# NTU-CompHydroMet-Lab/P2I-GAN-benchmark

Measured on AMD Instinct MI355X. Metric: train frames/sec (128x128x16), higher is better.
Workload: dtype f32

## Files before the change

include/p2i_hip.h:

```cpp
#ifndef P2I_HIP_H
#define P2I_HIP_H
#include <stdint.h>

#ifdef __cplusplus
extern "C" {
#endif

#define P2I_OK 0
#define P2I_EINVAL (-1)
#define P2I_ELDS (-2)

#define P2I_ACT_NONE 0
#define P2I_ACT_RELU 1
#define P2I_ACT_LEAKY 2
#define P2I_ACT_TANH 3

int p2i_abi_version(void);
const char* p2i_last_error(void);

typedef struct {
  int B, Cin, Cout;
  int Ti, Hi, Wi;
  int To, Ho, Wo;
  int kt, kh, kw;
  int st, sh, sw;
  int pt, ph, pw;
} p2i_conv_desc;

int p2i_conv_fwd(const p2i_conv_desc* d, const float* x, const float* wp, const float* bias,
                 const float* residual, float* y, int act, void* stream);
int p2i_conv_dgrad(const p2i_conv_desc* d, const float* dy, const float* y_act, int act,
                   const float* wp_d, const float* dx_add, const float* mask_y, int mask_act,
                   float* dx, void* stream);
int p2i_conv_wgrad(const p2i_conv_desc* d, const float* x, const float* dy, const float* y_act,
                   int act, float* dwp, float* dbias, void* stream);
int p2i_conv_wgrad_ws(const p2i_conv_desc* d, const float* x, const float* dy, const float* y_act, int act, float* dwp,
                      float* dbias, float* ws, int64_t ws_floats, void* stream);
int p2i_conv_fwd_x6(const p2i_conv_desc* d, const float* x, const float* wp, uint16_t* wsplit, const float* bias,
                    const float* residual, float* y, int act, void* stream);
int p2i_conv_dgrad_x6(const p2i_conv_desc* d, const float* dy, const float* wp_d, uint16_t* wsplit, const float* dx_add,
                      const float* mask_y, int mask_act, float* dx, void* stream);
int p2i_x6_split(const float* wp, uint16_t* wb, int ntaps, int K, int Mpad, void* stream);
int p2i_x6_split_batched(const float* const* wp, uint16_t* const* wb, const int* ntaps, const int* K, const int* Mpad, int n,
                         void* stream);
int p2i_x6c_would_take(const p2i_conv_desc* d, int dgrad, int act);
int p2i_conv_fwd_x6s(const p2i_conv_desc* d, const float* x, const float* wp, const uint16_t* wb_layer, int ntaps_w,
                     const float* bias, const float* residual, float* y, int act, void* stream);
int p2i_conv_dgrad_x6s(const p2i_conv_desc* d, const float* dy, const float* wp_d, const uint16_t* wb_layer, int ntaps_w,
                       const float* dx_add, const float* mask_y, int mask_act, float* dx, void* stream);
int p2i_conv_last_plan(int* out6);
int p2i_fast_div_magic(int d, uint32_t* magic);
int p2i_wgrad_last_plan(int* out4);

int p2i_doconv_fold_fwd(const float* W, const float* D, const float* D_diag, int O, int I, int groups,
                        int ksz, int identity_rep, float* wp_f, float* wp_d, void* stream);
int p2i_doconv_fold_bwd(const float* dwp_f, const float* W, const float* D, const float* D_diag,
                        int O, int I, int groups, int ksz, float* dW, float* dD, void* stream);

int p2i_doconv_fold_fwd_batched(const float* const* W, const float* const* D, const float* const* D_diag, int n, int O, int I,
                                float* const* wp_f, float* const* wp_d, void* stream);
int p2i_doconv_fold_bwd_batched(const float* const* dwp_f, const float* const* W, const float* const* D,
                                const float* const* D_diag, int n, int O, int I, float* const* dW, float* const* dD,
                                void* stream);

int p2i_weight_pack(const float* w, int O, int I, int ntaps, const float* inv_div_ptr,
                    float* wp_f, float* wp_d, void* stream);
int p2i_weight_unpack_grad(const float* dwp_f, int O, int I, int ntaps, const float* w_orig,
                           const float* sigma_ptr, const float* u, const float* v, float* scratch,
                           float* dw, void* stream);

int p2i_weight_pack_batched(const float* const* w, const int* O, const int* I, const int* ntaps, const float* const* inv_div,
                            float* const* wp_f, float* const* wp_d, int n, void* stream);
int p2i_weight_unpack_grad_batched(const float* const* dwp_f, const int* O, const int* I, const int* ntaps,
                                   const float* const* w_orig, const float* const* sigma, const float* const* u,
                                   const float* const* v, float* dots, float* const* dw, int n, void* stream);

int p2i_weight_unpack_grad_batched_acc(const float* const* dwp_f, const int* O, const int* I, const int* ntaps,
                                       const float* const* w_orig, const float* const* sigma, const float* const* u,
                                       const float* const* v, float* dots, float* const* dw, int n, int accumulate, void* stream);

int p2i_spectral_norm(const float* w, int O, int K, float* u, float* v, int training, float* sigma,
                      float* scratch, void* stream);

int p2i_spectral_norm_batched(const float* const* w, const int* O, const int* K, float* const* u, float* const* v,
                              int training, float* const* sigma, float* const* scratch, float* const* u_snap,
                              float* const* v_snap, int n, void* stream);

int p2i_attn_fwd(const float* x, const float* w0, const float* b0, const float* w1, const float* b1,
                 float* out, int B, int T, int HW, void* stream);
int p2i_attn_bwd(const float* x, const float* w0, const float* b0, const float* w1, const float* b1,
                 const float* dout, float* dw0, float* db0, float* dw1, float* db1,
                 int B, int T, int HW, void* stream);

int p2i_idw_fwd(const float* vals_src, const float* mask, const float* grid_x, const float* grid_y,
                const float* grid_z, float* out, int32_t* pt_pos, int32_t* pt_count, int32_t* frame_count,
                int32_t* row_start, float* pt_xyzn, int32_t* sel_idx, float* sel_w, int B, int T, int H, int W, float tau,
                void* stream);
int p2i_idw_fwd_ws(const float* vals_src, const float* mask, const float* grid_x, const float* grid_y,
                   const float* grid_z, float* out, int32_t* pt_pos, int32_t* pt_count, int32_t* frame_count,
                   int32_t* row_start, float* pt_xyzn, int32_t* sel_idx, float* sel_w, int32_t* amb, int B, int T, int H, int W,
                   float tau, void* stream);
int p2i_idw_bwd(const float* dout, const int32_t* pt_pos, const int32_t* pt_count, const int32_t* sel_idx,
                const float* sel_w, float* dvals_src, int B, int T, int H, int W, void* stream);

int p2i_pooldup_fwd(const float* x, float* y, int B, int C, int H, int W, void* stream);
int p2i_pooldup_bwd(const float* x, const float* dy, float* dx, int B, int C, int H, int W, void* stream);

int p2i_upmod_fwd(const float* x, const float* pos, float* u, int B, int C, int S, int S2w , void* stream);
int p2i_upmod_fwd_ba(const float* v, const float* pos, const float* bias, int act, float* u, int B, int C, int S, int S2w, void* stream);
int p2i_upmod_bwd(const float* x, const float* pos, const float* du, float* dx, float* dpos,
                  int B, int C, int S, int S2w, void* stream);

int p2i_dtail_fwd(const float* out2d, const float* out3d, const float* alpha2d, float* fused,
                  int B, int H2, int W2, int T3, int H3, int W3, void* stream);
int p2i_dtail_bwd(const float* out2d, const float* alpha2d, const float* dfused, float* dout2d,
                  float* dout3d, float* dalpha2d, int B, int H2, int W2, int T3, int H3, int W3, void* stream);

int p2i_recloss(const float* pred, const float* target, float k1_alpha, float* out3, float* dpred,
                float* scratch, int B, int T, int HW, void* stream);
int p2i_gan_loss(const float* logits_a, const float* logits_b, int n, int loss_type, int mode,
                 float weight, float real_label, float fake_label, float* loss, float* dlogits_a,
                 float* dlogits_b, void* stream);

int p2i_loss_transform_fwd(const float* x, float* y, int64_t n, void* stream);
int p2i_loss_transform_bwd(const float* x, const float* dy, float* dx, int64_t n, void* stream);
int p2i_fdiff_fwd(const float* x, float* out, int B, int T, int64_t inner, void* stream);
int p2i_fdiff_bwd(const float* dy, float* dx, int B, int T, int64_t inner, void* stream);
int p2i_wl1_fwd(const float* pred, const float* target, float* out1, int64_t n, void* stream);
int p2i_wl1_bwd(const float* pred, const float* target, const float* gout, float* dpred, int64_t n, void* stream);
int p2i_softmax_t_fwd(const float* x, float* y, int rows, int L, float temperature, void* stream);
int p2i_softmax_t_bwd(const float* y, const float* dy, float* dx, int rows, int L, float temperature, void* stream);
int p2i_kl_fwd(const float* p, const float* q, float* out1, int64_t n, int B, void* stream);
// ... 226 lines not shown
```

p2i-gan-benchmark_amd/csrc/conv.hip:

```cpp
#include "conv_dma.h"

namespace p2i {


template <int MB, int NPIX, int WAVES_M, int CK>
__global__ __launch_bounds__(256) void patch_gemm_kernel(const PatchGeom g) {
  extern __shared__ __attribute__((aligned(16))) float smem[];
  constexpr int WAVES_N = 4 / WAVES_M;
  constexpr int TM = MB / (32 * WAVES_M);
  constexpr int TN = NPIX / (32 * WAVES_N);
  static_assert(TM >= 1 && TN >= 1, "tile too small");
  float* lw = smem;
  float* lp = smem + g.ntaps * CK * MB;

  const int tid = threadIdx.x, lane = tid & 63, wave = tid >> 6;
  const int wm = wave / WAVES_N, wn = wave % WAVES_N;
  const int l31 = lane & 31, lhi = lane >> 5;

  int tile = blockIdx.x;
  const int tw = tile % g.ntw; tile /= g.ntw;
  const int th = tile % g.nth; tile /= g.nth;
  const int tt = tile % g.ntt;
  const int tb = tile / g.ntt;
  const int j0b = tb << g.ljb, j0t = tt << g.ljt, j0h = th << g.ljh, j0w = tw << g.ljw;
// ... 81 lines not shown
    }
  }

  const int dHW = g.dH * g.dW;
#pragma unroll
  for (int f = 0; f < TN; ++f) {
    const int pix = (wn * TN + f) * 32 + l31;
    const int gw = j0w + (pix & JWm);
    const int gh = j0h + ((pix >> g.ljw) & JHm);
    const int gt = j0t + ((pix >> (g.ljw + g.ljh)) & JTm);
    const int gb = j0b + (pix >> (g.ljw + g.ljh + g.ljt));
    const bool pv = gb < g.B && gt < g.nT && gh < g.nH && gw < g.nW;
    const int sp = (gt * g.oT + g.pT) * dHW + (gh * g.oH + g.pH) * g.dW + gw * g.oW + g.pW;
#pragma unroll
    for (int i = 0; i < TM; ++i) {
#pragma unroll
      for (int r = 0; r < 16; ++r) {
        const int o = o0 + (wm * TM + i) * 32 + (r & 3) + 8 * (r >> 2) + 4 * lhi;
        if (pv && o < g.Cm) {
          float v = acc[i][f][r];
          if (g.bias) v += g.bias[o];
          v = act_apply(v, g.act_epi);
          const size_t di = ((size_t)(gb * g.Cm + o)) * g.dT * dHW + sp;
          if (g.res) v += g.res[di];
          if (g.mask_y) v = act_grad(v, g.mask_y[di], g.mask_act);
          g.dst[di] = v;
        }
      }
    }
  }
}


typedef void (*patch_fn)(const PatchGeom);
template <int MB, int NPIX, int WM, int CK>
static int launch_patch(const PatchGeom& g, dim3 grid, size_t lds, hipStream_t s) {
  auto k = patch_gemm_kernel<MB, NPIX, WM, CK>;
  static bool attr_set = false;
  if (!attr_set) {
    (void)hipFuncSetAttribute((const void*)k, hipFuncAttributeMaxDynamicSharedMemorySize, 160 * 1024);
    attr_set = true;
  }
  P2I_LAUNCH(k, grid, dim3(256), lds, s, g);
  return launch_status();
}

static int dispatch_patch_dma(const TileCfg& c, int KG, const PatchGeom& g, dim3 grid, size_t lds, hipStream_t s) {
  int rc = dispatch_patch_dma_g0(c, KG, g, grid, lds, s);
  if (rc == -1) rc = dispatch_patch_dma_g1(c, KG, g, grid, lds, s);
  if (rc == -1) rc = dispatch_patch_dma_g2(c, KG, g, grid, lds, s);
  if (rc == -1) rc = dispatch_patch_dma_g3(c, KG, g, grid, lds, s);
  if (rc != -1) return rc;
  set_error("no DMA kernel instance for tile cfg %d %d %d %d kg %d", c.MB, c.NPIX, c.WM, c.CK, KG);
  return P2I_EINVAL;
}

static int dispatch_patch(const TileCfg& c, const PatchGeom& g, dim3 grid, size_t lds, hipStream_t s) {
#define P2I_CASE(mb_, npix_, wm_, ck_) \
  if (c.MB == mb_ && c.NPIX == npix_ && c.WM == wm_ && c.CK == ck_) return launch_patch<mb_, npix_, wm_, ck_>(g, grid, lds, s);
  P2I_CASE(128, 256, 2, 8)
  P2I_CASE(64, 256, 1, 8)
  P2I_CASE(64, 128, 2, 8)
  P2I_CASE(32, 128, 1, 8)
  P2I_CASE(128, 256, 2, 4)
  P2I_CASE(64, 256, 1, 4)
  P2I_CASE(64, 128, 2, 4)
  P2I_CASE(32, 128, 1, 4)
  P2I_CASE(128, 256, 2, 2)
  P2I_CASE(64, 256, 1, 2)
  P2I_CASE(64, 128, 2, 2)
  P2I_CASE(32, 128, 1, 2)
#undef P2I_CASE
  set_error("no kernel instance for tile cfg %d %d %d %d", c.MB, c.NPIX, c.WM, c.CK);
  return P2I_EINVAL;
}


static thread_local int g_last_plan[6] = {0, 0, 0, 0, 0, 0};

static int run_patch_gemm(PatchGeom g, const ClassSpec& cs, hipStream_t s);

static int run_patch_gemm_classes(PatchGeom g, const ClassSpec* css, int ncls, hipStream_t s) {
  if (g.src_y != nullptr || ncls > MAX_CLASSES) return 1;
  if (const X6Ctx& xc = x6_ctx(); xc.wb != nullptr) {
    bool all = true;
    for (int q = 0; q < ncls && all; ++q) all = run_patch_gemm_x6c(g, css[q], xc.wb, xc.ntaps_w, nullptr, s, true) == 0;
    if (all) {
      for (int q = 0; q < ncls; ++q)
        if (const int rc = run_patch_gemm_x6c(g, css[q], xc.wb, xc.ntaps_w, g_last_plan, s)) return rc == 1 ? P2I_EINVAL : rc;
      return P2I_OK;
    }
  }
  const ClassSpec& c0s = css[0];
  g.mT = c0s.mT; g.mH = c0s.mH; g.mW = c0s.mW;
  g.oT = c0s.oT; g.oH = c0s.oH; g.oW = c0s.oW;
  int lo[MAX_CLASSES][3], rng[3] = {0, 0, 0}, mx[3] = {0, 0, 0}, max_taps = 0;
  long long total_pix = 0;
  for (int q = 0; q < ncls; ++q) {
    const ClassSpec& cs = css[q];
    int hi[3] = {0, 0, 0};
    lo[q][0] = lo[q][1] = lo[q][2] = 0;
    for (int i = 0; i < cs.ntaps; ++i) {
      const int d[3] = {cs.dt[i], cs.dh[i], cs.dw[i]};
      for (int k = 0; k < 3; ++k) {
        if (i == 0 || d[k] < lo[q][k]) lo[q][k] = d[k];
        if (i == 0 || d[k] > hi[k]) hi[k] = d[k];
      }
    }
    for (int k = 0; k < 3; ++k) if (hi[k] - lo[q][k] > rng[k]) rng[k] = hi[k] - lo[q][k];
    if (cs.nT > mx[0]) mx[0] = cs.nT;
    if (cs.nH > mx[1]) mx[1] = cs.nH;
    if (cs.nW > mx[2]) mx[2] = cs.nW;
    if (cs.ntaps > max_taps) max_taps = cs.ntaps;
    total_pix += (long long)g.B * (cs.nT > 0 ? cs.nT : 0) * (cs.nH > 0 ? cs.nH : 0) * (cs.nW > 0 ? cs.nW : 0);
  }
  if (mx[0] <= 0 || mx[1] <= 0 || mx[2] <= 0) return P2I_OK;
  if (max_taps == 0) max_taps = 1;
  g.ntaps = max_taps;
  static const int cand[5][3] = {{128, 256, 2}, {64, 256, 1}, {128, 128, 2}, {64, 128, 2}, {32, 128, 1}};
  int best = -1, best_ck = 0;
  long long best_score = -1;
  PatchGeom bg = g;
  size_t best_lds = 0;
  dim3 best_grid;
  for (int ci = 0; ci < 5; ++ci) {
    const int MBc = cand[ci][0], NP = cand[ci][1];
    if (MBc > 32 && g.Cm <= MBc / 2) continue;
    int jb, jt, jh, jw;
    pick_tile_dims(NP, g.B, mx[0], mx[1], mx[2], jb, jt, jh, jw);
    PatchGeom t = g;
    t.ljb = ilog2(jb); t.ljt = ilog2(jt); t.ljh = ilog2(jh); t.ljw = ilog2(jw);
    t.eT = (jt - 1) * g.mT + rng[0] + 1;
    t.eH = patch_extent_div((jh - 1) * g.mH + rng[1] + 1);
    t.eW = (jw - 1) * g.mW + rng[2] + 1;
    bool same_lo_w = true;
    for (int q = 1; q < ncls; ++q) same_lo_w = same_lo_w && lo[q][2] == lo[0][2];
    t.v4 = (conv_v4_on() && same_lo_w && (g.sW & 3) == 0 && ((jw * g.mW) & 3) == 0) ? 1 : 0;
    t.v4sh = 0;
    if (t.v4) {
      t.v4sh = ((lo[0][2] % 4) + 4) % 4;
      t.eW = (t.eW + t.v4sh + 3) & ~3;
      t.eW4 = t.eW >> 2;
    }
    if (!t.v4) t.eW = patch_extent_div(t.eW);
    t.eWp = t.eW;
    t.eth = t.eT * t.eH;
    t.rpc = jb * t.eth;
    t.CSl = t.rpc * t.eW;
    t.CS = t.CSl;
    t.G4 = t.CSl >> 2;
    const int force_ck16 = P2I_ENV_ONCE("P2I_CONV_CK16", 0);
    for (int CKc = ((max_taps <= 4 || ((force_ck16 || g.Ck >= 256) && max_taps == 9 && MBc <= 64)) ? 16 : 8); CKc >= 2; CKc >>= 1) {
      if (g.Ck >= CKc ? (g.Ck % CKc != 0) : (CKc != 2 && g.Ck * 2 <= CKc)) continue;
      if (CKc == 2 && !(MBc == 64 && NP == 128) && !(MBc == 32)) continue;
      if ((CKc == 4 || CKc == 16) && MBc == 128 && NP == 128) continue;
      const int PT = CKc * t.CSl;
      if (PT >= 65536 || t.CSl >= 65536) continue;
      const int PTp = t.v4 ? (((PT >> 2) + 63) & ~63) * 4 : (PT + 63) & ~63;
      const int nwrows = max_taps * CKc;
      const size_t WSZ = (size_t)((nwrows * (MBc / 4) + 63) & ~63) * 4;
      const size_t lds = sizeof(float) * (((nwrows + 63) & ~63) + (size_t)PTp + 2 * (WSZ + PTp));
      if (lds > 160 * 1024) continue;
      const long long nb = (long long)ceil_div(g.Cm, MBc) * ((total_pix + NP - 1) / NP);
      long long score = (nb >= 256 ? 1000000000ll : nb * 1000000ll) + (long long)MBc * NP * 10 + CKc + (lds <= 80 * 1024 ? 5 : 0);
      if (score > best_score) {
        best_score = score; best = ci; best_ck = CKc; best_lds = lds;
        bg = t; bg.PT = PT;
// ... 224 lines not shown
        cs.ntaps = n;
        if (mergeable) css[ncls++] = cs;
        else if (int e = run_patch_gemm(g, cs, (hipStream_t)stream)) return e;
      }
  if (mergeable) {
    int rc = 1;
    if (const X6Ctx& xc = x6_ctx(); xc.wb != nullptr && ncls == 4)
      rc = run_patch_gemm_x6c_fused(g, css, ncls, xc.wb, xc.ntaps_w, g_last_plan, (hipStream_t)stream);
    if (rc == 1) rc = (ncls > 1 && x6_ctx().wb == nullptr) ? run_patch_gemm_fused(g, css, ncls, g_last_plan, (hipStream_t)stream) : 1;
    if (rc == 1) rc = ncls > 1 ? run_patch_gemm_classes(g, css, ncls, (hipStream_t)stream) : 1;
    if (rc == 1) {
      for (int q = 0; q < ncls; ++q)
        if (int e = run_patch_gemm(g, css[q], (hipStream_t)stream)) return e;
    } else if (rc != P2I_OK) return rc;
  }
  return P2I_OK;
}


namespace p2i { int x6_split_weights(const float* wp, uint16_t* wb, int ntaps, int Ck, int CmPad, hipStream_t s); }


extern "C" int p2i_conv_fwd_x6(const p2i_conv_desc* d, const float* x, const float* wp, uint16_t* wsplit, const float* bias,
                               const float* residual, float* y, int act, void* stream) {
  if (int e = check_desc(d)) return e;
  if (wsplit == nullptr || (d->Cin & 15) != 0 || !x6c_would_take(d, false, act))
    return p2i_conv_fwd(d, x, wp, bias, residual, y, act, stream);
  P2I_REQUIRE(wp != nullptr, "null pointer");
  const int nt = d->kt * d->kh * d->kw;
  if (int e = x6_split_weights(wp, wsplit, nt, d->Cin, (d->Cout + 31) / 32 * 32, (hipStream_t)stream)) return e;
  x6_ctx() = X6Ctx{wsplit, nt};
  const int rc = p2i_conv_fwd(d, x, wp, bias, residual, y, act, stream);
  x6_ctx() = X6Ctx{nullptr, 0};
  return rc;
}

extern "C" int p2i_conv_dgrad_x6(const p2i_conv_desc* d, const float* dy, const float* wp_d, uint16_t* wsplit, const float* dx_add,
                                 const float* mask_y, int mask_act, float* dx, void* stream) {
  if (int e = check_desc(d)) return e;
  if (wsplit == nullptr || (d->Cout & 15) != 0 || d->Cin == 1 || !x6c_would_take(d, true, P2I_ACT_NONE))
    return p2i_conv_dgrad(d, dy, nullptr, P2I_ACT_NONE, wp_d, dx_add, mask_y, mask_act, dx, stream);
  P2I_REQUIRE(wp_d != nullptr, "null pointer");
  const int nt = d->kt * d->kh * d->kw;
  if (int e = x6_split_weights(wp_d, wsplit, nt, d->Cout, (d->Cin + 31) / 32 * 32, (hipStream_t)stream)) return e;
  x6_ctx() = X6Ctx{wsplit, nt};
  const int rc = p2i_conv_dgrad(d, dy, nullptr, P2I_ACT_NONE, wp_d, dx_add, mask_y, mask_act, dx, stream);
  x6_ctx() = X6Ctx{nullptr, 0};
  return rc;
}

extern "C" int p2i_x6_split(const float* wp, uint16_t* wb, int ntaps, int K, int Mpad, void* stream) {
  P2I_REQUIRE(wp && wb && ntaps > 0 && K > 0 && (K & 7) == 0 && Mpad > 0 && (Mpad & 31) == 0, "p2i_x6_split: bad arguments");
  return x6_split_weights(wp, wb, ntaps, K, Mpad, (hipStream_t)stream);
}

extern "C" int p2i_x6c_would_take(const p2i_conv_desc* d, int dgrad, int act) {
  if (check_desc(d)) return 0;
  if (dgrad ? ((d->Cout & 15) != 0 || d->Cin == 1) : (d->Cin & 15) != 0) return 0;
  return x6c_would_take(d, dgrad != 0, dgrad ? P2I_ACT_NONE : act) ? 1 : 0;
}

extern "C" int p2i_conv_fwd_x6s(const p2i_conv_desc* d, const float* x, const float* wp, const uint16_t* wb_layer, int ntaps_w,
                                const float* bias, const float* residual, float* y, int act, void* stream) {
  if (int e = check_desc(d)) return e;
  if (wb_layer == nullptr || (d->Cin & 15) != 0 || !x6c_would_take(d, false, act)) return p2i_conv_fwd(d, x, wp, bias, residual, y, act, stream);
  P2I_REQUIRE(ntaps_w >= d->kt * d->kh * d->kw, "ntaps_w smaller than the layer's tap count");
  x6_ctx() = X6Ctx{wb_layer, ntaps_w};
  const int rc = p2i_conv_fwd(d, x, wp, bias, residual, y, act, stream);
  x6_ctx() = X6Ctx{nullptr, 0};
  return rc;
}

extern "C" int p2i_conv_dgrad_x6s(const p2i_conv_desc* d, const float* dy, const float* wp_d, const uint16_t* wb_layer, int ntaps_w,
                                  const float* dx_add, const float* mask_y, int mask_act, float* dx, void* stream) {
  if (int e = check_desc(d)) return e;
  if (wb_layer == nullptr || (d->Cout & 15) != 0 || d->Cin == 1 || !x6c_would_take(d, true, P2I_ACT_NONE))
    return p2i_conv_dgrad(d, dy, nullptr, P2I_ACT_NONE, wp_d, dx_add, mask_y, mask_act, dx, stream);
  P2I_REQUIRE(ntaps_w >= d->kt * d->kh * d->kw, "ntaps_w smaller than the layer's tap count");
  x6_ctx() = X6Ctx{wb_layer, ntaps_w};
  const int rc = p2i_conv_dgrad(d, dy, nullptr, P2I_ACT_NONE, wp_d, dx_add, mask_y, mask_act, dx, stream);
  x6_ctx() = X6Ctx{nullptr, 0};
  return rc;
}
```

p2i-gan-benchmark_amd/csrc/conv_common.h:

```cpp
#pragma once
#include "common.h"

namespace p2i {

typedef float f32x16 __attribute__((ext_vector_type(16)));
constexpr int MAX_TAPS = 27;

typedef __attribute__((address_space(3))) void lds_void;
typedef int v4i32 __attribute__((ext_vector_type(4)));

__device__ __forceinline__ v4i32 make_rsrc(const void* p, unsigned bytes) {
  const unsigned long long a = (unsigned long long)p;
  v4i32 r;
  r[0] = __builtin_amdgcn_readfirstlane((int)(unsigned)a);
  r[1] = __builtin_amdgcn_readfirstlane((int)(unsigned)(a >> 32));
  r[2] = __builtin_amdgcn_readfirstlane((int)bytes);
  r[3] = 0x00020000;
  return r;
}
__device__ __forceinline__ unsigned lds_base(const float* shared_array) {
  return (unsigned)(size_t)(const lds_void*)shared_array;
}
__device__ __forceinline__ void dma_b32(const v4i32 rsrc, unsigned lds_addr, int voff, int soff) {
  const unsigned la = __builtin_amdgcn_readfirstlane(lds_addr);
// ... 59 lines not shown
                                                  const float* __restrict__ res, const float* __restrict__ mask_y, int mask_act,
                                                  float* __restrict__ dst, bool atomic_out) {
#pragma unroll
  for (int k = 0; k < 8; ++k) {
    float v = acc[h8 * 8 + k];
    if (bias) v += b.bv[k];
    v = act_apply(v, act_epi);
    if (res) v += b.rv[k];
    if (mask_y) v = act_grad(v, b.mv[k], mask_act);
    if (b.ok[k]) {
      if (atomic_out) atomicAdd(dst + b.di[k], v);
      else dst[b.di[k]] = v;
    }
  }
}
__device__ __forceinline__ void epilogue_tile16(const f32x16& acc, int o_base, int lhi, int Cm, bool pv, size_t pos_off, size_t chan_stride,
                                                const float* __restrict__ bias, int act_epi, const float* __restrict__ res,
                                                const float* __restrict__ mask_y, int mask_act, float* __restrict__ dst,
                                                bool atomic_out = false) {
#pragma unroll
  for (int h8 = 0; h8 < 2; ++h8) {
    int di[8];
    bool ok[8];
#pragma unroll
    for (int k = 0; k < 8; ++k) {
      const int r = h8 * 8 + k;
      const int o = o_base + (r & 3) + 8 * (r >> 2) + 4 * lhi;
      ok[k] = pv && o < Cm;
      di[k] = ok[k] ? (int)((size_t)o * chan_stride + pos_off) : 0;
    }
    float rv[8], mv[8];
    if (res) {
#pragma unroll
      for (int k = 0; k < 8; ++k) rv[k] = res[di[k]];
    }
    if (mask_y) {
#pragma unroll
      for (int k = 0; k < 8; ++k) mv[k] = mask_y[di[k]];
    }
#pragma unroll
    for (int k = 0; k < 8; ++k) {
      const int r = h8 * 8 + k;
      const int o = o_base + (r & 3) + 8 * (r >> 2) + 4 * lhi;
      float v = acc[r];
      if (bias) v += bias[o < Cm ? o : 0];
      v = act_apply(v, act_epi);
      if (res) v += rv[k];
      if (mask_y) v = act_grad(v, mv[k], mask_act);
      if (ok[k]) {
        if (atomic_out) atomicAdd(dst + di[k], v);
        else dst[di[k]] = v;
      }
    }
    __builtin_amdgcn_sched_barrier(0);
  }
}

typedef float f32x4e __attribute__((ext_vector_type(4)));
struct EpiOps4v {
  int di[4];
  bool ok[4];
  f32x4e rv[4], mv[4];
  float bv[4];
};
__device__ __forceinline__ void epi_tile16_v4_fetch(EpiOps4v& b, int o_base, int lane, int Cm, size_t pos4_off, bool pv4, size_t chan_stride,
                                                    const float* __restrict__ bias, const float* __restrict__ res, const float* __restrict__ mask_y) {
#pragma unroll
  for (int k = 0; k < 4; ++k) {
    const int o = o_base + k * 8 + (lane >> 3);
    b.ok[k] = pv4 && o < Cm;
    b.di[k] = b.ok[k] ? (int)((size_t)o * chan_stride + pos4_off) : 0;
    b.bv[k] = bias ? bias[o < Cm ? o : 0] : 0.f;
  }
  if (res) {
#pragma unroll
    for (int k = 0; k < 4; ++k) b.rv[k] = *reinterpret_cast<const f32x4e*>(res + b.di[k]);
  }
  if (mask_y) {
#pragma unroll
    for (int k = 0; k < 4; ++k) b.mv[k] = *reinterpret_cast<const f32x4e*>(mask_y + b.di[k]);
  }
}
__device__ __forceinline__ void epi_tile16_v4_finish(const EpiOps4v& b, const f32x16& acc, float* __restrict__ tile_lds, int lane, int act_epi, const float* __restrict__ res,
                                                     const float* __restrict__ mask_y, int mask_act, float* __restrict__ dst, bool atomic_out) {
  constexpr int PITCH = 36;
  const int l31 = lane & 31, lhi = lane >> 5;
#pragma unroll
  for (int r = 0; r < 16; ++r) tile_lds[((r & 3) + 8 * (r >> 2) + 4 * lhi) * PITCH + l31] = acc[r];
  __builtin_amdgcn_fence(__ATOMIC_RELEASE, "wavefront");
  __builtin_amdgcn_wave_barrier();
  const int p4 = (lane & 7) * 4;
  f32x4e v[4];
#pragma unroll
  for (int k = 0; k < 4; ++k) v[k] = *reinterpret_cast<const f32x4e*>(tile_lds + (k * 8 + (lane >> 3)) * PITCH + p4);
#pragma unroll
  for (int k = 0; k < 4; ++k) {
#pragma unroll
    for (int e = 0; e < 4; ++e) {
      float x = act_apply(v[k][e] + b.bv[k], act_epi);
      if (res) x += b.rv[k][e];
      if (mask_y) x = act_grad(x, b.mv[k][e], mask_act);
      v[k][e] = x;
    }
    if (b.ok[k]) {
      if (atomic_out) {
#pragma unroll
        for (int e = 0; e < 4; ++e) atomicAdd(dst + b.di[k] + e, v[k][e]);
      } else {
        *reinterpret_cast<f32x4e*>(dst + b.di[k]) = v[k];
      }
    }
  }
  __builtin_amdgcn_wave_barrier();
}

typedef float f32x2e __attribute__((ext_vector_type(2)));
struct EpiOps4p {
  int di[4];
  bool ok[4];
  f32x2e rv[4], mv[4];
};
__device__ __forceinline__ void epi_pair16_fetch(EpiOps4p& b, int h4, int o_base, int lhi, int Cm, bool pv, size_t pos_off, size_t chan_stride,
                                                 const float* __restrict__ res, const float* __restrict__ mask_y) {
#pragma unroll
  for (int k = 0; k < 4; ++k) {
    const int r = h4 * 4 + k;
    const int o = o_base + (r & 3) + 8 * (r >> 2) + 4 * lhi;
    b.ok[k] = pv && o < Cm;
    b.di[k] = b.ok[k] ? (int)((size_t)o * chan_stride + pos_off) : 0;
  }
  if (res) {
#pragma unroll
    for (int k = 0; k < 4; ++k) b.rv[k] = *reinterpret_cast<const f32x2e*>(res + b.di[k]);
  }
  if (mask_y) {
#pragma unroll
    for (int k = 0; k < 4; ++k) b.mv[k] = *reinterpret_cast<const f32x2e*>(mask_y + b.di[k]);
  }
}
__device__ __forceinline__ void epi_pair16_finish(const EpiOps4p& b, int h4, const f32x16& acc0, const f32x16& acc1,
                                                  const float* __restrict__ res, const float* __restrict__ mask_y, int mask_act,
                                                  float* __restrict__ dst, bool atomic_out) {
#pragma unroll
  for (int k = 0; k < 4; ++k) {
    const int r = h4 * 4 + k;
    f32x2e v;
    v[0] = acc0[r]; v[1] = acc1[r];
    if (res) { v[0] += b.rv[k][0]; v[1] += b.rv[k][1]; }
    if (mask_y) { v[0] = act_grad(v[0], b.mv[k][0], mask_act); v[1] = act_grad(v[1], b.mv[k][1], mask_act); }
    if (b.ok[k]) {
      if (atomic_out) { atomicAdd(dst + b.di[k], v[0]); atomicAdd(dst + b.di[k] + 1, v[1]); }
      else *reinterpret_cast<f32x2e*>(dst + b.di[k]) = v;
    }
  }
}
__device__ __forceinline__ void epilogue_pair16(const f32x16& acc0, const f32x16& acc1, int o_base, int lhi, int Cm, bool pv, size_t pos_off,
                                                size_t chan_stride, const float* __restrict__ res, const float* __restrict__ mask_y,
                                                int mask_act, float* __restrict__ dst, bool atomic_out = false) {
#pragma unroll
  for (int h4 = 0; h4 < 4; ++h4) {
    int di[4];
    bool ok[4];
#pragma unroll
    for (int k = 0; k < 4; ++k) {
      const int r = h4 * 4 + k;
      const int o = o_base + (r & 3) + 8 * (r >> 2) + 4 * lhi;
      ok[k] = pv && o < Cm;
      di[k] = ok[k] ? (int)((size_t)o * chan_stride + pos_off) : 0;
    }
    f32x2e rv[4], mv[4];
    if (res) {
#pragma unroll
      for (int k = 0; k < 4; ++k) rv[k] = *reinterpret_cast<const f32x2e*>(res + di[k]);
    }
    if (mask_y) {
#pragma unroll
      for (int k = 0; k < 4; ++k) mv[k] = *reinterpret_cast<const f32x2e*>(mask_y + di[k]);
    }
#pragma unroll
    for (int k = 0; k < 4; ++k) {
      const int r = h4 * 4 + k;
      f32x2e v;
      v[0] = acc0[r]; v[1] = acc1[r];
      if (res) { v[0] += rv[k][0]; v[1] += rv[k][1]; }
      if (mask_y) { v[0] = act_grad(v[0], mv[k][0], mask_act); v[1] = act_grad(v[1], mv[k][1], mask_act); }
      if (ok[k]) {
        if (atomic_out) { atomicAdd(dst + di[k], v[0]); atomicAdd(dst + di[k] + 1, v[1]); }
        else *reinterpret_cast<f32x2e*>(dst + di[k]) = v;
      }
    }
    __builtin_amdgcn_sched_barrier(0);
  }
// ... 9 lines not shown
  jt = pow2_ceil(nT); if (jt > rem) jt = rem;
  rem /= jt;
  jb = rem;
  (void)B;
}


static inline int check_desc(const p2i_conv_desc* d) {
  P2I_REQUIRE(d != nullptr, "null conv desc");
  P2I_REQUIRE(d->B > 0 && d->Cin > 0 && d->Cout > 0, "bad channel/batch dims");
  P2I_REQUIRE(d->kt >= 1 && d->kh >= 1 && d->kw >= 1 && d->kt * d->kh * d->kw <= MAX_TAPS, "kernel taps > %d", MAX_TAPS);
  P2I_REQUIRE(d->st >= 1 && d->sh >= 1 && d->sw >= 1, "bad stride");
  P2I_REQUIRE(d->To == (d->Ti + 2 * d->pt - d->kt) / d->st + 1, "To inconsistent");
  P2I_REQUIRE(d->Ho == (d->Hi + 2 * d->ph - d->kh) / d->sh + 1, "Ho inconsistent");
  P2I_REQUIRE(d->Wo == (d->Wi + 2 * d->pw - d->kw) / d->sw + 1, "Wo inconsistent");
  const long long nin = (long long)d->B * d->Cin * d->Ti * d->Hi * d->Wi;
  const long long nout = (long long)d->B * d->Cout * d->To * d->Ho * d->Wo;
  P2I_REQUIRE(nin < (1ll << 31) && nout < (1ll << 31), "tensor too large for 32-bit indexing");
  return P2I_OK;
}


struct ClassGeom {
  int nT, nH, nW, pT, pH, pW, bT, bH, bW, ntaps;
  short tap_w[MAX_TAPS];
  int tap_off[MAX_TAPS];
};
constexpr int MAX_CLASSES = 8;

struct PatchGeom {
  const float* src;
  const float* src_y;
  const float* wp;
  const float* bias;
  const float* res;
  float* dst;
  int act_epi;
  int act_pro;
  int B, Ck, Cm, CmPad;
  int sT, sH, sW;
  int dT, dH, dW;
  int nT, nH, nW;
  int mT, mH, mW;
  int oT, oH, oW;
  int pT, pH, pW;
  int bT, bH, bW;
  int eT, eH, eW, eWp;
  int ljb, ljt, ljh, ljw;
  int ntt, nth, ntw;
  int ntaps;
  int CS;
  int rpc, eth;
  unsigned mg_rpc, mg_eth, mg_eh;
  short tap_w[MAX_TAPS];
  int tap_off[MAX_TAPS];
  const float* mask_y;
  int mask_act;
  int CSl;
  int PT;
  unsigned src_bytes, wp_bytes;
  unsigned mg_csl, mg_ew;
  int v4, v4sh;
  int eW4, G4;
  unsigned mg_g4, mg_ew4;
  const uint16_t* wb;
  unsigned wb_bytes;
  int ntaps_w;
  int TG, NTP, R;
  int ksplit;
  int pair_w;
  int nclass;
  ClassGeom cls[MAX_CLASSES];
};

struct ClassSpec {
  int nT, nH, nW;
  int mT, mH, mW;
  int oT, oH, oW, pT, pH, pW;
  int ntaps;
  short tw[MAX_TAPS];
  int dt[MAX_TAPS], dh[MAX_TAPS], dw[MAX_TAPS];
};

struct X6Ctx { const uint16_t* wb; int ntaps_w; };
X6Ctx& x6_ctx();

int run_patch_gemm_x6c(const PatchGeom& g, const ClassSpec& cs, const uint16_t* wb, int ntaps_w, int* plan6, hipStream_t s, bool dry = false);
int run_patch_gemm_x6c_fused(const PatchGeom& g, const ClassSpec* css, int ncls, const uint16_t* wb, int ntaps_w, int* plan6, hipStream_t s, bool dry = false);
bool x6c_would_take(const p2i_conv_desc* d, bool dgrad, int act_epi);

int run_patch_gemm_fused(PatchGeom g, const ClassSpec* css, int ncls, int* plan6, hipStream_t s);

int c1_dgrad(const p2i_conv_desc* d, const float* dy, const float* wp_d, const float* add, const float* mask_y, int mask_act,
             float* dx, hipStream_t s);
int c1_wgrad(const p2i_conv_desc* d, const float* x, const float* dy, float* dwp, float* dbias, hipStream_t s);
int c1_fwd(const p2i_conv_desc* d, const float* x, const float* wp, const float* bias, float* y, int act, hipStream_t s);
int o1_fwd(const p2i_conv_desc* d, const float* x, const float* wp, const float* bias, float* y, int act, hipStream_t s);

}
```

p2i-gan-benchmark_amd/csrc/conv_x6c.hip:

```cpp
#include "conv_common.h"

namespace p2i {

#ifdef P2I_STAMP
extern __device__ unsigned long long* p2i_stamp_buf;
#define X6C_NOW(v) do { __builtin_amdgcn_sched_barrier(0); asm volatile("s_memtime %0\n\ts_waitcnt lgkmcnt(0)" : "=s"(v) :: "memory"); __builtin_amdgcn_sched_barrier(0); } while (0)
#define X6C_ACC(sum, t_prev) do { unsigned long long t_; X6C_NOW(t_); sum += t_ - t_prev; t_prev = t_; } while (0)
#else
#define X6C_NOW(v) do { } while (0)
#define X6C_ACC(sum, t_prev) do { } while (0)
#endif

typedef __bf16 bf16x8c __attribute__((ext_vector_type(8)));
typedef unsigned u32x4c __attribute__((ext_vector_type(4)));

__device__ __forceinline__ unsigned pack_hi16c(float lo_elem, float hi_elem) {
  return __builtin_amdgcn_perm(__float_as_uint(hi_elem), __float_as_uint(lo_elem), 0x07060302u);
}
__device__ __forceinline__ float trunc_bf16c(float v) { return __uint_as_float(__float_as_uint(v) & 0xFFFF0000u); }
__device__ __forceinline__ void split8c(const float (&v)[8], u32x4c& hi, u32x4c& mid, u32x4c& lo) {
#pragma unroll
  for (int j = 0; j < 4; ++j) {
    const float a = v[2 * j], b = v[2 * j + 1];
    hi[j] = pack_hi16c(a, b);
    const float ra = a - trunc_bf16c(a), rb = b - trunc_bf16c(b);
    mid[j] = pack_hi16c(ra, rb);
    const float sa = ra - trunc_bf16c(ra), sb = rb - trunc_bf16c(rb);
    lo[j] = pack_hi16c(sa, sb);
  }
}

template <class S, class I>
__device__ __forceinline__ void split8_store(const float* __restrict__ p, S stride, u32x4c* __restrict__ out, I total, I i) {
  float v[8];
#pragma unroll
  for (int q = 0; q < 8; ++q) v[q] = p[(S)q * stride];
  u32x4c h, mi, lo;
  split8c(v, h, mi, lo);
  out[i] = h;
  out[total + i] = mi;
  out[2 * total + i] = lo;
}

__global__ __launch_bounds__(256) void wsplit_kernel(const float* __restrict__ wp, u32x4c* __restrict__ wb, int ntaps, int Ck, int CmPad) {
  const int KCt = Ck >> 3;
  const int total = ntaps * KCt * CmPad;
  for (int i = blockIdx.x * 256 + threadIdx.x; i < total; i += gridDim.x * 256) {
    const int m = i % CmPad;
    const int r = i / CmPad;
    const int kc = r % KCt, tap = r / KCt;
    const float* p = wp + ((size_t)tap * Ck + kc * 8) * CmPad + m;
    split8_store(p, (size_t)CmPad, wb, total, i);
  }
}

struct WsplitBatch { const float* wp[24]; u32x4c* wb[24]; int ntaps[24], Ck[24], CmPad[24]; };
__global__ __launch_bounds__(256) void wsplit_batched_kernel(const WsplitBatch b) {
  const int L = blockIdx.y;
  const float* wp = b.wp[L];
  u32x4c* wb = b.wb[L];
  const int Ck = b.Ck[L], CmPad = b.CmPad[L], KCt = Ck >> 3;
  const int total = b.ntaps[L] * KCt * CmPad;
  for (int i = blockIdx.x * 256 + threadIdx.x; i < total; i += gridDim.x * 256) {
    const int m = i % CmPad;
    const int r = i / CmPad;
    const int kc = r % KCt, tap = r / KCt;
    const float* p = wp + ((size_t)tap * Ck + kc * 8) * CmPad + m;
    split8_store(p, (size_t)CmPad, wb, total, i);
  }
}

__global__ __launch_bounds__(256) void split_planes_kernel(const float* __restrict__ x, u32x4c* __restrict__ planes, int B, int KCt, long long P) {
  const long long total = (long long)B * KCt * P;
  for (long long i = blockIdx.x * 256ll + threadIdx.x; i < total; i += (long long)gridDim.x * 256) {
    const long long pix = i % P, r = i / P;
    const float* px = x + (r * 8) * P + pix;
    split8_store(px, P, planes, total, i);
  }
}

X6Ctx& x6_ctx() {
  static thread_local X6Ctx c{nullptr, 0};
  return c;
}

int x6_split_weights(const float* wp, uint16_t* wb, int ntaps, int Ck, int CmPad, hipStream_t s) {
  const int total = ntaps * (Ck >> 3) * CmPad;
  const int blocks = total > 0 ? (total + 255) / 256 : 1;
  P2I_LAUNCH(wsplit_kernel, dim3(blocks > 2048 ? 2048 : blocks), dim3(256), 0, s, wp, reinterpret_cast<u32x4c*>(wb), ntaps, Ck, CmPad);
  return launch_status();
}

struct X6cGeom {
  const float* src; float* dst; const uint16_t* wb; const float* bias; const float* res; const float* mask_y;
  unsigned wb_bytes;
  int act_epi, mask_act;
  int B, Ck, Cm, CmPad;
  int sH, sW, dT, dH, dW, nH, nW;
  int ljb, ljh, ljw, eH, eW, CSl, bH, bW, nth, ntw;
  unsigned mg_ew, mg_eh;
  int ntaps_w, ksplit;
  int sT, nT, mT, oT, pT, ns, sdt0, sdt1, sdt2, swt0, swt1, swt2;
  int tap_off[9];
  int tap_w[9];
  int fused_atomic;
  int stagger;
  int vec4_epi;
  const u32x4c* splanes;
  unsigned plane_units;
  int cons_prio;
};

__device__ constexpr int X6C_CLS[9] = {3, 3, 3, 3, 2, 2, 1, 1, 0};

template <int NW> struct X6cTile {
  static constexpr int MAXCSL = NW == 8 ? 384 : 256;
  static constexpr int NI = (2 * MAXCSL + 64 * NW - 1) / (64 * NW);
};

#define X6C_WAIT1(b) asm volatile("s_waitcnt vmcnt(%0)" ::"n"(b) : "memory")
#define X6C_WAIT2(b) if (n < (b) + 1) { X6C_WAIT1(b); } else { X6C_WAIT1((b) + 1); }
#define X6C_WAIT4(b) if (n < (b) + 2) { X6C_WAIT2(b) } else { X6C_WAIT2((b) + 2) }
#define X6C_WAIT8(b) if (n < (b) + 4) { X6C_WAIT4(b) } else { X6C_WAIT4((b) + 4) }
#define X6C_WAIT16(b) if (n < (b) + 8) { X6C_WAIT8(b) } else { X6C_WAIT8((b) + 8) }
#define X6C_WAIT32(b) if (n < (b) + 16) { X6C_WAIT16(b) } else { X6C_WAIT16((b) + 16) }
__device__ __forceinline__ void x6c_wait_vm(int n) {
  if (n < 0 || n > 62) n = 0;
  if (n < 32) { X6C_WAIT32(0) } else { X6C_WAIT32(32) }
}

template <int NW, int TM, bool FUSED = false, int TPS = 3>
__global__ __launch_bounds__(64 * NW) void patch_gemm_x6c_kernel(const X6cGeom g) {
  constexpr int NCLS = FUSED ? 4 : 1;
  constexpr int NSTG = 9 / TPS;
  static_assert(TPS == 3 || TPS == 9, "taps per stage");
  extern __shared__ __attribute__((aligned(16))) float smem[];
#ifdef P2I_STAMP
  unsigned long long st_entry, st_prev, st_wait = 0, st_bar = 0, st_issue = 0, st_mfma = 0, st_loop0;
  X6C_NOW(st_entry);
#endif
  constexpr int MB = 32 * TM, NTHR = 64 * NW, NI = X6cTile<NW>::NI;
  constexpr int RING = TPS == 9 ? 3 : (TM == 2 ? 4 : 6), LEAD = RING - 1;
  constexpr int WST = 6 * TPS * MB;
  constexpr int NWI = WST / 64;
  const int CSl = g.CSl;
  int* ptab = reinterpret_cast<int*>(smem);
  const int ptab_sz = (CSl + 3) & ~3;
  u32x4c* wbuf = reinterpret_cast<u32x4c*>(smem + ptab_sz);
  u32x4c* planes = wbuf + RING * WST;
  const int PST = 6 * CSl;

  const int tid = threadIdx.x, lane = tid & 63, wave = __builtin_amdgcn_readfirstlane(tid >> 6);
  const int l31 = lane & 31, lhi = lane >> 5;
  int tile = blockIdx.x;
  const int tw = tile % g.ntw; tile /= g.ntw;
  const int th = tile % g.nth;
  const int tb = tile / g.nth;
  const int j0b = tb << g.ljb, j0h = th << g.ljh, j0w = tw << g.ljw;
  const int o0 = blockIdx.y * MB;
  const int JWm = (1 << g.ljw) - 1, JHm = (1 << g.ljh) - 1;
  const int sHW = g.sH * g.sW;
  const int src_h0 = j0h + g.bH, src_w0 = j0w + g.bW;
  const int KCt = g.Ck >> 3;
  const int cps = g.Ck >> 4;
  const int cs = g.sT * sHW;
  const int nimg = g.B * g.nT;
  const int c0 = blockIdx.z * ((g.ns * cps) / g.ksplit);

  for (int e = tid; e < CSl; e += NTHR) {
    const int row = fast_div(e, g.mg_ew);
    const int ew = e - row * g.eW;
    const int jb = fast_div(row, g.mg_eh);
    const int eh = row - jb * g.eH;
    const int n = j0b + jb, h = src_h0 + eh, w = src_w0 + ew;
    const int b = n / g.nT, lt = n - b * g.nT;
    ptab[e] = (n < nimg && (unsigned)h < (unsigned)g.sH && (unsigned)w < (unsigned)g.sW) ? ((b * g.Ck) * g.sT + lt * g.mT) * sHW + h * g.sW + w : -1;
  }
  const int pix = wave * 32 + l31;
  const int pjw = pix & JWm, pjh = (pix >> g.ljw) & JHm, pjb = pix >> (g.ljw + g.ljh);
  const int lane_base = (pjb * g.eH + pjh) * g.eW + pjw + lhi * CSl;
  int toff[9];
#pragma unroll
  for (int t = 0; t < 9; ++t) toff[t] = g.tap_off[t];

  f32x16 acc[NCLS][TM];
#pragma unroll
  for (int q = 0; q < NCLS; ++q)
#pragma unroll
    for (int i = 0; i < TM; ++i)
#pragma unroll
      for (int r = 0; r < 16; ++r) acc[q][i][r] = 0.f;

  const v4i32 rs_w = make_rsrc(g.wb, g.wb_bytes);
// ... 162 lines not shown
      if (TPS == 9 || !late) staging();
      X6C_ACC(st_issue, st_prev);
      const u32x4c* wsl = wlane + (s % RING) * WST;
      __builtin_amdgcn_sched_barrier(0);
#pragma unroll
      for (int t = 0; t < TPS - 1; ++t) {
        if constexpr (TPS == 9) {
          if (more_c && (t == 4 || t == 6 || t == 7) && t == split_t) {
            x6c_wait_vm(nwb(sa));
            __builtin_amdgcn_sched_barrier(0);
            split_patch(planes + ((c + 1) & 1) * PST);
            __builtin_amdgcn_sched_barrier(0);
          }
        }
        load_tap(wsl, pb, TPS * b + t + 1, (t + 1) % 3);
        mfma_tap(t % 3, TPS * b + t);
        ilv();
        __builtin_amdgcn_sched_barrier(0);
      }
      if (TPS == 3 && late) { staging(); __builtin_amdgcn_sched_barrier(0); }
      X6C_ACC(st_mfma, st_prev);
      {
        int n = 0;
#pragma unroll
        for (int j = 2; j <= LEAD; ++j) n += nwb(s + j);
        if constexpr (TPS == 3) {
#pragma unroll
          for (int j = 0; j <= LEAD - 2; ++j) {
            const int bj = ((b - j) % 3 + 3) % 3;
            if (bj == 0 && s - j >= 0 && (s - j) / 3 + 1 < nch) n += NPL;
          }
        }
        x6c_wait_vm(n);
      }
      asm volatile("s_waitcnt lgkmcnt(0)" ::: "memory");
      X6C_ACC(st_wait, st_prev);
      __builtin_amdgcn_s_barrier();
      X6C_ACC(st_bar, st_prev);
      if (s + 1 < nst) load_tap(wlane + ((s + 1) % RING) * WST, b == NSTG - 1 ? pbn : pb, b == NSTG - 1 ? 0 : TPS * b + TPS, 0);
      mfma_tap(2, TPS * b + TPS - 1);
      ilv();
      __builtin_amdgcn_sched_barrier(0);
      X6C_ACC(st_mfma, st_prev);
    }
  }
#ifdef P2I_STAMP
  unsigned long long st_loop_end; X6C_NOW(st_loop_end);
#endif

  const int gw = j0w + pjw, gh = j0h + pjh, gn = j0b + pjb;
  const bool pvld = gn < nimg && gh < g.nH && gw < g.nW;
  const int dHW = g.dT * g.dH * g.dW;
  const int gb_ = gn / g.nT, glt = gn - gb_ * g.nT;
  if constexpr (FUSED) {
    const size_t pos0 = (size_t)gb_ * g.Cm * dHW + (size_t)(glt * g.oT + g.pT) * g.dH * g.dW + (size_t)(2 * gh) * g.dW + 2 * gw;
#pragma unroll
    for (int ph = 0; ph < 2; ++ph)
#pragma unroll
      for (int i = 0; i < TM; ++i)
        epilogue_pair16(acc[2 * ph][i], acc[2 * ph + 1][i], o0 + i * 32, lhi, g.Cm, pvld, pos0 + (size_t)ph * g.dW, (size_t)dHW,
                        (g.fused_atomic && blockIdx.z) ? nullptr : g.res, g.mask_y, g.mask_act, g.dst, g.fused_atomic != 0);
  } else {
    const size_t pos = (size_t)gb_ * g.Cm * dHW + (size_t)(glt * g.oT + g.pT) * g.dH * g.dW + (size_t)gh * g.dW + gw;
#pragma unroll
    for (int i = 0; i < TM; ++i)
      if (g.ksplit > 1)
        epilogue_tile16(acc[0][i], o0 + i * 32, lhi, g.Cm, pvld, pos, (size_t)dHW, blockIdx.z ? nullptr : g.bias, P2I_ACT_NONE,
                        blockIdx.z ? nullptr : g.res, g.mask_y, g.mask_act, g.dst, true);
      else
        epilogue_tile16(acc[0][i], o0 + i * 32, lhi, g.Cm, pvld, pos, (size_t)dHW, g.bias, g.act_epi, g.res, g.mask_y, g.mask_act, g.dst);
  }
#ifdef P2I_STAMP
  if (p2i_stamp_buf && lane == 0) {
    asm volatile("s_waitcnt vmcnt(0)" ::: "memory");
    unsigned long long st_x; X6C_NOW(st_x);
    unsigned long long* o = p2i_stamp_buf + ((size_t)(blockIdx.x + gridDim.x * blockIdx.y) * NW + wave) * 8;
    o[0] = st_wait; o[1] = st_bar; o[2] = st_issue; o[3] = st_mfma; o[4] = st_loop_end - st_loop0; o[5] = st_loop0; o[6] = st_loop0 - st_entry;
    o[7] = st_x - st_loop_end;
  }
#endif
}


template <int TM, int TPS, bool FUSED = false, bool EPI4 = false, int NPW = 4, int TN = 2, bool PRE = false>
__global__ __launch_bounds__(64 * (4 + NPW)) void patch_gemm_x6p_kernel(const X6cGeom g) {
  constexpr int NSTG = 9 / TPS;
  constexpr int NCLS = FUSED ? 4 : 1;
  static_assert(TPS == 3 || TPS == 9, "taps per stage");
  extern __shared__ __attribute__((aligned(16))) float smem[];
  constexpr int MB = 32 * TM, NCW = 4, NTHR = 64 * (NCW + NPW), NPT = 64 * NPW;
  constexpr int NI = (2 * (TN == 2 ? X6cTile<8>::MAXCSL : X6cTile<4>::MAXCSL) + NPT - 1) / NPT;
  constexpr int RING = TPS == 9 ? 3 : (TM == 2 ? 4 : 6), LEAD = RING - 1;
  constexpr int WST = 6 * TPS * MB, NWI = WST / 64;
  const int CSl = g.CSl;
  int* ptab = reinterpret_cast<int*>(smem);
  const int ptab_sz = (CSl + 3) & ~3;
  u32x4c* wbuf = reinterpret_cast<u32x4c*>(smem + ptab_sz);
  u32x4c* planes = wbuf + RING * WST;
  const int PST = 6 * CSl;

  const int tid = threadIdx.x, lane = tid & 63, wave = __builtin_amdgcn_readfirstlane(tid >> 6);
  const int l31 = lane & 31, lhi = lane >> 5;
  int tile = blockIdx.x;
  const int tw = tile % g.ntw; tile /= g.ntw;
  const int th = tile % g.nth;
  const int tb = tile / g.nth;
  const int j0b = tb << g.ljb, j0h = th << g.ljh, j0w = tw << g.ljw;
  const int o0 = blockIdx.y * MB;
  const int JWm = (1 << g.ljw) - 1, JHm = (1 << g.ljh) - 1;
  const int sHW = g.sH * g.sW;
  const int src_h0 = j0h + g.bH, src_w0 = j0w + g.bW;
  const int KCt = g.Ck >> 3;
  const int cps = g.Ck >> 4;
  const int cs = g.sT * sHW;
  const int nimg = g.B * g.nT;
  const int c0 = blockIdx.z * ((g.ns * cps) / g.ksplit);
  const int nch = (g.ns * cps) / g.ksplit;
  const int nst = NSTG * nch;

  for (int e = tid; e < CSl; e += NTHR) {
    const int row = fast_div(e, g.mg_ew);
    const int ew = e - row * g.eW;
    const int jb = fast_div(row, g.mg_eh);
    const int eh = row - jb * g.eH;
    const int n = j0b + jb, h = src_h0 + eh, w = src_w0 + ew;
    const int b = n / g.nT, lt = n - b * g.nT;
    ptab[e] = (n < nimg && (unsigned)h < (unsigned)g.sH && (unsigned)w < (unsigned)g.sW) ? ((b * (PRE ? KCt : g.Ck)) * g.sT + lt * g.mT) * sHW + h * g.sW + w : -1;
  }
  __syncthreads();

#ifdef P2I_STAMP
  unsigned long long st_a = 0, st_b = 0, st_c = 0, st_d = 0, st_e = 0, st_f = 0, st_t0, st_t1, st_l0 = 0, st_l1 = 0, st_entry;
  X6C_NOW(st_entry);
#endif
  if (wave >= NCW) {
    const int ptid = tid - 64 * NCW, pw = wave - NCW;
    const v4i32 rs_w = make_rsrc(g.wb, g.wb_bytes);
    const unsigned wbuf_la = lds_base(smem) + 4u * ptab_sz;
    const int wl_m = TM == 2 ? lane : l31, wl_kg = TM == 2 ? 0 : lhi;
    const int wvoff = (o0 + wl_m < g.CmPad) ? (wl_kg * g.CmPad + wl_m) * 16 : -16;
    int it_off[NI], it_dst[NI], it_f0[NI];
#pragma unroll
    for (int it = 0; it < NI; ++it) {
      const int item = it * NPT + ptid;
      const int kg = item >= CSl ? 1 : 0, e = item - kg * CSl;
      const bool in = item < 2 * CSl;
      const int po = in ? ptab[e] : -1;
      it_off[it] = po < 0 ? -1 : po + kg * (PRE ? 1 : 8) * cs;
      it_dst[it] = in ? kg * CSl + e : -1;
      const int jbi = fast_div(fast_div(in ? e : 0, g.mg_ew), g.mg_eh);
      it_f0[it] = ((j0b + jbi) % g.nT) * g.mT;
    }
    float pv[PRE ? 1 : NI][8];
    u32x4c pq[PRE ? NI : 1][3];
    bool pok[NI];
    auto load_patch = [&](int c) {
      if constexpr (PRE) {
        const int cg = c0 + c;
        const int j = cg >= 2 * cps ? 2 : (cg >= cps ? 1 : 0);
        const int dt = j == 2 ? g.sdt2 : (j == 1 ? g.sdt1 : g.sdt0);
        int voff[NI];
#pragma unroll
        for (int it = 0; it < NI; ++it) {
          pok[it] = it_off[it] >= 0 && (unsigned)(it_f0[it] + dt) < (unsigned)g.sT;
          voff[it] = pok[it] ? (it_off[it] + dt * sHW) * 16 : 0;
        }
#pragma unroll
        for (int p = 0; p < 3; ++p) {
          const u32x4c* sq = g.splanes + (size_t)p * g.plane_units + (size_t)(cg - j * cps) * 2 * cs;
          const unsigned long long sq_u = (unsigned long long)__builtin_amdgcn_readfirstlane((int)(unsigned)(unsigned long long)sq) & 0xffffffffull;
          const unsigned long long sq_hi = (unsigned long long)(unsigned)__builtin_amdgcn_readfirstlane((int)((unsigned long long)sq >> 32));
          const unsigned long long sbase = sq_u | (sq_hi << 32);
#pragma unroll
          for (int it = 0; it < NI; ++it) {
            if (it == 0) asm volatile("s_nop 4\n\tglobal_load_dwordx4 %0, %1, %2" : "=v"(pq[it][p]) : "v"(voff[it]), "s"(sbase) : "memory");
            else asm volatile("global_load_dwordx4 %0, %1, %2" : "=v"(pq[it][p]) : "v"(voff[it]), "s"(sbase) : "memory");
          }
        }
      } else {
      const int cg = c0 + c;
      const int j = cg >= 2 * cps ? 2 : (cg >= cps ? 1 : 0);
      const int dt = j == 2 ? g.sdt2 : (j == 1 ? g.sdt1 : g.sdt0);
      const float* sc = g.src + (size_t)(cg - j * cps) * 16 * cs;
      int voff[NI];
#pragma unroll
      for (int it = 0; it < NI; ++it) {
        pok[it] = it_off[it] >= 0 && (unsigned)(it_f0[it] + dt) < (unsigned)g.sT;
        voff[it] = pok[it] ? (it_off[it] + dt * sHW) * 4 : 0;
      }
#pragma unroll
      for (int q = 0; q < 8; ++q) {
        const float* sq = sc + (size_t)q * cs;
        const unsigned long long sq_u = (unsigned long long)__builtin_amdgcn_readfirstlane((int)(unsigned)(unsigned long long)sq) & 0xffffffffull;
        const unsigned long long sq_hi = (unsigned long long)(unsigned)__builtin_amdgcn_readfirstlane((int)((unsigned long long)sq >> 32));
        const unsigned long long sbase = sq_u | (sq_hi << 32);
#pragma unroll
        for (int it = 0; it < NI; ++it) {
          if (it == 0) asm volatile("s_nop 4\n\tglobal_load_dword %0, %1, %2" : "=v"(pv[it][q]) : "v"(voff[it]), "s"(sbase) : "memory");
          else asm volatile("global_load_dword %0, %1, %2" : "=v"(pv[it][q]) : "v"(voff[it]), "s"(sbase) : "memory");
        }
      }
      }
    };
    auto split_patch = [&](u32x4c* pb) {
      if constexpr (PRE) {
#pragma unroll
        for (int it = 0; it < NI; ++it)
#pragma unroll
          for (int p = 0; p < 3; ++p) asm volatile("" : "+v"(pq[it][p]));
        const u32x4c zero = {0u, 0u, 0u, 0u};
#pragma unroll
        for (int it = 0; it < NI; ++it) {
          if (it_dst[it] < 0) continue;
          pb[it_dst[it]] = pok[it] ? pq[it][0] : zero;
          pb[2 * CSl + it_dst[it]] = pok[it] ? pq[it][1] : zero;
          pb[4 * CSl + it_dst[it]] = pok[it] ? pq[it][2] : zero;
        }
      } else {
#pragma unroll
      for (int it = 0; it < NI; ++it)
#pragma unroll
        for (int q = 0; q < 8; ++q) asm volatile("" : "+v"(pv[it][q]));
#pragma unroll
      for (int it = 0; it < NI; ++it) {
        if (it_dst[it] < 0) continue;
        float v[8];
#pragma unroll
        for (int q = 0; q < 8; ++q) v[q] = pok[it] ? pv[it][q] : 0.f;
        u32x4c h, mi, lo;
        split8c(v, h, mi, lo);
        pb[it_dst[it]] = h;
        pb[2 * CSl + it_dst[it]] = mi;
        pb[4 * CSl + it_dst[it]] = lo;
      }
      }
    };
    constexpr int NWR = (NWI + NPW - 1) / NPW;
    int w_soff[NWR][NSTG];
    unsigned w_dst[NWR];
#pragma unroll
    for (int r = 0; r < NWR; ++r) {
      const int u = pw + NPW * r;
      const int pt = TM == 2 ? u >> 1 : u, kg = TM == 2 ? u & 1 : 0;
      const int p = pt / TPS, tl = pt % TPS;
#pragma unroll
      for (int b = 0; b < NSTG; ++b)
        w_soff[r][b] = u < NWI ? __builtin_amdgcn_readfirstlane((((p * g.ntaps_w + g.tap_w[TPS * b + tl]) * KCt + kg) * g.CmPad + o0) * 16) : 0;
      w_dst[r] = wbuf_la + 16u * (unsigned)(u * 64);
    }
    const int w_cstep = 2 * g.CmPad * 16;
    const int w_tstep = KCt * g.CmPad * 16;
    auto issue_w = [&](int c, int b, int sb) {
      const int cg = c0 + c;
      const int j = cg >= 2 * cps ? 2 : (cg >= cps ? 1 : 0);
      const int soff = (cg - j * cps) * w_cstep + (j == 2 ? g.swt2 : (j == 1 ? g.swt1 : g.swt0)) * w_tstep;
#pragma unroll
      for (int r = 0; r < NWR; ++r)
        if (pw + NPW * r < NWI) dma_b128(rs_w, w_dst[r] + 16u * (unsigned)(sb * WST), wvoff, w_soff[r][b] + soff);
    };
    const int nw_mine = (NWI / NPW) + (pw < NWI % NPW ? 1 : 0);
    constexpr int NPL = (PRE ? 3 : 8) * NI;
    auto nwb = [&](int st) { return (st >= LEAD && st < nst) ? nw_mine : 0; };
    load_patch(0);
    {
      int n = 0;
#pragma unroll
      for (int st = 0; st < LEAD; ++st) n += nwb(st);
      x6c_wait_vm(n);
      __builtin_amdgcn_sched_barrier(0);
      split_patch(planes);
      if constexpr (TPS == 9) {
        if (nch > 1) load_patch(1);
        x6c_wait_vm(n - nwb(0) + (nch > 1 ? NPL : 0));
      } else {
        x6c_wait_vm(n - nwb(0));
      }
    }
    asm volatile("s_waitcnt lgkmcnt(0)" ::: "memory");
    __builtin_amdgcn_s_barrier();
    int s = 0;
    for (int c = 0; c < nch; ++c) {
      const bool more_c = c + 1 < nch;
#pragma unroll
      for (int b = 0; b < NSTG; ++b, ++s) {
        const int sa = s + LEAD;
        if constexpr (TPS == 9) {
#ifdef P2I_STAMP
          X6C_NOW(st_t0);
          if (s == 0) st_l0 = st_t0;
#endif
          if (more_c) {
            x6c_wait_vm(s == 0 ? 0 : nwb(s - 1 + LEAD));
            X6C_ACC(st_a, st_t0);
            __builtin_amdgcn_sched_barrier(0);
            split_patch(planes + ((c + 1) & 1) * PST);
            __builtin_amdgcn_sched_barrier(0);
            X6C_ACC(st_b, st_t0);
            if (c + 2 < nch) load_patch(c + 2);
            X6C_ACC(st_e, st_t0);
          }
          if (sa < nst) issue_w(c + LEAD, 0, sa % RING);
          X6C_ACC(st_f, st_t0);
          x6c_wait_vm(nwb(s + 2) + ((more_c && c + 2 < nch) ? NPL : 0));
          X6C_ACC(st_c, st_t0);
        } else {
          if (b == 0 && more_c) load_patch(c + 1);
          if (sa < nst) issue_w(c + (b + LEAD) / NSTG, (b + LEAD) % NSTG, sa % RING);
          if (b == NSTG - 1 && more_c) {
            int n = 0;
#pragma unroll
            for (int j = 0; j < NSTG; ++j) n += nwb(sa - j);
            x6c_wait_vm(n);
            __builtin_amdgcn_sched_barrier(0);
            split_patch(planes + ((c + 1) & 1) * PST);
          }
          int n = 0;
#pragma unroll
          for (int j = 2; j <= LEAD; ++j) n += nwb(s + j);
#pragma unroll
          for (int j = 0; j <= LEAD - 2; ++j) {
            const int sj = s - j;
            if (sj >= 0 && sj % NSTG == 0 && sj / NSTG + 1 < nch) n += NPL;
          }
          x6c_wait_vm(n);
        }
        asm volatile("s_waitcnt lgkmcnt(0)" ::: "memory");
#ifdef P2I_STAMP
        X6C_NOW(st_t1);
#endif
        __builtin_amdgcn_s_barrier();
#ifdef P2I_STAMP
        X6C_ACC(st_d, st_t1);
        st_l1 = st_t1;
#endif
      }
    }
  }

  const bool producer = wave >= NCW;
  const int cw = wave & (NCW - 1);
  int lane_base[TN], pjw_[TN], pjh_[TN], pjb_[TN];
#pragma unroll
  for (int nb = 0; nb < TN; ++nb) {
    const int pix = cw * 32 * TN + nb * 32 + l31;
    pjw_[nb] = pix & JWm; pjh_[nb] = (pix >> g.ljw) & JHm; pjb_[nb] = pix >> (g.ljw + g.ljh);
    lane_base[nb] = (pjb_[nb] * g.eH + pjh_[nb]) * g.eW + pjw_[nb] + lhi * CSl;
  }
  int toff[9];
#pragma unroll
  for (int t = 0; t < 9; ++t) toff[t] = g.tap_off[t];
  f32x16 acc[NCLS][TM][TN];
#pragma unroll
  for (int q = 0; q < NCLS; ++q)
#pragma unroll
    for (int i = 0; i < TM; ++i)
#pragma unroll
      for (int nb = 0; nb < TN; ++nb)
#pragma unroll
        for (int r = 0; r < 16; ++r) acc[q][i][nb][r] = 0.f;
  constexpr int PA[6] = {2, 0, 1, 1, 0, 0};
  constexpr int PB[6] = {0, 2, 1, 0, 1, 0};
  u32x4c A[3][TM][3], Bv[3][TN][3];
  auto load_tap = [&](const u32x4c* wsl, const u32x4c* pbuf, int tap, int buf) {
    const int tl = tap % TPS;
    const int to = toff[tap];
#pragma unroll
    for (int p = 0; p < 3; ++p) {
#pragma unroll
      for (int i = 0; i < TM; ++i) A[buf][i][p] = wsl[((p * TPS + tl) * 2) * MB + 32 * i];
#pragma unroll
      for (int nb = 0; nb < TN; ++nb) Bv[buf][nb][p] = pbuf[lane_base[nb] + p * 2 * CSl + to];
    }
  };
  auto mfma_tap = [&](int buf, int slot) {
    const int cl = FUSED ? X6C_CLS[slot] : 0;
#pragma unroll
    for (int q = 0; q < 6; ++q)
#pragma unroll
      for (int i = 0; i < TM; ++i)
#pragma unroll
        for (int nb = 0; nb < TN; ++nb)
          acc[cl][i][nb] = __builtin_amdgcn_mfma_f32_32x32x16_bf16(__builtin_bit_cast(bf16x8c, A[buf][i][PA[q]]), __builtin_bit_cast(bf16x8c, Bv[buf][nb][PB[q]]),
                                                                   acc[cl][i][nb], 0, 0, 0);
  };
  auto ilv = [&]() {
    constexpr int NR = 3 * TM + 3 * TN, NM = 6 * TM * TN;
#pragma unroll
    for (int i = 0; i < NM; ++i) {
      __builtin_amdgcn_sched_group_barrier(0x008, 1, 0);
      if (i < NR) __builtin_amdgcn_sched_group_barrier(0x100, 1, 0);
    }
  };
  const int dHW = g.dT * g.dH * g.dW;
  const int mynb = (TN == 2 && producer) ? 1 : 0;
  const bool has_epi = wave < 2 * NCW;
  const bool split = FUSED ? g.fused_atomic != 0 : g.ksplit > 1;
  const float* const bias_q = (split && blockIdx.z) ? nullptr : g.bias;
  const float* const res_q = (split && blockIdx.z) ? nullptr : g.res;
  const bool blk1 = TN == 2 && producer;
  const int gw = j0w + (blk1 ? pjw_[TN - 1] : pjw_[0]), gh = j0h + (blk1 ? pjh_[TN - 1] : pjh_[0]), gn = j0b + (blk1 ? pjb_[TN - 1] : pjb_[0]);
  const bool pvld = gn < nimg && gh < g.nH && gw < g.nW;
  const int gb_ = gn / g.nT, glt = gn - gb_ * g.nT;
  const size_t img0 = (size_t)gb_ * g.Cm * dHW + (size_t)(glt * g.oT + g.pT) * g.dH * g.dW;
  const size_t pos0 = img0 + (size_t)(2 * gh) * g.dW + 2 * gw;
  const size_t pos = img0 + (size_t)gh * g.dW + gw;
  const int pg = cw * 32 * TN + mynb * 32 + 4 * (lane & 7);
  const int qw = pg & JWm, qh = (pg >> g.ljw) & JHm, qb = pg >> (g.ljw + g.ljh);
  const int hw = j0w + qw, hh = j0h + qh, hn = j0b + qb;
  const bool pv4 = hn < nimg && hh < g.nH && hw < g.nW;
  const int hb = hn / g.nT, hlt = hn - hb * g.nT;
  const size_t pos4 = (size_t)hb * g.Cm * dHW + (size_t)(hlt * g.oT + g.pT) * g.dH * g.dW + (size_t)hh * g.dW + hw;
  float* xch = reinterpret_cast<float*>(wbuf);
  float* tl = xch + 4 * NCLS * TM * 16 * 64 + wave * (32 * 36);
  EpiOps4p ops_p[FUSED ? 2 : 1];
  EpiOps4v ops_v[(!FUSED && EPI4) ? 2 : 1];
  EpiOps8 ops_t[(!FUSED && !EPI4) ? 2 : 1];
  auto fetch = [&](int slot, int k) {
    if constexpr (FUSED)
      epi_pair16_fetch(ops_p[slot], k & 3, o0 + ((k >> 2) % TM) * 32, lhi, g.Cm, pvld, pos0 + (size_t)(k / (4 * TM)) * g.dW, (size_t)dHW, res_q, g.mask_y);
    else if constexpr (EPI4)
      epi_tile16_v4_fetch(ops_v[slot], o0 + k * 32, lane, g.Cm, pos4, pv4, (size_t)dHW, bias_q, res_q, g.mask_y);
    else
      epi_tile16_fetch(ops_t[slot], k & 1, o0 + (k >> 1) * 32, lhi, g.Cm, pvld, pos, (size_t)dHW, bias_q, res_q, g.mask_y);
  };
  constexpr bool EARLY_C = !FUSED && TN == 1;
  const u32x4c* wlane = wbuf + lhi * MB + l31;
  if (!producer) {
    {
      const v4i32 rs_w = make_rsrc(g.wb, g.wb_bytes);
      const unsigned wbuf_la = lds_base(smem) + 4u * ptab_sz;
      const int wl_m = TM == 2 ? lane : l31, wl_kg = TM == 2 ? 0 : lhi;
      const int wvoff = (o0 + wl_m < g.CmPad) ? (wl_kg * g.CmPad + wl_m) * 16 : -16;
      const int w_cstep = 2 * g.CmPad * 16, w_tstep = KCt * g.CmPad * 16;
#pragma unroll
      for (int st = 0; st < LEAD; ++st) {
        if (st >= nst) break;
        const int cg = c0 + st / NSTG, b = st % NSTG;
        const int j = cg >= 2 * cps ? 2 : (cg >= cps ? 1 : 0);
        const int soff = (cg - j * cps) * w_cstep + (j == 2 ? g.swt2 : (j == 1 ? g.swt1 : g.swt0)) * w_tstep;
        for (int u = cw; u < NWI; u += NCW) {
          const int pt = TM == 2 ? u >> 1 : u, kg = TM == 2 ? u & 1 : 0;
          const int p = pt / TPS, tl = pt % TPS;
          const int so = (((p * g.ntaps_w + g.tap_w[TPS * b + tl]) * KCt + kg) * g.CmPad + o0) * 16 + soff;
          dma_b128(rs_w, wbuf_la + 16u * (unsigned)(u * 64 + (st % RING) * WST), wvoff, so);
        }
      }
      asm volatile("s_waitcnt vmcnt(0)" ::: "memory");
    }
    __builtin_amdgcn_s_barrier();
    if (g.cons_prio == 1) __builtin_amdgcn_s_setprio(1);
    else if (g.cons_prio == 2) __builtin_amdgcn_s_setprio(2);
    else if (g.cons_prio == 3) __builtin_amdgcn_s_setprio(3);
    load_tap(wlane, planes, 0, 0);
    int s = 0;
    for (int c = 0; c < nch; ++c) {
      const u32x4c* pb = planes + (c & 1) * PST;
      const u32x4c* pbn = planes + ((c + 1) & 1) * PST;
#pragma unroll
      for (int b = 0; b < NSTG; ++b, ++s) {
        const u32x4c* wsl = wlane + (s % RING) * WST;
        if constexpr (EARLY_C) { if (s + 1 == nst) fetch(0, 0); }
        __builtin_amdgcn_sched_barrier(0);
#pragma unroll
        for (int t = 0; t < TPS - 1; ++t) {
          load_tap(wsl, pb, TPS * b + t + 1, (t + 1) % 3);
          mfma_tap(t % 3, TPS * b + t);
          ilv();
          __builtin_amdgcn_sched_barrier(0);
        }
#ifdef P2I_STAMP
        X6C_NOW(st_t0);
        if (s == 0) st_l0 = st_t0;
#endif
        asm volatile("s_waitcnt lgkmcnt(0)" ::: "memory");
        X6C_ACC(st_a, st_t0);
        __builtin_amdgcn_s_barrier();
#ifdef P2I_STAMP
        X6C_ACC(st_d, st_t0);
        st_l1 = st_t0;
#endif
        if (s + 1 < nst) load_tap(wlane + ((s + 1) % RING) * WST, b == NSTG - 1 ? pbn : pb, b == NSTG - 1 ? 0 : TPS * b + TPS, 0);
        mfma_tap(2, TPS * b + TPS - 1);
        ilv();
        __builtin_amdgcn_sched_barrier(0);
      }
    }
  }
  if (!producer && g.cons_prio) __builtin_amdgcn_s_setprio(0);
  if (TN == 1 && producer) return;
  if (has_epi && !(EARLY_C && !producer)) fetch(0, 0);
  if constexpr (TN == 2) {
    if (!producer) {
#pragma unroll
      for (int q = 0; q < NCLS; ++q)
#pragma unroll
        for (int i = 0; i < TM; ++i)
#pragma unroll
          for (int r = 0; r < 16; ++r) xch[(((cw * NCLS + q) * TM + i) * 16 + r) * 64 + lane] = acc[q][i][1][r];
    }
    asm volatile("s_waitcnt lgkmcnt(0)" ::: "memory");
    __builtin_amdgcn_s_barrier();
    asm volatile("" ::: "memory");
    if (!has_epi) return;
    if (producer) {
#pragma unroll
      for (int q = 0; q < NCLS; ++q)
#pragma unroll
        for (int i = 0; i < TM; ++i)
#pragma unroll
          for (int r = 0; r < 16; ++r) acc[q][i][0][r] = xch[(((cw * NCLS + q) * TM + i) * 16 + r) * 64 + lane];
    }
  }
  if constexpr (FUSED) {
    auto finish = [&](int slot, int k) {
      const int ph = k / (4 * TM), i = (k >> 2) % TM;
      epi_pair16_finish(ops_p[slot], k & 3, acc[2 * ph][i][0], acc[2 * ph + 1][i][0], res_q, g.mask_y, g.mask_act, g.dst, split);
    };
    epilogue_pipelined<8 * TM>(fetch, finish, true);
  } else if constexpr (EPI4) {
    if (split) epilogue_pipelined<TM>(fetch, [&](int slot, int k) {
      epi_tile16_v4_finish(ops_v[slot], acc[0][k][0], tl, lane, P2I_ACT_NONE, res_q, g.mask_y, g.mask_act, g.dst, true); }, true);
    else epilogue_pipelined<TM>(fetch, [&](int slot, int k) {
      epi_tile16_v4_finish(ops_v[slot], acc[0][k][0], tl, lane, g.act_epi, g.res, g.mask_y, g.mask_act, g.dst, false); }, true);
  } else {
    if (split) epilogue_pipelined<2 * TM>(fetch, [&](int slot, int k) {
      epi_tile16_finish(ops_t[slot], k & 1, acc[0][k >> 1][0], bias_q, P2I_ACT_NONE, res_q, g.mask_y, g.mask_act, g.dst, true); }, true);
    else epilogue_pipelined<2 * TM>(fetch, [&](int slot, int k) {
      epi_tile16_finish(ops_t[slot], k & 1, acc[0][k >> 1][0], g.bias, g.act_epi, g.res, g.mask_y, g.mask_act, g.dst, false); }, true);
  }
#ifdef P2I_STAMP
  if (p2i_stamp_buf && lane == 0) {
    asm volatile("s_waitcnt vmcnt(0)" ::: "memory");
    unsigned long long st_end; X6C_NOW(st_end);
    unsigned long long* o = p2i_stamp_buf + ((size_t)(blockIdx.x + gridDim.x * blockIdx.y) * 8 + wave) * 8;
    o[0] = st_a; o[1] = st_d; o[2] = st_b; o[3] = st_c; o[4] = st_l1 - st_l0; o[5] = st_l0 - st_entry; o[6] = st_e; o[7] = st_end - st_l1;
  }
#endif
}

static bool x6c_on() { return P2I_ENV_ONCE("P2I_CONV_X6C", 1) != 0; }
static bool x6c_fused_on() { return P2I_ENV_ONCE("P2I_CONV_X6C_FUSED", 1) != 0; }
static int x6c_min_wg() { return env_int("P2I_X6C_MIN_WG", 200); }
static int x6c_min_wg_low() { return env_int("P2I_X6C_MIN_WG", env_int("P2I_X6C_MIN_WG_LOW", 64)); }
static int x6c_fused_min_wg() { return env_int("P2I_X6C_MIN_WG", 128); }
static int x6p_tn1() { return env_int("P2I_X6P_TN1", 1); }
static int x6c_forced() { return env_int("P2I_X6C_TILE", 0); }
static int x6c_stagger() { return env_int("P2I_X6C_STAGGER", 0); }
static int x6c_fused_ksplit() { return env_int("P2I_X6C_FUSED_KSPLIT", 0); }
static int x6p_npw() { return env_int("P2I_X6P_NPW", 8) == 4 ? 4 : 8; }
static int x6c_pc() { return env_int("P2I_X6C_PC", 1); }
static int x6c_tps1() { return env_int("P2I_X6C_TPS", 9) == 3 ? 3 : 9; }
static int x6p_prio() { return env_int("P2I_X6P_PRIO", 0); }

struct X6cVariant { int NW, TM; };
static const X6cVariant kX6cVariants[] = {{8, 2}, {8, 1}, {4, 1}};

struct X6cPick { int v, jb, jh, jw, csl, ksplit; long long wgs; };
static X6cPick x6c_pick(int B, int nH, int nW, int Cm, int Ck, bool linear_epi, int Ck_slice) {
  int forced = x6c_forced();
  const int min_wg = x6c_min_wg();
  const bool tn1_ok = x6c_pc() && Ck_slice >= 32;
  if (forced == 41 && !tn1_ok) forced = 81;
  const int ksplit_on = P2I_ENV_ONCE("P2I_X6C_KSPLIT", 1);
  static const int order_a[5][2] = {{0, 0}, {1, 0}, {2, 0}, {1, 1}, {0, 1}}, order_b[5][2] = {{0, 0}, {0, 1}, {1, 0}, {2, 0}, {1, 1}};
  X6cPick low{-1, 0, 0, 0, 0, 1, 0};
  for (int cand = 0; cand < 5; ++cand) {
      const int v = (ksplit_on == 2 ? order_b : order_a)[cand][0], pass = (ksplit_on == 2 ? order_b : order_a)[cand][1];
      const X6cVariant& t = kX6cVariants[v];
      if (v == 2 && (!tn1_ok || (forced ? forced != 41 : !x6p_tn1()))) continue;
      if (forced && forced != t.NW * 10 + t.TM) continue;
      if (t.TM == 2 && Cm <= 32 && !forced) continue;
      if (pass == 1 && ((ksplit_on != 2 && t.TM != 1) || !ksplit_on || !linear_epi || ((Ck >> 4) & 1) || forced)) continue;
      int jb, jt, jh, jw;
      pick_tile_dims(32 * t.NW, B, 1, nH, nW, jb, jt, jh, jw);
      const int csl = jb * (jh + 2) * (jw + 2);
      if (jt != 1 || csl > (t.NW == 8 ? X6cTile<8>::MAXCSL : X6cTile<4>::MAXCSL)) continue;
      const long long wgs = (long long)ceil_div(B, jb) * ceil_div(nH, jh) * ceil_div(nW, jw) * ceil_div(Cm, 32 * t.TM) * (pass + 1);
      if (wgs >= min_wg) return X6cPick{v, jb, jh, jw, csl, pass + 1, wgs};
      if (pass == 0 && !forced && wgs >= x6c_min_wg_low() && (low.v < 0 || wgs > low.wgs)) low = X6cPick{v, jb, jh, jw, csl, 1, wgs};
    }
  return low;
}

static X6cPick x6c_fused_pick(int nimg, int nH, int nW, int Cm, int chunks, bool may_split) {
  X6cPick pk{-1, 0, 0, 0, 0, 1, 0};
  int jt;
  pick_tile_dims(256, nimg, 1, nH, nW, pk.jb, jt, pk.jh, pk.jw);
  pk.csl = pk.jb * (pk.jh + 1) * (pk.jw + 1);
  if (jt != 1 || pk.csl > X6cTile<8>::MAXCSL) return pk;
  const long long tiles = (long long)ceil_div(nimg, pk.jb) * ceil_div(nH, pk.jh) * ceil_div(nW, pk.jw) * ceil_div(Cm, 32);
  const bool can_split = x6c_fused_ksplit() && may_split && (chunks & 1) == 0;
  const int min_wg = x6c_fused_min_wg();
  if (tiles < min_wg && !(can_split && 2 * tiles >= min_wg)) return pk;
  pk.ksplit = tiles < min_wg ? 2 : 1;
  pk.wgs = tiles * pk.ksplit;
  pk.v = 1;
  return pk;
}

bool x6c_would_take(const p2i_conv_desc* d, bool dgrad, int act_epi) {
  const bool on = x6c_on();
  (void)act_epi;
  if (on && dgrad && d->sh == 2 && d->sw == 2 && d->st == 1 && d->kh == 3 && d->kw == 3 && d->ph == 1 && d->pw == 1 &&
      ((d->kt == 1 && d->pt == 0) || (d->kt == 3 && d->pt == 1)) && (d->Cout & 15) == 0 && d->Cout >= 16 && !(d->Hi & 1) && !(d->Wi & 1))
    return x6c_fused_on() && x6c_fused_pick(d->B * d->Ti, d->Hi / 2, d->Wi / 2, d->Cin, d->kt * (d->Cout >> 4), true).v >= 0;
  if (!on || d->kh != 3 || d->kw != 3 || d->sh != 1 || d->sw != 1 || d->ph != 1 || d->pw != 1) return false;
  const bool flat = d->kt == 1 && d->st == 1 && d->pt == 0;
  const bool vol = d->kt == 3 && d->pt == 1 && d->st <= 2;
  if (!flat && !vol) return false;
  const int Ck = dgrad ? d->Cout : d->Cin, Cm = dgrad ? d->Cin : d->Cout;
  const int nH = dgrad ? d->Hi : d->Ho, nW = dgrad ? d->Wi : d->Wo;
  if ((Ck & 15) != 0 || Ck < 16) return false;
  const int nT = dgrad ? d->Ti / d->st : d->To;
  if (nT < 1) return false;
  const int ns = flat ? 1 : (dgrad && d->st == 2 ? 1 : 3);
  const bool whole = !dgrad || d->st == 1;
  return x6c_pick(d->B * nT, nH, nW, Cm, ns * Ck, whole, Ck).v >= 0;
}

__global__ __launch_bounds__(256) void x6c_post_act_kernel(float* __restrict__ y, const float* __restrict__ res, long long n4, int act) {
  typedef float f32x4p __attribute__((ext_vector_type(4)));
  for (long long i = blockIdx.x * 256ll + threadIdx.x; i < n4; i += (long long)gridDim.x * 256) {
    f32x4p v = reinterpret_cast<f32x4p*>(y)[i];
#pragma unroll
    for (int e = 0; e < 4; ++e) v[e] = act_apply(v[e], act);
    if (res) {
      const f32x4p r = reinterpret_cast<const f32x4p*>(res)[i];
#pragma unroll
      for (int e = 0; e < 4; ++e) v[e] += r[e];
    }
    reinterpret_cast<f32x4p*>(y)[i] = v;
  }
}

static thread_local const void* g_next_splanes = nullptr;

static size_t x6c_lds_bytes(int csl, int tm, int tps) {
  const int ring = tps == 9 ? 3 : (tm == 2 ? 4 : 6);
  return sizeof(float) * (size_t)((csl + 3) & ~3) + 16 * (size_t)(ring * 6 * tps * 32 * tm + 2 * 6 * csl);
}

static X6cGeom x6c_geom(const PatchGeom& g, const ClassSpec* css, int ncls, const X6cPick& pk, int halo, int ns, const uint16_t* wb, int ntaps_w) {
  const ClassSpec& c0 = css[0];
  X6cGeom k{};
  k.src = g.src; k.dst = g.dst; k.wb = wb; k.bias = g.bias; k.res = g.res; k.mask_y = g.mask_y;
  int tw_max = 0;
  for (int q = 0; q < ncls; ++q)
    for (int i = 0; i < css[q].ntaps; ++i) tw_max = css[q].tw[i] > tw_max ? css[q].tw[i] : tw_max;
  k.wb_bytes = (2u * (unsigned)ntaps_w + (unsigned)tw_max + 1u) * (unsigned)g.Ck * (unsigned)g.CmPad * 2u;
  k.act_epi = g.act_epi; k.mask_act = g.mask_act;
  k.B = g.B; k.Ck = g.Ck; k.Cm = g.Cm; k.CmPad = g.CmPad;
  k.sH = g.sH; k.sW = g.sW; k.dT = g.dT; k.dH = g.dH; k.dW = g.dW; k.nH = c0.nH; k.nW = c0.nW;
  k.ljb = ilog2(pk.jb); k.ljh = ilog2(pk.jh); k.ljw = ilog2(pk.jw);
  k.eH = pk.jh + halo; k.eW = pk.jw + halo; k.CSl = pk.csl;
  k.nth = ceil_div(c0.nH, pk.jh); k.ntw = ceil_div(c0.nW, pk.jw);
  k.mg_ew = magic_u16(k.eW); k.mg_eh = magic_u16(k.eH);
  k.ntaps_w = ntaps_w; k.ksplit = pk.ksplit;
  k.sT = g.sT; k.nT = c0.nT; k.mT = c0.mT; k.oT = c0.oT; k.pT = c0.pT; k.ns = ns;
  k.stagger = x6c_stagger(); k.cons_prio = x6p_prio();
  return k;
}

template <void (*KERN)(const X6cGeom), int NTHR>
static void x6c_launch(const X6cGeom& k, dim3 grid, size_t lds, hipStream_t s) {
  static bool attr_set = false;
  if (!attr_set) {
    (void)hipFuncSetAttribute((const void*)KERN, hipFuncAttributeMaxDynamicSharedMemorySize, 160 * 1024);
    attr_set = true;
  }
  P2I_LAUNCH(KERN, grid, dim3(NTHR), lds, s, k);
}
static void x6c_dispatch(const X6cGeom& k, const X6cVariant& tv, int tps, bool fused, int* plan6, hipStream_t s) {
  const size_t lds = x6c_lds_bytes(k.CSl, tv.TM, tps);
  const dim3 grid((unsigned)(ceil_div(k.B * k.nT, 1 << k.ljb) * k.nth * k.ntw), (unsigned)ceil_div(k.Cm, 32 * tv.TM), (unsigned)k.ksplit);
  const bool pc = x6c_pc() && k.Ck >= 32 && (!fused || tps == 9);
  if (plan6) { plan6[0] = 32 * tv.TM; plan6[1] = 32 * tv.NW; plan6[2] = k.ksplit; plan6[3] = pc ? 4 : 8; plan6[4] = tps; plan6[5] = fused ? 8 : 7; }
  const bool pre = k.splanes != nullptr;
  if (!fused && pc) {
    if (tv.TM == 2) {
      if (k.vec4_epi) x6c_launch<patch_gemm_x6p_kernel<2, 3, false, true>, 512>(k, grid, lds, s);
      else x6c_launch<patch_gemm_x6p_kernel<2, 3>, 512>(k, grid, lds, s);
    } else if (tv.NW == 4) {
      if (pre) x6c_launch<patch_gemm_x6p_kernel<1, 9, false, false, 8, 1, true>, 768>(k, grid, lds, s);
      else x6c_launch<patch_gemm_x6p_kernel<1, 9, false, false, 8, 1>, 768>(k, grid, lds, s);
    } else if (tps == 9) {
      if (pre && x6p_npw() == 8) x6c_launch<patch_gemm_x6p_kernel<1, 9, false, false, 8, 2, true>, 768>(k, grid, lds, s);
      else if (x6p_npw() == 8) x6c_launch<patch_gemm_x6p_kernel<1, 9, false, false, 8>, 768>(k, grid, lds, s);
      else x6c_launch<patch_gemm_x6p_kernel<1, 9>, 512>(k, grid, lds, s);
    } else x6c_launch<patch_gemm_x6p_kernel<1, 3>, 512>(k, grid, lds, s);
  } else if (!fused) {
    if (tv.TM == 2) x6c_launch<patch_gemm_x6c_kernel<8, 2>, 512>(k, grid, lds, s);
    else if (tps == 9) x6c_launch<patch_gemm_x6c_kernel<8, 1, false, 9>, 512>(k, grid, lds, s);
    else x6c_launch<patch_gemm_x6c_kernel<8, 1>, 512>(k, grid, lds, s);
  } else if (pc) x6c_launch<patch_gemm_x6p_kernel<1, 9, true>, 512>(k, grid, lds, s);
  else if (tps == 9) x6c_launch<patch_gemm_x6c_kernel<8, 1, true, 9>, 512>(k, grid, lds, s);
  else x6c_launch<patch_gemm_x6c_kernel<8, 1, true>, 512>(k, grid, lds, s);
}

int run_patch_gemm_x6c(const PatchGeom& g, const ClassSpec& cs, const uint16_t* wb, int ntaps_w, int* plan6, hipStream_t s, bool dry) {
  if (!x6c_on() || (!dry && wb == nullptr) || g.src_y != nullptr || (g.Ck & 15) != 0 || g.Ck < 16) return 1;
  if (cs.mH != 1 || cs.mW != 1 || cs.oH != 1 || cs.oW != 1 || cs.pH || cs.pW) return 1;
  if (cs.ntaps != 9 && cs.ntaps != 18 && cs.ntaps != 27) return 1;
  const int ns = cs.ntaps / 9;
  int lo[3] = {0, 0, 0}, hi[3] = {0, 0, 0};
  for (int i = 0; i < 9; ++i) {
    const int d[3] = {cs.dt[i], cs.dh[i], cs.dw[i]};
    for (int k = 0; k < 3; ++k) {
      if (i == 0 || d[k] < lo[k]) lo[k] = d[k];
      if (i == 0 || d[k] > hi[k]) hi[k] = d[k];
    }
  }
  if (lo[0] != hi[0] || hi[1] - lo[1] != 2 || hi[2] - lo[2] != 2) return 1;
  for (int j = 0; j < ns; ++j)
    for (int i = 0; i < 9; ++i) {
      const int q = 9 * j + i;
      if (cs.dt[q] != cs.dt[9 * j] || cs.dh[q] != cs.dh[i] || cs.dw[q] != cs.dw[i] || cs.tw[q] - cs.tw[i] != cs.tw[9 * j] - cs.tw[0]) return 1;
    }
  const long long n_dst = (long long)g.B * g.Cm * g.dT * g.dH * g.dW;
  const long long nimg = (long long)g.B * cs.nT;
  if (nimg >= (1 << 24)) return 1;
  const bool alias = g.dst == g.res || g.dst == g.mask_y;
  const X6cPick pk = x6c_pick((int)nimg, cs.nH, cs.nW, g.Cm, ns * g.Ck,
                              (n_dst & 3) == 0 && cs.oT == 1 && cs.pT == 0 && cs.nT == g.dT && !alias, g.Ck);
  if (pk.v < 0) return 1;
  const unsigned long long sbytes = 4ull * g.B * g.Ck * g.sT * g.sH * g.sW;
  if (sbytes >= 0x7FFFFFF0ull || 4ull * (unsigned long long)n_dst >= 0x7FFFFFF0ull) return 1;
  if (dry) return 0;
  const X6cVariant& tv = kX6cVariants[pk.v];
  X6cGeom k = x6c_geom(g, &cs, 1, pk, 2, ns, wb, ntaps_w);
  k.bH = lo[1]; k.bW = lo[2];
  for (int i = 0; i < 9; ++i) {
    k.tap_w[i] = cs.tw[i];
    k.tap_off[i] = (cs.dh[i] - lo[1]) * k.eW + (cs.dw[i] - lo[2]);
  }
  k.sdt0 = cs.dt[0]; k.swt0 = 0;
  k.sdt1 = ns > 1 ? cs.dt[9] : 0; k.swt1 = ns > 1 ? cs.tw[9] - cs.tw[0] : 0;
  k.sdt2 = ns > 2 ? cs.dt[18] : 0; k.swt2 = ns > 2 ? cs.tw[18] - cs.tw[0] : 0;
  const int tps = tv.NW == 4 ? 9 : (tv.TM == 1 ? x6c_tps1() : 3);
  const size_t lds = x6c_lds_bytes(k.CSl, tv.TM, tps);
  const int post_act = (pk.ksplit > 1 && g.act_epi != P2I_ACT_NONE) ? g.act_epi : P2I_ACT_NONE;
  if (pk.ksplit > 1) {
    if (p2i::memset_async(g.dst, 0, sizeof(float) * (size_t)n_dst, s) != hipSuccess) return P2I_EINVAL;
    if (post_act != P2I_ACT_NONE) { k.res = nullptr; k.act_epi = P2I_ACT_NONE; }
  }
  if (g_next_splanes != nullptr) {
    if (x6c_pc() && g.Ck >= 32 && tv.TM == 1 && tps == 9 && pk.ksplit == 1) {
      k.splanes = static_cast<const u32x4c*>(g_next_splanes);
      k.plane_units = (unsigned)((long long)g.B * (g.Ck >> 3) * g.sT * g.sH * g.sW);
    }
    g_next_splanes = nullptr;
  }
  {
    const int v4_on = P2I_ENV_ONCE("P2I_X6C_EPI4", 1);
    auto al16 = [](const void* q) { return ((uintptr_t)q & 15) == 0; };
    k.vec4_epi = v4_on && tv.TM == 2 && pk.ksplit == 1 && pk.jw >= 4 && (cs.nW & 3) == 0 && (g.dW & 3) == 0 && al16(g.dst) && al16(k.res) && al16(g.mask_y) &&
                 (32 * 36 * 8 + 4 * tv.TM * 16 * 64) * 4 <= (int)lds - 4 * ((k.CSl + 3) & ~3);
  }
  x6c_dispatch(k, tv, tps, false, plan6, s);
  if (post_act != P2I_ACT_NONE) {
    const long long n4 = n_dst / 4;
    const long long blocks = (n4 + 255) / 256;
    P2I_LAUNCH(x6c_post_act_kernel, dim3((unsigned)(blocks > 2048 ? 2048 : blocks)), dim3(256), 0, s, g.dst, g.res, n4, post_act);
  }
  return launch_status();
}

int run_patch_gemm_x6c_fused(const PatchGeom& g, const ClassSpec* css, int ncls, const uint16_t* wb, int ntaps_w, int* plan6, hipStream_t s, bool dry) {
  if (!x6c_fused_on() || ncls != 4 || (!dry && wb == nullptr) || g.src_y != nullptr || (g.Ck & 15) != 0 || g.Ck < 16) return 1;
  static const int per[4] = {1, 2, 2, 4};
  const int ns = css[0].ntaps;
  if (ns < 1 || ns > 3) return 1;
  for (int q = 0; q < 4; ++q) {
    const ClassSpec& c = css[q];
    if (c.ntaps != ns * per[q] || c.mT != 1 || c.mH != 1 || c.mW != 1 || c.oH != 2 || c.oW != 2 || c.pH != (q >> 1) || c.pW != (q & 1)) return 1;
    if (c.nT != css[0].nT || c.nH != css[0].nH || c.nW != css[0].nW || c.oT != css[0].oT || c.pT != css[0].pT) return 1;
  }
  if ((g.dH & 1) || (g.dW & 1) || css[0].nH * 2 != g.dH || css[0].nW * 2 != g.dW) return 1;
  static const int slot_cls[9] = {3, 3, 3, 3, 2, 2, 1, 1, 0}, slot_idx[9] = {0, 1, 2, 3, 0, 1, 0, 1, 0};
  int sdt[3] = {0, 0, 0}, swt[3] = {0, 0, 0};
  for (int j = 0; j < ns; ++j)
    for (int sl = 0; sl < 9; ++sl) {
      const ClassSpec& c = css[slot_cls[sl]];
      const int i = j * per[slot_cls[sl]] + slot_idx[sl];
      const int i0 = slot_idx[sl];
      if (c.dh[i] < 0 || c.dh[i] > 1 || c.dw[i] < 0 || c.dw[i] > 1) return 1;
      if (c.dh[i] != c.dh[i0] || c.dw[i] != c.dw[i0]) return 1;
      if (sl == 0) { sdt[j] = c.dt[i]; swt[j] = c.tw[i] - c.tw[i0]; }
      else if (c.dt[i] != sdt[j] || c.tw[i] - c.tw[i0] != swt[j]) return 1;
    }
  const ClassSpec& c0 = css[0];
  const long long n_dst = (long long)g.B * g.Cm * g.dT * g.dH * g.dW;
  const long long nimg = (long long)g.B * c0.nT;
  if (nimg >= (1 << 24)) return 1;
  const bool alias = g.dst == g.res || g.dst == g.mask_y;
  const X6cPick pk = x6c_fused_pick((int)nimg, c0.nH, c0.nW, g.Cm, ns * (g.Ck >> 4), !alias && c0.oT == 1 && c0.pT == 0 && c0.nT == g.dT);
  if (pk.v < 0) return 1;
  const unsigned long long sbytes = 4ull * g.B * g.Ck * g.sT * g.sH * g.sW;
  if (sbytes >= 0x7FFFFFF0ull || 4ull * (unsigned long long)n_dst >= 0x7FFFFFF0ull) return 1;
  if (dry) return 0;
  X6cGeom k = x6c_geom(g, css, 4, pk, 1, ns, wb, ntaps_w);
  k.bias = nullptr; k.act_epi = P2I_ACT_NONE;
  k.fused_atomic = pk.ksplit > 1 ? 1 : 0;
  k.sdt0 = sdt[0]; k.sdt1 = sdt[1]; k.sdt2 = sdt[2]; k.swt0 = swt[0]; k.swt1 = swt[1]; k.swt2 = swt[2];
  for (int sl = 0; sl < 9; ++sl) {
    const ClassSpec& c = css[slot_cls[sl]];
    k.tap_w[sl] = c.tw[slot_idx[sl]];
    k.tap_off[sl] = c.dh[slot_idx[sl]] * k.eW + c.dw[slot_idx[sl]];
  }
  if (pk.ksplit > 1 && p2i::memset_async(g.dst, 0, sizeof(float) * (size_t)n_dst, s) != hipSuccess) return P2I_EINVAL;
  x6c_dispatch(k, kX6cVariants[pk.v], x6c_tps1(), true, plan6, s);
  return launch_status();
}

}

extern "C" int p2i_x6_split_batched(const float* const* wp, uint16_t* const* wb, const int* ntaps, const int* K, const int* Mpad, int n,
                                    void* stream) {
  using namespace p2i;
  P2I_REQUIRE(wp && wb && ntaps && K && Mpad && n >= 1 && n <= 24, "p2i_x6_split_batched: 1..24 tensors");
  WsplitBatch b{};
  int maxn = 0;
  for (int i = 0; i < n; ++i) {
    P2I_REQUIRE(wp[i] && wb[i] && ntaps[i] > 0 && K[i] > 0 && (K[i] & 7) == 0 && Mpad[i] > 0 && (Mpad[i] & 31) == 0, "p2i_x6_split_batched: bad tensor %d", i);
    b.wp[i] = wp[i]; b.wb[i] = reinterpret_cast<u32x4c*>(wb[i]); b.ntaps[i] = ntaps[i]; b.Ck[i] = K[i]; b.CmPad[i] = Mpad[i];
    const int tot = ntaps[i] * (K[i] >> 3) * Mpad[i];
    if (tot > maxn) maxn = tot;
  }
  const int blocks = (maxn + 255) / 256;
  P2I_LAUNCH(wsplit_batched_kernel, dim3(blocks > 1024 ? 1024 : blocks, n), dim3(256), 0, (hipStream_t)stream, b);
  return launch_status();
}

extern "C" int p2i_x6_split_planes(const float* x, void* planes, int B, int C, int64_t P, void* stream) {
  P2I_REQUIRE(x && planes && B > 0 && C > 0 && (C & 7) == 0 && P > 0, "split planes: C % 8 == 0");
  const long long total = (long long)B * (C >> 3) * P;
  const long long blocks = (total + 255) / 256;
  P2I_LAUNCH(p2i::split_planes_kernel, dim3((unsigned)(blocks > 8192 ? 8192 : blocks)), dim3(256), 0, (hipStream_t)stream, x,
             static_cast<p2i::u32x4c*>(planes), B, C >> 3, (long long)P);
  return p2i::launch_status();
}
extern "C" int p2i_x6_next_source_planes(const void* planes) {
  p2i::g_next_splanes = planes;
  return P2I_OK;
}
```

p2i-gan-benchmark_amd/p2igan_bench/_hip.py:

```python
from __future__ import annotations

import ctypes as C
import os

_LIB_PATH = os.path.join(os.path.dirname(os.path.abspath(__file__)), "_lib", "libp2i_hip.so")
_lib = None

ACT_NONE, ACT_RELU, ACT_LEAKY, ACT_TANH = 0, 1, 2, 3


class ConvDesc(C.Structure):
    _fields_ = [(n, C.c_int) for n in
                ("B", "Cin", "Cout", "Ti", "Hi", "Wi", "To", "Ho", "Wo", "kt", "kh", "kw",
                 "st", "sh", "sw", "pt", "ph", "pw")]


_P = C.c_void_p
_I = C.c_int
_F = C.c_float
_L = C.c_int64
_F64 = C.c_double
_D = C.POINTER(ConvDesc)

SIGNATURES = {
    "p2i_conv_fwd": [_D, _P, _P, _P, _P, _P, _I, _P],
    "p2i_conv_dgrad": [_D, _P, _P, _I, _P, _P, _P, _I, _P, _P],
    "p2i_conv_wgrad": [_D, _P, _P, _P, _I, _P, _P, _P],
    "p2i_conv_wgrad_ws": [_D, _P, _P, _P, _I, _P, _P, _P, _L, _P],
    "p2i_conv_fwd_x6": [_D, _P, _P, _P, _P, _P, _P, _I, _P],
    "p2i_conv_dgrad_x6": [_D, _P, _P, _P, _P, _P, _I, _P, _P],
    "p2i_x6_split": [_P, _P, _I, _I, _I, _P],
    "p2i_x6_split_batched": [_P, _P, _P, _P, _P, _I, _P],
    "p2i_x6c_would_take": [_D, _I, _I],
    "p2i_conv_fwd_x6s": [_D, _P, _P, _P, _I, _P, _P, _P, _I, _P],
    "p2i_conv_dgrad_x6s": [_D, _P, _P, _P, _I, _P, _P, _I, _P, _P],
    "p2i_conv_last_plan": [C.POINTER(C.c_int)],
    "p2i_wgrad_last_plan": [C.POINTER(C.c_int)],
    "p2i_fast_div_magic": [_I, C.POINTER(C.c_uint32)],
    "p2i_doconv_fold_fwd": [_P, _P, _P, _I, _I, _I, _I, _I, _P, _P, _P],
    "p2i_doconv_fold_bwd": [_P, _P, _P, _P, _I, _I, _I, _I, _P, _P, _P],
    "p2i_doconv_fold_fwd_batched": [_P, _P, _P, _I, _I, _I, _P, _P, _P],
    "p2i_doconv_fold_bwd_batched": [_P, _P, _P, _P, _I, _I, _I, _P, _P, _P],
    "p2i_weight_pack": [_P, _I, _I, _I, _P, _P, _P, _P],
    "p2i_weight_pack_batched": [_P, _P, _P, _P, _P, _P, _P, _I, _P],
    "p2i_weight_unpack_grad_batched": [_P, _P, _P, _P, _P, _P, _P, _P, _P, _P, _I, _P],
    "p2i_weight_unpack_grad_batched_acc": [_P, _P, _P, _P, _P, _P, _P, _P, _P, _P, _I, _I, _P],
    "p2i_weight_unpack_grad": [_P, _I, _I, _I, _P, _P, _P, _P, _P, _P, _P],
    "p2i_spectral_norm": [_P, _I, _I, _P, _P, _I, _P, _P, _P],
    "p2i_spectral_norm_batched": [_P, _P, _P, _P, _P, _I, _P, _P, _P, _P, _I, _P],
    "p2i_attn_fwd": [_P, _P, _P, _P, _P, _P, _I, _I, _I, _P],
    "p2i_attn_bwd": [_P, _P, _P, _P, _P, _P, _P, _P, _P, _P, _I, _I, _I, _P],
    "p2i_idw_fwd": [_P, _P, _P, _P, _P, _P, _P, _P, _P, _P, _P, _P, _P, _I, _I, _I, _I, _F, _P],
    "p2i_idw_fwd_ws": [_P, _P, _P, _P, _P, _P, _P, _P, _P, _P, _P, _P, _P, _P, _I, _I, _I, _I, _F, _P],
    "p2i_idw_bwd": [_P, _P, _P, _P, _P, _P, _I, _I, _I, _I, _P],
    "p2i_pooldup_fwd": [_P, _P, _I, _I, _I, _I, _P],
    "p2i_pooldup_bwd": [_P, _P, _P, _I, _I, _I, _I, _P],
    "p2i_upmod_fwd": [_P, _P, _P, _I, _I, _I, _I, _P],
    "p2i_window_gather": [_P, _P, _P, _P, _I, _L, _I, _I, _I, _I, _P],
    "p2i_window_mean": [_P, _P, _I, _L, _I, _I, _I, _F, _P],
    "p2i_upmod_fwd_ba": [_P, _P, _P, _I, _P, _I, _I, _I, _I, _P],
    "p2i_upmod_bwd": [_P, _P, _P, _P, _P, _I, _I, _I, _I, _P],
    "p2i_dtail_fwd": [_P, _P, _P, _P, _I, _I, _I, _I, _I, _I, _P],
    "p2i_dtail_bwd": [_P, _P, _P, _P, _P, _P, _I, _I, _I, _I, _I, _I, _P],
    "p2i_recloss": [_P, _P, _F, _P, _P, _P, _I, _I, _I, _P],
    "p2i_gan_loss": [_P, _P, _I, _I, _I, _F, _F, _F, _P, _P, _P, _P],
    "p2i_loss_transform_fwd": [_P, _P, _L, _P],
    "p2i_loss_transform_bwd": [_P, _P, _P, _L, _P],
    "p2i_fdiff_fwd": [_P, _P, _I, _I, _L, _P],
    "p2i_fdiff_bwd": [_P, _P, _I, _I, _L, _P],
    "p2i_wl1_fwd": [_P, _P, _P, _L, _P],
    "p2i_wl1_bwd": [_P, _P, _P, _P, _L, _P],
    "p2i_softmax_t_fwd": [_P, _P, _I, _I, _F, _P],
    "p2i_softmax_t_bwd": [_P, _P, _P, _I, _I, _F, _P],
    "p2i_kl_fwd": [_P, _P, _P, _L, _I, _P],
    "p2i_kl_bwd": [_P, _P, _P, _P, _L, _I, _P],
    "p2i_spool_fwd": [_P, _P, _P, _I, _I, _I, _P],
    "p2i_spool_bwd": [_P, _P, _P, _P, _I, _I, _I, _P],
    "p2i_tdm_fwd": [_P, _P, _P, _F, _F, _P, _P, _P, _I, _I, _I, _I, _P],
    "p2i_shock_map_fwd": [_P, _P, _I, _I, _I, _F, _F, _P],
    "p2i_shock_map_bwd": [_P, _P, _P, _P, _I, _I, _I, _F, _F, _P],
    "p2i_shock_loss_fwd": [_P, _P, _P, _I, _I, _I, _I, _I, _F, _F, _P],
    "p2i_shock_loss_bwd": [_P, _P, _P, _P, _P, _I, _I, _I, _I, _I, _F, _F, _P],
    "p2i_adam": [_P, _P, _P, _P, _L, _F, _F, _F, _F, _I, _P],
    "p2i_adam_dev": [_P, _P, _P, _P, _L, _F, _F, _F, _F, _P, _P, _P],
    "p2i_metrics_pointwise": [_P, _P, _L, C.POINTER(C.c_float), _I, _I, _P, _P, _P, _P],
    "p2i_metrics_fss": [_P, _I, _I, _I, _I, C.POINTER(C.c_int), _I, _P, _P, _P],
    "p2i_assemble_batch": [_P, _P, _L, _P, _P, _P, _I, _I, _I, _I, _P],
    "p2i_axpy": [_P, _P, _F, _L, _P],
    "p2i_add2": [_P, _P, _P, _L, _P],
    "p2i_zero": [_P, _L, _P],
    "p2i_act_bwd": [_P, _P, _I, _P, _L, _P],
    "p2i_bias_grad": [_P, _P, _I, _P, _I, _I, _L, _P],
    "p2i_act_bwd_bias": [_P, _P, _I, _P, _P, _I, _I, _L, _P],
    "p2i_det_workspace": [_P, _L, _P, _I],
    "p2i_x6_split_planes": [_P, _P, _I, _I, _L, _P],
    "p2i_x6_next_source_planes": [_P],
    "p2i_event_record": [_I, _P],
    "p2i_event_wait": [_I, _P],
    "p2i_tape_begin": [_P],
    "p2i_tape_end": [C.POINTER(C.c_void_p)],
    "p2i_tape_info": [_P, C.POINTER(C.c_int)],
    "p2i_tape_replay": [_P, _P],
    "p2i_tape_free": [_P],
    "p2i_stdk_basis": [_P, _P, _I, _I, _I, _P, _P],
    "p2i_stdk_select": [_P, _P, _I, _I, _I, _P, _P, _P],
    "p2i_stdk_layer1_fwd": [_P, _P, _P, _P, _P, _I, _I, _I, _I, _I, _I, _P, _P, _P, _P, _P],
    "p2i_stdk_mlp_fwd": [_P, _P, _P, _P, _P, _P, _P, _P, _I, _I, _P, _P],
    "p2i_stdk_bwd_workspace": [_I, _I, C.POINTER(C.c_int64)],
    "p2i_stdk_mlp_bwd": [_P] * 8 + [_I, _I] + [_P] * 13,
    "p2i_stdk_layer1_bwd": [_P, _P, _P, _P, _P, _I, _I, _I, _I, _I, _I, _P, _P, _P, _I, _P, _P, _P],
    "p2i_exp1_transform": [_P, _I, _L, _I, _P, _P],
    "p2i_exp1_workspace": [_I, _I, _I, C.POINTER(C.c_int64)],
    "p2i_exp1_accumulate": [_P, _I, _I, _I, _I, _I, _P, _I, _I, _I, _I, _I, _I, _I, _I, _P, _I, _P,
                            C.POINTER(C.c_double), _I, _I, _P, _P, _P, _P, _P, _P],
    "p2i_exp1_merge": [_P, _L, _P, _P],
    "p2i_exp1_hist": [_P, _P, _I, _I, _P, _P, _P, _P, _P],
    "p2i_exp1_ssim": [_P, _P, _I, _I, _P, _P, _P, _P],
    "p2i_exp1_finalize": [_P, C.POINTER(C.c_double), _I, _I, _P, _P, _P, _P, _P, _P, _P, _P],
# ... 89 lines not shown
```

p2i-gan-benchmark_amd/p2igan_bench/models/p2igan.py:

```python
from __future__ import annotations

import math
import os
from typing import List

import torch
import torch.nn as nn
from torch.nn import init

from .. import ops
from ..ops import ACT_LEAKY, ACT_NONE, ACT_RELU, ACT_TANH, ConvSpec

BASE_CH = 64
SUPPORTED_T = (8, 16, 32)


class _DOConvParams(nn.Module):

    def __init__(self, in_ch: int, out_ch: int, ksz: int, groups: int = 1, folded: bool = False):
        super().__init__()
        self.in_ch, self.out_ch, self.ksz, self.groups, self.folded = in_ch, out_ch, ksz, groups, folded
        mn = ksz * ksz
        if folded:
            self.W = nn.Parameter(torch.empty(out_ch, in_ch // groups, ksz, ksz))
# ... 83 lines not shown
        self.Convsin = nn.ModuleList([_basic_conv(length, base, 3, groups=4, folded=inference)])
        if init_weights:
            self.init_weights()
        self._pnames = [n for n, _ in self.named_parameters()]
        self._wp_cache = {}
        self._weights_epoch = 0
        self.debug_taps = None

    def invalidate_weight_cache(self):
        self._weights_epoch += 1

    def _cached(self, key, tensors, make):
        ver = (self._weights_epoch,) + tuple((t._version, t.data_ptr()) for t in tensors if t is not None)
        hit = self._wp_cache.get(key)
        if hit is not None and hit[0] == ver:
            return hit[1]
        val = make()
        self._wp_cache[key] = (ver, val)
        return val

    def init_weights(self, init_type: str = "kaiming", gain: float = 0.02):
        if init_type != "kaiming":
            raise NotImplementedError(init_type)
        for m in [l.conv for l in self.input.layers] + [u.proj for u in self.UP]:
            init.kaiming_normal_(m.weight.data, a=0, mode="fan_in")
            init.constant_(m.bias.data, 0.0)

    def _arena_numel(self) -> int:
        if not hasattr(self, "_arena_n"):
            n = 0
            for lvl in range(4):
                ch = self.base << lvl
                n += 2 * self.num_res * 9 * ch * ops.pad32(ch)
            for up in self.UP:
                co, ci = up.proj.weight.shape[0], up.proj.weight.shape[1]
                n += ci * ops.pad32(co) + co + 8
            n += 9 * self.length * ops.pad32(self.base) + self.base * ops.pad32(self.length) + 64
            self._arena_n = n
        return self._arena_n

    def forward(self, masked_frames, masks):
        params = [p for _, p in self.named_parameters()]
        self._grad_on = torch.is_grad_enabled()
        return _GeneratorFn.apply(self, masked_frames, masks, *params)


def _doconv_of(holder):
    return holder.main[0]


import os as _os

SIDE_WGRAD = _os.environ.get("P2I_SIDE_WGRAD", "1") != "0"
LATE_JOIN = _os.environ.get("P2I_LATE_JOIN", "1") != "0"


def _side_of(net, device):
    if not SIDE_WGRAD:
        return None
    if ops.side_depth() > 0 and _os.environ.get("P2I_NESTED_SIDE", "0") != "1":
        return None
    sd = getattr(net, "_side", None)
    if sd is None or sd.stream.device != device:
        sd = net._side = ops.SideStream(device)
    return sd


def _grad_target(prm, inplace):
    return prm.grad if inplace else None


def generator_prepare(net: "P2IGenerator", b: int, h: int, w: int):
    t, BASE_CH = net.length, net.base
    prep = {"folded": {}, "up": {}}
    cin = _doconv_of(net.Convsin[0])
    prep["wp_in"] = ops.doconv_fold(*cin.tensors(), BASE_CH, t, 4, 3, identity_rep=4, need_d=True)
    for lvl in (3, 2, 1, 0):
        ch = BASE_CH << lvl
        convs = [_doconv_of(m) for rb in net.Decoder[lvl].layers for m in (rb.main[0], rb.main[1])]
        wps = ops.doconv_fold_batched([cv.tensors() for cv in convs], ch, ch, need_d=True)
        for cv, wp in zip(convs, wps):
            prep["folded"][id(cv)] = wp
        d = _spec2d(ch, ch, 3).desc(b, 1, h >> lvl, w >> lvl)
        ops._x6s_of(wps[0][0], d, False, ACT_RELU)
        ops._x6s_of(wps[0][1], d, True)
    for i in (2, 1, 0):
        up = net.UP[i]
        cin_, cout_ = up.proj.weight.shape[1], up.proj.weight.shape[0]
        prep["up"][i] = ops.weight_pack(up.proj.weight.reshape(cout_, cin_, 1), need_d=True)
    cout = _doconv_of(net.ConvsOut[0])
    prep["wp_out"] = ops.doconv_fold(*cout.tensors(), t, BASE_CH, 4, 1, need_d=True)
    return prep


def generator_forward(net: "P2IGenerator", masked_frames, masks, need_grad: bool, prep=None, weights_ready=None, after_head=None):
    b, t, c, h, w = masked_frames.shape
    BASE_CH = net.base
    if c != 1 or t != net.length:
        raise RuntimeError(f"generator expects (B,{net.length},1,H,W), got {tuple(masked_frames.shape)}")
    if h % 8 or w % 8:
        raise RuntimeError("H and W must be multiples of 8")
    if need_grad and net.inference:
        raise RuntimeError("P2IGenerator(inference=True) holds folded DO-Conv kernels and is forward-only")

    def fold(conv, out_ch, in_ch, groups, ksz, identity_rep=0):
        make = lambda: ops.doconv_fold(*conv.tensors(), out_ch, in_ch, groups, ksz, identity_rep=identity_rep, need_d=need_grad)
        return make() if need_grad else net._cached(id(conv), conv.tensors(), make)

    x0 = masked_frames.reshape(b, t, h, w).contiguous().float()
    mk = masks.reshape(b, t, h, w).contiguous().float()
    att = [l.conv for l in net.input.layers]
    a = ops.attn_fwd(x0, att[0].weight, att[0].bias, att[1].weight, att[1].bias)
    idw, sel = ops.idw_fwd(a, mk, tau=0.05, save=need_grad)
    del a
    if after_head is not None:
        late = after_head()
        if late is not None:
            prep, weights_ready = late
    if weights_ready is not None:
        weights_ready()
    cin = _doconv_of(net.Convsin[0])
    wp_in = prep["wp_in"] if prep is not None else fold(cin, BASE_CH, t, 4, 3, identity_rep=4)
    spec_in = _spec2d(t, BASE_CH, 3)
    x_ = ops.conv_fwd(spec_in, idw, wp_in[0])
    x_2 = ops.pooldup_fwd(x_)
    x_4 = ops.pooldup_fwd(x_2)
    x_8 = ops.pooldup_fwd(x_4)

    def eblock(lvl, hcur):
        ch = BASE_CH << lvl
        spec = _spec2d(ch, ch, 3)
        rec = []
        folded = prep["folded"] if prep is not None else {}
        if need_grad and prep is None:
            convs = [_doconv_of(m) for rb in net.Decoder[lvl].layers for m in (rb.main[0], rb.main[1])]
            for cv, wp in zip(convs, ops.doconv_fold_batched([cv.tensors() for cv in convs], ch, ch, need_d=True)):
                folded[id(cv)] = wp
        for rb in net.Decoder[lvl].layers:
            c1, c2 = _doconv_of(rb.main[0]), _doconv_of(rb.main[1])
            w1 = folded[id(c1)] if need_grad else fold(c1, ch, ch, 1, 3)
            w2 = folded[id(c2)] if need_grad else fold(c2, ch, ch, 1, 3)
            y1 = ops.conv_fwd(spec, hcur, w1[0], act=ACT_RELU)
            hn = ops.conv_fwd(spec, y1, w2[0], residual=hcur)
            rec.append((hcur, y1, w1[1], w2[1]))
            hcur = hn
        return hcur, rec

    def uppos(i, hcur):
        up = net.UP[i]
        cin_, cout_ = up.proj.weight.shape[1], up.proj.weight.shape[0]
        pack = lambda: ops.weight_pack(up.proj.weight.reshape(cout_, cin_, 1), need_d=need_grad)
        wp = prep["up"][i] if prep is not None else (pack() if need_grad else net._cached(id(up), (up.proj.weight,), pack))
        v = ops.conv_fwd(_spec2d(cin_, cout_, 1), hcur, wp[0])
        r = ops.upmod_fwd(v, up.pos, bias=up.proj.bias, act=ACT_RELU)
        return r, (hcur, v, r, wp[1])

    h3, rec3 = eblock(3, x_8)
    res1, up2 = uppos(2, h3)
    x4s = ops.add2(x_4, res1)
    h2, rec2 = eblock(2, x4s)
    res2, up1 = uppos(1, h2)
    h1, rec1 = eblock(1, res2)
    res3, up0 = uppos(0, h1)
    h0, rec0 = eblock(0, res3)
    cout = _doconv_of(net.ConvsOut[0])
    wp_out = prep["wp_out"] if prep is not None else fold(cout, t, BASE_CH, 4, 1)
    spec_out = _spec2d(BASE_CH, t, 1)
    z = ops.conv_fwd(spec_out, h0, wp_out[0], act=ACT_TANH)
    if net.debug_taps is not None:
        net.debug_taps.update(idw=idw, x_=x_, x_8=x_8, dec3=h3, res1=res1, res3=res3)
    S = None
    if need_grad:
        S = dict(x0=x0, idw=idw, sel=sel, wp_in_d=wp_in[1], x_=x_, x_2=x_2, x_4=x_4,
                 rec=[rec0, rec1, rec2, rec3], up=[up0, up1, up2], h0=h0, z=z, wp_out_d=wp_out[1], shape=(b, t, h, w))
    return z.view(b, t, c, h, w), S


def generator_backward(net: "P2IGenerator", S, dout, inplace: bool = False, on_level_done=None):
    b, t, h, w = S["shape"]
    BASE_CH = net.base
    grads = {}
    if inplace:
        plist = getattr(net, "_plist", None)
        if plist is None:
            plist = net._plist = [p_ for p_ in net.parameters() if p_.requires_grad]
        if any(p_.grad is None or not p_.grad.is_contiguous() for p_ in plist):
            raise RuntimeError("generator_backward(inplace=True) needs contiguous .grad views on every trainable parameter")
    if inplace and (getattr(net, "_arena_buf", None) is None or net._arena_buf.numel() < net._arena_numel() or net._arena_buf.device != dout.device):
        net._arena_buf = torch.empty(net._arena_numel(), device=dout.device, dtype=torch.float32)
    arena = ops.ZeroArena(net._arena_numel(), dout.device, buf=net._arena_buf if inplace else None)
    side = _side_of(net, dout.device) if inplace else None

    def wgrad(spec, x, dy, **kw):
        if side is None:
            return ops.conv_wgrad(spec, x, dy, arena=arena, **kw)
        tgt = arena.take(spec.wp_f_shape())
        return side.run(lambda: ops.conv_wgrad(spec, x, dy, dwp_out=tgt, **kw), x, dy)

    late = side is not None and LATE_JOIN

    def weight_side(fn):
        if late:
            return side.run(fn)
        if side is not None:
            side.join()
        return fn()

    dz = dout.reshape(b, t, h, w).contiguous().float()
    spec_out = _spec2d(BASE_CH, t, 1)
    cout = _doconv_of(net.ConvsOut[0])
    dz = ops.act_bwd(dz, S["z"], ACT_TANH)
    dwp, _ = wgrad(spec_out, S["h0"], dz)
    gw, _ = weight_side(lambda: ops.doconv_fold_bwd(dwp, *cout.tensors(), t, BASE_CH, 4, 1, out=(cout.W.grad, None) if inplace else None))
    if not inplace:
        grads[id(cout.W)] = gw
    dh = ops.conv_dgrad(spec_out, dz, S["wp_out_d"], tuple(S["h0"].shape))

    def eblock_bwd(lvl, dh):
        ch = BASE_CH << lvl
        spec = _spec2d(ch, ch, 3)
        blocks = net.Decoder[lvl].layers
        pend = []
        for rb, (hin, y1, w1d, w2d) in zip(reversed(list(blocks)), reversed(S["rec"][lvl])):
            c1, c2 = _doconv_of(rb.main[0]), _doconv_of(rb.main[1])
            dwp2, _ = wgrad(spec, y1, dh)
            pend.append((dwp2, c2))
            dy1 = ops.conv_dgrad(spec, dh, w2d, tuple(y1.shape), mask_y=y1, mask_act=ACT_RELU)
            dwp1, _ = wgrad(spec, hin, dy1)
            pend.append((dwp1, c1))
            dh = ops.conv_dgrad(spec, dy1, w1d, tuple(hin.shape), add=dh)
        outs = ([cv.W.grad for _, cv in pend], [cv.D.grad for _, cv in pend]) if inplace else None

        def fold_level():
            r_ = ops.doconv_fold_bwd_batched([g_ for g_, _ in pend], [cv.tensors() for _, cv in pend], ch, ch, outs=outs)
            if inplace and on_level_done is not None:
                on_level_done(lvl)
            return r_

        dWs, dDs = weight_side(fold_level)
        if not inplace:
            for (_, cv), dW_, dD_ in zip(pend, dWs, dDs):
                grads[id(cv.W)], grads[id(cv.D)] = dW_, dD_
        return dh

    def uppos_bwd(i, dr):
        up = net.UP[i]
        hin, v, r, wpd = S["up"][i]
        cin_, cout_ = up.proj.weight.shape[1], up.proj.weight.shape[0]
        spec = _spec2d(cin_, cout_, 1)
        dz, db = ops.act_bwd_bias(dr, r, ACT_RELU, db_out=_grad_target(up.proj.bias, inplace))
        dv, dpos = ops.upmod_bwd(v, up.pos, dz, dpos_out=_grad_target(up.pos, inplace))
        dwp, _ = wgrad(spec, hin, dv)
        gw_ = weight_side(lambda: ops.weight_unpack_grad(dwp, up.proj.weight.reshape(cout_, cin_, 1), out=_grad_target(up.proj.weight, inplace)))
        dx = ops.conv_dgrad(spec, dv, wpd, tuple(hin.shape))
        if not inplace:
            grads[id(up.proj.weight)] = gw_.reshape(up.proj.weight.shape)
            grads[id(up.proj.bias)] = db
            grads[id(up.pos)] = dpos
        return dx

    dh = eblock_bwd(0, dh)
    dh = uppos_bwd(0, dh)
    dh = eblock_bwd(1, dh)
    dh = uppos_bwd(1, dh)
    dx4s = eblock_bwd(2, dh)
    dh = uppos_bwd(2, dx4s)
    dx8 = eblock_bwd(3, dh)
    dx4 = ops.axpy_(ops.pooldup_bwd(S["x_4"], dx8), dx4s)
    dx2 = ops.pooldup_bwd(S["x_2"], dx4)
    dx_ = ops.pooldup_bwd(S["x_"], dx2)
    spec_in = _spec2d(t, BASE_CH, 3)
    cin = _doconv_of(net.Convsin[0])
    dwp, _ = wgrad(spec_in, S["idw"], dx_)
    gW, gD = weight_side(lambda: ops.doconv_fold_bwd(dwp, *cin.tensors(), BASE_CH, t, 4, 3, out=(cin.W.grad, cin.D.grad) if inplace else None))
    if not inplace:
        grads[id(cin.W)], grads[id(cin.D)] = gW, gD
    didw = ops.conv_dgrad(spec_in, dx_, S["wp_in_d"], tuple(S["idw"].shape))
    da = ops.idw_bwd(didw, S["sel"])
    att = [l.conv for l in net.input.layers]
    prm4 = (att[0].weight, att[0].bias, att[1].weight, att[1].bias)
    g = ops.attn_bwd(S["x0"], *prm4, da, out=[p_.grad for p_ in prm4] if inplace else None)
    if not inplace:
        for prm, gr in zip(prm4, g):
            grads[id(prm)] = gr.reshape(prm.shape)
    if side is not None:
        side.join()
    return grads


class _GeneratorFn(torch.autograd.Function):

    @staticmethod
    def forward(ctx, net: P2IGenerator, masked_frames, masks, *params):
        need_grad = net._grad_on and any(ctx.needs_input_grad[3:])
        z, S = generator_forward(net, masked_frames, masks, need_grad)
        if need_grad:
            ctx.net, ctx.S = net, S
        return z

    @staticmethod
    def backward(ctx, dout):
        net, S = ctx.net, ctx.S
        grads = generator_backward(net, S, dout, inplace=False)
        out = []
        for (name, prm), need in zip(net.named_parameters(), ctx.needs_input_grad[3:]):
            out.append(grads.get(id(prm)) if need else None)
        ctx.S = None
        return (None, None, None, *out)


def fold_generator_state_dict(sd):
    out = {}
    for k, v in sd.items():
# ... 252 lines not shown
```

p2i-gan-benchmark_amd/p2igan_bench/ops.py:

```python
from __future__ import annotations

import ctypes as C
import math
from dataclasses import dataclass
from typing import Optional, Tuple

import torch

from . import _hip
from ._hip import ACT_LEAKY, ACT_NONE, ACT_RELU, ACT_TANH, ConvDesc


def _ptr(t: Optional[torch.Tensor]):
    return None if t is None else t.data_ptr()


_CUR_STREAM = None


def _stream():
    return _CUR_STREAM if _CUR_STREAM is not None else torch.cuda.current_stream().cuda_stream


class step_stream:

    def __enter__(self):
        global _CUR_STREAM
        self.prev = _CUR_STREAM
        _CUR_STREAM = torch.cuda.current_stream().cuda_stream
        return self

    def __exit__(self, *exc):
        global _CUR_STREAM
        _CUR_STREAM = self.prev
        return False


def _chk(*ts):
    for t in ts:
        if t is None:
            continue
        if not (t.is_cuda and t.is_contiguous()):
            raise RuntimeError("p2i ops need contiguous CUDA tensors (the HIP path has no CPU fallback)")
        if t.dtype not in (torch.float32, torch.int32, torch.uint8, torch.int16):
            raise RuntimeError(f"unsupported dtype {t.dtype}")


class KernelProfile:

    def __init__(self):
        self.records = []

    def summary(self):
        torch.cuda.synchronize()
        agg = {}
        for key, flops, e0, e1 in self.records:
            a = agg.setdefault(key, [0, 0.0, 0.0])
            a[0] += 1
            a[1] += e0.elapsed_time(e1) * 1e-3
            a[2] += flops
        return {k: {"launches": v[0], "seconds": v[1], "flops": v[2]} for k, v in agg.items()}


PROFILE: Optional[KernelProfile] = None


def _prof_begin():
    if PROFILE is None:
        return None
    e = torch.cuda.Event(enable_timing=True)
    e.record()
    return e


def _prof_end(e0, kind, spec, desc, stride1):
    if e0 is None:
        return
    e1 = torch.cuda.Event(enable_timing=True)
    e1.record()
    flops = 2.0 * desc.B * desc.Cout * desc.Cin * spec.ntaps * desc.To * desc.Ho * desc.Wo
    if kind == "wgrad":
        import ctypes
        wp = (ctypes.c_int * 4)()
        _hip.load().p2i_wgrad_last_plan(wp)
        key = {0: "wgrad_kernel<64>", 2: "c1_wgrad_kernel<32>", 3: "wgrad_x6_kernel (bf16-split x6)"}.get(wp[0]) or \
            "wgrad_dma_kernel<64, %d, %s, %d>%s" % (wp[1], "true" if wp[2] else "false", wp[3], "" if spec.k[0] == 1 else " (x%d kt slices)" % spec.k[0])
    else:
        import ctypes
        plan = (ctypes.c_int * 6)()
        _hip.load().p2i_conv_last_plan(plan)
        if plan[5] > 10:
            key = "patch_gemm_fused_kernel<%d, %d, %d, %d, %d> (strided dgrad, %d parity classes per workgroup)" % (plan[0], plan[1], plan[2], plan[3], plan[5] - 10, plan[5] - 10)
        elif plan[5] == 7 and plan[3] == 4:
            key = "patch_gemm_x6p_kernel<%d, %d, false> (%d x %d tile, %d taps per stage, producer / consumer waves, bf16-split x6)" % (
                plan[0] // 32, plan[4], plan[0], plan[1], plan[4])
        elif plan[5] == 7:
            key = "patch_gemm_x6c_kernel<%d, %d, false, %d> (%d x %d tile, %d taps per stage, bf16-split x6)" % (
                plan[1] // 32, plan[0] // 32, plan[4], plan[0], plan[1], plan[4])
        elif plan[5] == 3:
            key = "o1_fwd_kernel (single output channel, bandwidth-bound)"
        elif plan[5] == 4:
            key = "c1_dgrad_kernel (single input channel, %d taps)" % plan[4]
        elif plan[5] == 8 and plan[3] == 4:
            key = "patch_gemm_x6p_kernel<1, %d, true> (strided dgrad, 4 parity classes per workgroup, producer / consumer waves, bf16-split x6)" % plan[4]
        elif plan[5] == 8:
            key = "patch_gemm_x6c_kernel<8, 1, true, %d> (strided dgrad, 4 parity classes per workgroup, bf16-split x6)" % plan[4]
        else:
            key = "patch_gemm_dma_kernel<%d, %d, %d, %d, %d, %d>" % tuple(plan)
    PROFILE.records.append((key, flops, e0, e1))


import os as _os

CONV_ENGINE = _os.environ.get("P2I_CONV_ENGINE", "auto")
_X6_SCRATCH = {}


def _x6_scratch(numel: int, device):
    if CONV_ENGINE not in ("auto", "x6"):
        return None
    key = (device.index, _stream())
    buf = _X6_SCRATCH.get(key)
    if buf is None or buf.numel() < numel:
        buf = torch.empty(max(numel, 1 << 22), device=device, dtype=torch.int16)
        _X6_SCRATCH[key] = buf
    return buf


class X6Stack:

    def __init__(self, wstack):
        self.w = wstack
        self.wb = None
        self.n, self.taps, self.k, self.mpad = wstack.shape

    def layer_ptr(self, i):
        if self.wb is None:
            self.wb = torch.empty(3 * self.w.numel(), device=self.w.device, dtype=torch.int16)
            _hip.check(_hip.load().p2i_x6_split(_ptr(self.w), _ptr(self.wb), self.n * self.taps, self.k, self.mpad, _stream()), "p2i_x6_split")
        return self.wb.data_ptr() + 2 * i * self.taps * self.k * self.mpad

    @staticmethod
    def attach(wstack, views):
        if CONV_ENGINE in ("auto", "x6") and wstack is not None and wstack.shape[2] % 16 == 0 and wstack.shape[3] % 32 == 0:
            st = X6Stack(wstack)
            for i, v in enumerate(views):
                v._x6s = (st, i)


class _X6One:

    def __init__(self, ptr, taps):
        self.ptr, self.n, self.taps = ptr, 1, taps

    def layer_ptr(self, i):
        return self.ptr


def x6_presplit(tensors, wants, buf=None):
    if CONV_ENGINE not in ("auto", "x6"):
        return buf
    sel = [t for t, w in zip(tensors, wants) if w and t is not None and t.shape[1] % 16 == 0]
    if not sel:
        return buf
    import ctypes
    need = sum(3 * t.numel() for t in sel)
    if buf is None or buf.numel() < need:
        buf = torch.empty(need, device=sel[0].device, dtype=torch.int16)
    n = len(sel)
    ptrs, off = [], 0
    for t in sel:
        ptrs.append(buf.data_ptr() + 2 * off)
        off += 3 * t.numel()
    arr_i = ctypes.c_int * n
    _hip.check(_hip.load().p2i_x6_split_batched(_ptr_array(sel), (ctypes.c_void_p * n)(*ptrs), arr_i(*[t.shape[0] for t in sel]),
                                                arr_i(*[t.shape[1] for t in sel]), arr_i(*[t.shape[2] for t in sel]), n, _stream()),
               "p2i_x6_split_batched")
    for t, p_ in zip(sel, ptrs):
        t._x6s = (_X6One(p_, t.shape[0]), 0)
        t._x6buf = buf
    return buf


def _x6s_of(wp, d, dgrad, act=ACT_NONE):
    h = getattr(wp, "_x6s", None)
    if h is None or CONV_ENGINE not in ("auto", "x6") or not _hip.load().p2i_x6c_would_take(d, 1 if dgrad else 0, act):
        return None
    st, i = h
    return st.layer_ptr(i), st.n * st.taps


WGRAD_SLICES = _os.environ.get("P2I_WGRAD_SLICES", "1") != "0"
_WGRAD_WS = {}


def _wgrad_scratch(device):
    if not WGRAD_SLICES:
        return None
    key = (device.index, _stream())
    buf = _WGRAD_WS.get(key)
    if buf is None:
        buf = torch.empty(256 * (9 * 64 * 64 + 512) + 1024, device=device, dtype=torch.float32)
        _WGRAD_WS[key] = buf
    return buf


_SIDE_DEPTH = 0


def side_depth() -> int:
    return _SIDE_DEPTH


class SideStream:

    def __init__(self, device):
        self.stream = torch.cuda.Stream(device)
        self.keep = []
        self.pending = False

    def run(self, fn, *tensors, after=None):
        if after is None:
            fork(_stream(), self.stream.cuda_stream)
        else:
            _hip.check(_hip.load().p2i_event_wait(after, self.stream.cuda_stream), "p2i_event_wait")
        global _CUR_STREAM, _SIDE_DEPTH
        prev, _CUR_STREAM = _CUR_STREAM, self.stream.cuda_stream
        _SIDE_DEPTH += 1
        try:
            with torch.cuda.stream(self.stream):
                out = fn()
        finally:
            _CUR_STREAM = prev
            _SIDE_DEPTH -= 1
        self.keep.extend(tensors)
        self.pending = True
        return out

    def mark(self):
        slot = _next_slot()
        _hip.check(_hip.load().p2i_event_record(slot, self.stream.cuda_stream), "p2i_event_record")
        return lambda: _hip.check(_hip.load().p2i_event_wait(slot, _stream()), "p2i_event_wait")

    def join(self):
        if self.pending:
            fork(self.stream.cuda_stream, _stream())
            self.pending = False
        self.keep.clear()


_SLOT = 0


def _next_slot() -> int:
    global _SLOT
    _SLOT = (_SLOT + 1) % 256
    return _SLOT


def mark_stream() -> int:
    slot = _next_slot()
    _hip.check(_hip.load().p2i_event_record(slot, _stream()), "p2i_event_record")
    return slot


def fork(src_stream: int, dst_stream: int):
    lib = _hip.load()
    slot = _next_slot()
    _hip.check(lib.p2i_event_record(slot, src_stream), "p2i_event_record")
    _hip.check(lib.p2i_event_wait(slot, dst_stream), "p2i_event_wait")


_DET = {}


def det_ready(device):
    key = device.index if device.index is not None else torch.cuda.current_device()
    if key in _DET:
        return
    if _os.environ.get("P2I_DETERMINISTIC", "1") == "0":
        _DET[key] = None
        return
    mb = int(_os.environ.get("P2I_DET_SCRATCH_MB", "128"))
    part = torch.empty(mb << 18, device=device, dtype=torch.float32)
    cnt = torch.zeros(8192, device=device, dtype=torch.int32)
    torch.cuda.current_stream(device).synchronize()
    _hip.check(_hip.load().p2i_det_workspace(part.data_ptr(), part.numel(), cnt.data_ptr(), cnt.numel()), "p2i_det_workspace")
    _DET[key] = (part, cnt)


def pad32(n: int) -> int:
    return (n + 31) // 32 * 32


@dataclass(frozen=True)
class ConvSpec:
    cin: int
    cout: int
    k: Tuple[int, int, int]
    stride: Tuple[int, int, int] = (1, 1, 1)
    pad: Tuple[int, int, int] = (0, 0, 0)

    @property
    def ntaps(self) -> int:
        return self.k[0] * self.k[1] * self.k[2]

    def out_dims(self, t, h, w):
        return tuple((d + 2 * p - k) // s + 1 for d, p, k, s in zip((t, h, w), self.pad, self.k, self.stride))

    def desc(self, b, t, h, w) -> ConvDesc:
        return _conv_desc(self, b, t, h, w)

    def wp_f_shape(self):
        return (self.ntaps, self.cin, pad32(self.cout))

    def wp_d_shape(self):
        return (self.ntaps, self.cout, pad32(self.cin))


import functools


@functools.lru_cache(maxsize=512)
def _conv_desc(spec: ConvSpec, b, t, h, w) -> ConvDesc:
    to, ho, wo = spec.out_dims(t, h, w)
    return ConvDesc(b, spec.cin, spec.cout, t, h, w, to, ho, wo, *spec.k, *spec.stride, *spec.pad)


def _dims5(x: torch.Tensor):
    if x.dim() == 4:
        b, c, h, w = x.shape
        return b, c, 1, h, w
    b, c, t, h, w = x.shape
    return b, c, t, h, w


def conv_fwd(spec: ConvSpec, x, wp_f, bias=None, residual=None, act=ACT_NONE, out=None):
    lib = _hip.load()
    b, c, t, h, w = _dims5(x)
    if c != spec.cin or tuple(wp_f.shape) != spec.wp_f_shape():
        raise RuntimeError(f"conv_fwd: shape mismatch x={tuple(x.shape)} wp={tuple(wp_f.shape)} spec={spec}")
    to, ho, wo = spec.out_dims(t, h, w)
    oshape = (b, spec.cout, ho, wo) if x.dim() == 4 else (b, spec.cout, to, ho, wo)
    y = out if out is not None else torch.empty(oshape, device=x.device, dtype=torch.float32)
    if tuple(y.shape) != oshape or (residual is not None and tuple(residual.shape) != oshape):
        raise RuntimeError("conv_fwd: output/residual shape mismatch")
    if bias is not None and bias.numel() != spec.cout:
        raise RuntimeError("conv_fwd: bias size mismatch")
    _chk(x, wp_f, bias, residual, y)
    d = spec.desc(b, t, h, w)
    e0 = _prof_begin()
    pre = _x6s_of(wp_f, d, False, act)
    ws = _x6_scratch(3 * wp_f.numel(), x.device) if (pre is None and spec.cin % 16 == 0) else None
    if pre is not None:
        _hip.check(lib.p2i_conv_fwd_x6s(d, _ptr(x), _ptr(wp_f), pre[0], pre[1], _ptr(bias), _ptr(residual), _ptr(y), act, _stream()),
                   "p2i_conv_fwd_x6s")
    elif ws is not None:
        _hip.check(lib.p2i_conv_fwd_x6(d, _ptr(x), _ptr(wp_f), _ptr(ws), _ptr(bias), _ptr(residual), _ptr(y), act, _stream()),
                   "p2i_conv_fwd_x6")
    else:
        _hip.check(lib.p2i_conv_fwd(d, _ptr(x), _ptr(wp_f), _ptr(bias), _ptr(residual), _ptr(y), act, _stream()), "p2i_conv_fwd")
    _prof_end(e0, "fwd", spec, d, True)
    return y


def conv_dgrad(spec: ConvSpec, dy, wp_d, in_shape, y_act=None, act=ACT_NONE, add=None, mask_y=None, mask_act=ACT_NONE):
    lib = _hip.load()
    if len(in_shape) == 4:
        b, c, h, w = in_shape
        t = 1
    else:
        b, c, t, h, w = in_shape
    to, ho, wo = spec.out_dims(t, h, w)
    eshape = (b, spec.cout, ho, wo) if len(in_shape) == 4 else (b, spec.cout, to, ho, wo)
    if tuple(dy.shape) != eshape or c != spec.cin or tuple(wp_d.shape) != spec.wp_d_shape():
        raise RuntimeError(f"conv_dgrad: shape mismatch dy={tuple(dy.shape)} expected {eshape}")
    if y_act is not None and y_act.shape != dy.shape:
        raise RuntimeError("conv_dgrad: y_act shape mismatch")
    if add is not None and tuple(add.shape) != tuple(in_shape):
        raise RuntimeError("conv_dgrad: add shape mismatch")
    if mask_y is not None and tuple(mask_y.shape) != tuple(in_shape):
        raise RuntimeError("conv_dgrad: mask_y shape mismatch")
    dx = torch.empty(in_shape, device=dy.device, dtype=torch.float32)
    _chk(dy, wp_d, y_act, dx, add, mask_y)
    d = spec.desc(b, t, h, w)
    e0 = _prof_begin()
    pre = _x6s_of(wp_d, d, True) if y_act is None else None
    ws = _x6_scratch(3 * wp_d.numel(), dy.device) if (pre is None and y_act is None and spec.cout % 16 == 0 and spec.cin > 1) else None
    if pre is not None:
        _hip.check(lib.p2i_conv_dgrad_x6s(d, _ptr(dy), _ptr(wp_d), pre[0], pre[1], _ptr(add), _ptr(mask_y), mask_act, _ptr(dx), _stream()),
                   "p2i_conv_dgrad_x6s")
    elif ws is not None:
        _hip.check(lib.p2i_conv_dgrad_x6(d, _ptr(dy), _ptr(wp_d), _ptr(ws), _ptr(add), _ptr(mask_y), mask_act, _ptr(dx), _stream()),
                   "p2i_conv_dgrad_x6")
    else:
        _hip.check(lib.p2i_conv_dgrad(d, _ptr(dy), _ptr(y_act), act, _ptr(wp_d), _ptr(add), _ptr(mask_y), mask_act, _ptr(dx), _stream()),
                   "p2i_conv_dgrad")
    _prof_end(e0, "dgrad", spec, d, spec.stride == (1, 1, 1))
    return dx


class ZeroArena:

    def __init__(self, numel: int, device, buf: Optional[torch.Tensor] = None):
        if buf is not None and buf.numel() >= numel:
            self.buf = buf
            zero_(buf[:numel])
        else:
            self.buf = torch.zeros(numel, device=device, dtype=torch.float32)
        self.off = 0

    def take(self, shape):
        n = 1
        for d in shape:
            n *= d
        n4 = (n + 3) // 4 * 4
        if self.off + n4 > self.buf.numel():
            return zero_(torch.empty(shape, device=self.buf.device, dtype=torch.float32))
        t = self.buf[self.off:self.off + n].view(shape)
        self.off += n4
        return t


def conv_wgrad(spec: ConvSpec, x, dy, y_act=None, act=ACT_NONE, want_bias=False, arena: Optional["ZeroArena"] = None, db_out=None,
               dwp_out=None):
    lib = _hip.load()
    det_ready(x.device)
    b, c, t, h, w = _dims5(x)
    to, ho, wo = spec.out_dims(t, h, w)
    eshape = (b, spec.cout, ho, wo) if x.dim() == 4 else (b, spec.cout, to, ho, wo)
    if tuple(dy.shape) != eshape or c != spec.cin:
        raise RuntimeError(f"conv_wgrad: shape mismatch dy={tuple(dy.shape)} expected {eshape}")
    if y_act is not None and y_act.shape != dy.shape:
        raise RuntimeError("conv_wgrad: y_act shape mismatch")
    if db_out is not None and (tuple(db_out.shape) != (spec.cout,) or not want_bias):
        raise RuntimeError("conv_wgrad: db_out must be (cout,) and want_bias set")
    if dwp_out is not None:
        if tuple(dwp_out.shape) != spec.wp_f_shape() or (want_bias and db_out is None):
            raise RuntimeError("conv_wgrad: dwp_out shape mismatch (and a bias gradient needs db_out with it)")
        dwp, db = dwp_out, db_out
    elif arena is not None:
        dwp = arena.take(spec.wp_f_shape())
        db = db_out if db_out is not None else (arena.take((spec.cout,)) if want_bias else None)
    else:
        dwp = zero_(torch.empty(spec.wp_f_shape(), device=x.device, dtype=torch.float32))
        db = db_out if db_out is not None else (zero_(torch.empty(spec.cout, device=x.device, dtype=torch.float32)) if want_bias else None)
    _chk(x, dy, y_act, dwp, db)
    d = spec.desc(b, t, h, w)
    e0 = _prof_begin()
    ws = _wgrad_scratch(x.device)
    if ws is not None:
        _hip.check(lib.p2i_conv_wgrad_ws(d, _ptr(x), _ptr(dy), _ptr(y_act), act, _ptr(dwp), _ptr(db), _ptr(ws), ws.numel(), _stream()),
                   "p2i_conv_wgrad_ws")
    else:
        _hip.check(lib.p2i_conv_wgrad(d, _ptr(x), _ptr(dy), _ptr(y_act), act, _ptr(dwp), _ptr(db), _stream()), "p2i_conv_wgrad")
    _prof_end(e0, "wgrad", spec, d, True)
    return dwp, db


def doconv_fold(W, D, D_diag, out_ch, in_ch, groups, ksz, identity_rep=0, need_d=True):
    lib = _hip.load()
    nt = ksz * ksz
    exp_w = (out_ch, in_ch // groups, nt)
    if tuple(W.shape) != exp_w:
        raise RuntimeError(f"doconv_fold: W shape {tuple(W.shape)} != {exp_w}")
    if ksz == 3 and (tuple(D.shape) != (in_ch, 9, 9) or tuple(D_diag.shape) != (in_ch, 9, 9)):
        raise RuntimeError("doconv_fold: D/D_diag shape mismatch")
    wp_f = torch.empty((nt, in_ch, pad32(out_ch)), device=W.device, dtype=torch.float32)
    wp_d = torch.empty((nt, out_ch, pad32(in_ch)), device=W.device, dtype=torch.float32) if need_d else None
# ... 1823 lines not shown
```

Measured before the change: 11450.

## Add scaled fp16 two-term split path for decoder 3x3 convs

```diff
diff --git a/include/p2i_hip.h b/include/p2i_hip.h
--- a/include/p2i_hip.h
+++ b/include/p2i_hip.h
@@ -48,6 +48,15 @@
                      const float* bias, const float* residual, float* y, int act, void* stream);
 int p2i_conv_dgrad_x6s(const p2i_conv_desc* d, const float* dy, const float* wp_d, const uint16_t* wb_layer, int ntaps_w,
                        const float* dx_add, const float* mask_y, int mask_act, float* dx, void* stream);
+int p2i_absmax_partials(const float* x, int64_t n, uint32_t* part, int* count, void* stream);
+int p2i_x6h_split(const float* wp, uint16_t* wh, int32_t* kexp, uint32_t* part, int n, int taps, int K, int Mpad, void* stream);
+int p2i_x6h_would_take(const p2i_conv_desc* d, int dgrad);
+int p2i_conv_fwd_x6h(const p2i_conv_desc* d, const float* x, const float* wp, const uint16_t* wb_layer, const uint16_t* wh_layer,
+                     const int32_t* w_kexp, int ntaps_w, const uint32_t* src_part, int src_count, uint32_t* dst_part, int* dst_count,
+                     const float* bias, const float* residual, float* y, int act, void* stream);
+int p2i_conv_dgrad_x6h(const p2i_conv_desc* d, const float* dy, const float* wp_d, const uint16_t* wb_layer, const uint16_t* wh_layer,
+                       const int32_t* w_kexp, int ntaps_w, const uint32_t* src_part, int src_count, uint32_t* dst_part, int* dst_count,
+                       const float* dx_add, const float* mask_y, int mask_act, float* dx, void* stream);
 int p2i_conv_last_plan(int* out6);
 int p2i_fast_div_magic(int d, uint32_t* magic);
 int p2i_wgrad_last_plan(int* out4);
diff --git a/p2i-gan-benchmark_amd/csrc/conv.hip b/p2i-gan-benchmark_amd/csrc/conv.hip
--- a/p2i-gan-benchmark_amd/csrc/conv.hip
+++ b/p2i-gan-benchmark_amd/csrc/conv.hip
@@ -187,7 +187,7 @@
 
 static int run_patch_gemm_classes(PatchGeom g, const ClassSpec* css, int ncls, hipStream_t s) {
   if (g.src_y != nullptr || ncls > MAX_CLASSES) return 1;
-  if (const X6Ctx& xc = x6_ctx(); xc.wb != nullptr) {
+  if (const X6Ctx& xc = x6_ctx(); xc.wb != nullptr || xc.wh != nullptr) {
     bool all = true;
     for (int q = 0; q < ncls && all; ++q) all = run_patch_gemm_x6c(g, css[q], xc.wb, xc.ntaps_w, nullptr, s, true) == 0;
     if (all) {
@@ -578,3 +578,36 @@
   x6_ctx() = X6Ctx{nullptr, 0};
   return rc;
 }
+
+extern "C" int p2i_x6h_would_take(const p2i_conv_desc* d, int dgrad) {
+  if (check_desc(d)) return 0;
+  return x6h_would_take(d, dgrad != 0) ? 1 : 0;
+}
+
+extern "C" int p2i_conv_fwd_x6h(const p2i_conv_desc* d, const float* x, const float* wp, const uint16_t* wb_layer, const uint16_t* wh_layer,
+                                const int32_t* w_kexp, int ntaps_w, const uint32_t* src_part, int src_count, uint32_t* dst_part, int* dst_count,
+                                const float* bias, const float* residual, float* y, int act, void* stream) {
+  if (int e = check_desc(d)) return e;
+  if (dst_count) *dst_count = 0;
+  if (wh_layer == nullptr || w_kexp == nullptr || src_part == nullptr || src_count < 1 || !x6h_would_take(d, false))
+    return p2i_conv_fwd_x6s(d, x, wp, wb_layer, ntaps_w, bias, residual, y, act, stream);
+  P2I_REQUIRE(ntaps_w >= d->kt * d->kh * d->kw, "ntaps_w smaller than the layer's tap count");
+  x6_ctx() = X6Ctx{wb_layer, ntaps_w, wh_layer, w_kexp, src_part, src_count, dst_part, dst_count};
+  const int rc = p2i_conv_fwd(d, x, wp, bias, residual, y, act, stream);
+  x6_ctx() = X6Ctx{nullptr, 0};
+  return rc;
+}
+
+extern "C" int p2i_conv_dgrad_x6h(const p2i_conv_desc* d, const float* dy, const float* wp_d, const uint16_t* wb_layer, const uint16_t* wh_layer,
+                                  const int32_t* w_kexp, int ntaps_w, const uint32_t* src_part, int src_count, uint32_t* dst_part, int* dst_count,
+                                  const float* dx_add, const float* mask_y, int mask_act, float* dx, void* stream) {
+  if (int e = check_desc(d)) return e;
+  if (dst_count) *dst_count = 0;
+  if (wh_layer == nullptr || w_kexp == nullptr || src_part == nullptr || src_count < 1 || !x6h_would_take(d, true))
+    return p2i_conv_dgrad_x6s(d, dy, wp_d, wb_layer, ntaps_w, dx_add, mask_y, mask_act, dx, stream);
+  P2I_REQUIRE(ntaps_w >= d->kt * d->kh * d->kw, "ntaps_w smaller than the layer's tap count");
+  x6_ctx() = X6Ctx{wb_layer, ntaps_w, wh_layer, w_kexp, src_part, src_count, dst_part, dst_count};
+  const int rc = p2i_conv_dgrad(d, dy, nullptr, P2I_ACT_NONE, wp_d, dx_add, mask_y, mask_act, dx, stream);
+  x6_ctx() = X6Ctx{nullptr, 0};
+  return rc;
+}
diff --git a/p2i-gan-benchmark_amd/csrc/conv_common.h b/p2i-gan-benchmark_amd/csrc/conv_common.h
--- a/p2i-gan-benchmark_amd/csrc/conv_common.h
+++ b/p2i-gan-benchmark_amd/csrc/conv_common.h
@@ -165,7 +165,8 @@
   }
 }
 __device__ __forceinline__ void epi_tile16_v4_finish(const EpiOps4v& b, const f32x16& acc, float* __restrict__ tile_lds, int lane, int act_epi, const float* __restrict__ res,
-                                                     const float* __restrict__ mask_y, int mask_act, float* __restrict__ dst, bool atomic_out) {
+                                                     const float* __restrict__ mask_y, int mask_act, float* __restrict__ dst, bool atomic_out,
+                                                     unsigned* __restrict__ amax = nullptr) {
   constexpr int PITCH = 36;
   const int l31 = lane & 31, lhi = lane >> 5;
 #pragma unroll
@@ -191,6 +192,13 @@
         for (int e = 0; e < 4; ++e) atomicAdd(dst + b.di[k] + e, v[k][e]);
       } else {
         *reinterpret_cast<f32x4e*>(dst + b.di[k]) = v[k];
+      }
+      if (amax) {
+#pragma unroll
+        for (int e = 0; e < 4; ++e) {
+          const unsigned a = __float_as_uint(v[k][e]) & 0x7FFFFFFFu;
+          *amax = a > *amax ? a : *amax;
+        }
       }
     }
   }
@@ -366,12 +374,16 @@
   int dt[MAX_TAPS], dh[MAX_TAPS], dw[MAX_TAPS];
 };
 
-struct X6Ctx { const uint16_t* wb; int ntaps_w; };
+struct X6Ctx {
+  const uint16_t* wb; int ntaps_w;
+  const uint16_t* wh; const int* w_kexp; const uint32_t* src_part; int src_count; uint32_t* dst_part; int* dst_count;
+};
 X6Ctx& x6_ctx();
 
 int run_patch_gemm_x6c(const PatchGeom& g, const ClassSpec& cs, const uint16_t* wb, int ntaps_w, int* plan6, hipStream_t s, bool dry = false);
 int run_patch_gemm_x6c_fused(const PatchGeom& g, const ClassSpec* css, int ncls, const uint16_t* wb, int ntaps_w, int* plan6, hipStream_t s, bool dry = false);
 bool x6c_would_take(const p2i_conv_desc* d, bool dgrad, int act_epi);
+bool x6h_would_take(const p2i_conv_desc* d, bool dgrad);
 
 int run_patch_gemm_fused(PatchGeom g, const ClassSpec* css, int ncls, int* plan6, hipStream_t s);
 
diff --git a/p2i-gan-benchmark_amd/csrc/conv_x6c.hip b/p2i-gan-benchmark_amd/csrc/conv_x6c.hip
--- a/p2i-gan-benchmark_amd/csrc/conv_x6c.hip
+++ b/p2i-gan-benchmark_amd/csrc/conv_x6c.hip
@@ -76,6 +76,112 @@
     const long long pix = i % P, r = i / P;
     const float* px = x + (r * 8) * P + pix;
     split8_store(px, P, planes, total, i);
+  }
+}
+
+typedef _Float16 f16x8c __attribute__((ext_vector_type(8)));
+typedef _Float16 f16x2c __attribute__((ext_vector_type(2)));
+constexpr int X6H_MAX_PART = 1024;
+
+__host__ __device__ __forceinline__ int x6h_scale_exp(unsigned amax_bits) {
+  if (amax_bits == 0u || amax_bits >= 0x7F800000u) return 0;
+  const int k = 13 - ((int)(amax_bits >> 23) - 127);
+  return k < -60 ? -60 : (k > 60 ? 60 : k);
+}
+__device__ __forceinline__ float x6h_pow2(int k) { return __uint_as_float((unsigned)(k + 127) << 23); }
+
+__device__ __forceinline__ unsigned wave_max_u32(unsigned v) {
+#pragma unroll
+  for (int o = 32; o > 0; o >>= 1) {
+    const unsigned w = (unsigned)__shfl_xor((int)v, o, 64);
+    v = w > v ? w : v;
+  }
+  return v;
+}
+
+__device__ __forceinline__ unsigned x6h_reduce_partials(const unsigned* __restrict__ part, int count, int lane) {
+  unsigned v[X6H_MAX_PART / 64];
+#pragma unroll
+  for (int j = 0; j < X6H_MAX_PART / 64; ++j) {
+    const int i = lane + 64 * j;
+    v[j] = part[i < count ? i : count - 1];
+  }
+  unsigned m = 0u;
+#pragma unroll
+  for (int j = 0; j < X6H_MAX_PART / 64; ++j) m = v[j] > m ? v[j] : m;
+  return wave_max_u32(m);
+}
+
+__device__ __forceinline__ void split8h(const float (&v)[8], float s, u32x4c& hi, u32x4c& lo) {
+#pragma unroll
+  for (int j = 0; j < 4; ++j) {
+    const float a = v[2 * j] * s, b = v[2 * j + 1] * s;
+    const f16x2c h = {(_Float16)a, (_Float16)b};
+    const f16x2c l = {(_Float16)(a - (float)h[0]), (_Float16)(b - (float)h[1])};
+    hi[j] = __builtin_bit_cast(unsigned, h);
+    lo[j] = __builtin_bit_cast(unsigned, l);
+  }
+}
+
+__global__ __launch_bounds__(256) void absmax_partials_kernel(const float* __restrict__ x, long long n, unsigned* __restrict__ part) {
+  __shared__ unsigned sm[4];
+  const long long n4 = n >> 2;
+  unsigned m = 0u;
+  for (long long i = blockIdx.x * 256ll + threadIdx.x; i < n4; i += (long long)gridDim.x * 256) {
+    const u32x4c v = reinterpret_cast<const u32x4c*>(x)[i];
+#pragma unroll
+    for (int e = 0; e < 4; ++e) { const unsigned a = v[e] & 0x7FFFFFFFu; m = a > m ? a : m; }
+  }
+  if (blockIdx.x == 0 && threadIdx.x < (unsigned)(n & 3)) {
+    const unsigned a = __float_as_uint(x[(n4 << 2) + threadIdx.x]) & 0x7FFFFFFFu;
+    m = a > m ? a : m;
+  }
+  m = wave_max_u32(m);
+  if ((threadIdx.x & 63) == 0) sm[threadIdx.x >> 6] = m;
+  __syncthreads();
+  if (threadIdx.x == 0) {
+    for (int w = 1; w < 4; ++w) m = sm[w] > m ? sm[w] : m;
+    part[blockIdx.x] = m;
+  }
+}
+
+__global__ __launch_bounds__(256) void wabsmax_kernel(const float* __restrict__ wp, long long per_layer, unsigned* __restrict__ part) {
+  __shared__ unsigned sm[4];
+  const float* w = wp + (size_t)blockIdx.y * per_layer;
+  unsigned m = 0u;
+  for (long long i = blockIdx.x * 256ll + threadIdx.x; i < per_layer; i += (long long)gridDim.x * 256) {
+    const unsigned a = __float_as_uint(w[i]) & 0x7FFFFFFFu;
+    m = a > m ? a : m;
+  }
+  m = wave_max_u32(m);
+  if ((threadIdx.x & 63) == 0) sm[threadIdx.x >> 6] = m;
+  __syncthreads();
+  if (threadIdx.x == 0) {
+    for (int q = 1; q < 4; ++q) m = sm[q] > m ? sm[q] : m;
+    part[blockIdx.y * gridDim.x + blockIdx.x] = m;
+  }
+}
+__global__ __launch_bounds__(256) void wsplit_f16_kernel(const float* __restrict__ wp, u32x4c* __restrict__ wh, int* __restrict__ kexp,
+                                                         const unsigned* __restrict__ part, int nparts, int nlayers, int ntaps, int Ck, int CmPad) {
+  const int L = blockIdx.y;
+  const int k = x6h_scale_exp(x6h_reduce_partials(part + (size_t)L * nparts, nparts, threadIdx.x & 63));
+  if (blockIdx.x == 0 && threadIdx.x == 0) kexp[L] = k;
+  const float s = x6h_pow2(k);
+  const int KCt = Ck >> 3;
+  const int per = ntaps * KCt * CmPad;
+  const int total = nlayers * per;
+  for (int i = blockIdx.x * 256 + threadIdx.x; i < per; i += gridDim.x * 256) {
+    const int m = i % CmPad;
+    const int r = i / CmPad;
+    const int kc = r % KCt, tap = r / KCt;
+    const float* p = wp + (((size_t)L * ntaps + tap) * Ck + kc * 8) * CmPad + m;
+    float v[8];
+#pragma unroll
+    for (int q = 0; q < 8; ++q) v[q] = p[(size_t)q * CmPad];
+    u32x4c h, lo;
+    split8h(v, s, h, lo);
+    wh[(size_t)L * per + i] = h;
+    wh[(size_t)total + (size_t)L * per + i] = lo;
   }
 }
 
@@ -109,6 +215,10 @@
   const u32x4c* splanes;
   unsigned plane_units;
   int cons_prio;
+  const unsigned* src_part;
+  int src_count;
+  const int* w_kexp;
+  unsigned* dst_part;
 };
 
 __device__ constexpr int X6C_CLS[9] = {3, 3, 3, 3, 2, 2, 1, 1, 0};
@@ -437,22 +547,24 @@
 }
 
 
-template <int TM, int TPS, bool FUSED = false, bool EPI4 = false, int NPW = 4, int TN = 2, bool PRE = false>
+template <int TM, int TPS, bool FUSED = false, bool EPI4 = false, int NPW = 4, int TN = 2, bool PRE = false, bool F16 = false>
 __global__ __launch_bounds__(64 * (4 + NPW)) void patch_gemm_x6p_kernel(const X6cGeom g) {
   constexpr int NSTG = 9 / TPS;
   constexpr int NCLS = FUSED ? 4 : 1;
   static_assert(TPS == 3 || TPS == 9, "taps per stage");
+  static_assert(!F16 || (EPI4 && !FUSED && !PRE && TN == 2), "the fp16 two-term format exists for the 16-byte-epilogue tile only");
+  constexpr int NPLN = F16 ? 2 : 3, NPROD = F16 ? 3 : 6;
   extern __shared__ __attribute__((aligned(16))) float smem[];
   constexpr int MB = 32 * TM, NCW = 4, NTHR = 64 * (NCW + NPW), NPT = 64 * NPW;
   constexpr int NI = (2 * (TN == 2 ? X6cTile<8>::MAXCSL : X6cTile<4>::MAXCSL) + NPT - 1) / NPT;
   constexpr int RING = TPS == 9 ? 3 : (TM == 2 ? 4 : 6), LEAD = RING - 1;
-  constexpr int WST = 6 * TPS * MB, NWI = WST / 64;
+  constexpr int WST = 2 * NPLN * TPS * MB, NWI = WST / 64;
   const int CSl = g.CSl;
   int* ptab = reinterpret_cast<int*>(smem);
   const int ptab_sz = (CSl + 3) & ~3;
   u32x4c* wbuf = reinterpret_cast<u32x4c*>(smem + ptab_sz);
   u32x4c* planes = wbuf + RING * WST;
-  const int PST = 6 * CSl;
+  const int PST = 2 * NPLN * CSl;
 
   const int tid = threadIdx.x, lane = tid & 63, wave = __builtin_amdgcn_readfirstlane(tid >> 6);
   const int l31 = lane & 31, lhi = lane >> 5;
@@ -473,6 +585,11 @@
   const int nch = (g.ns * cps) / g.ksplit;
   const int nst = NSTG * nch;
 
+  int kx = 0;
+  if constexpr (F16) {
+    kx = __builtin_amdgcn_readfirstlane(x6h_scale_exp(x6h_reduce_partials(g.src_part, g.src_count, lane)));
+    __builtin_amdgcn_sched_barrier(0);
+  }
   for (int e = tid; e < CSl; e += NTHR) {
     const int row = fast_div(e, g.mg_ew);
     const int ew = e - row * g.eW;
@@ -509,6 +626,7 @@
     float pv[PRE ? 1 : NI][8];
     u32x4c pq[PRE ? NI : 1][3];
     bool pok[NI];
+    [[maybe_unused]] const float src_scale = x6h_pow2(kx);
     auto load_patch = [&](int c) {
       if constexpr (PRE) {
         const int cg = c0 + c;
@@ -582,11 +700,18 @@
         float v[8];
 #pragma unroll
         for (int q = 0; q < 8; ++q) v[q] = pok[it] ? pv[it][q] : 0.f;
+        if constexpr (F16) {
+          u32x4c h, lo;
+          split8h(v, src_scale, h, lo);
+          pb[it_dst[it]] = h;
+          pb[2 * CSl + it_dst[it]] = lo;
+        } else {
         u32x4c h, mi, lo;
         split8c(v, h, mi, lo);
         pb[it_dst[it]] = h;
         pb[2 * CSl + it_dst[it]] = mi;
         pb[4 * CSl + it_dst[it]] = lo;
+        }
       }
       }
     };
@@ -713,14 +838,14 @@
       for (int nb = 0; nb < TN; ++nb)
 #pragma unroll
         for (int r = 0; r < 16; ++r) acc[q][i][nb][r] = 0.f;
-  constexpr int PA[6] = {2, 0, 1, 1, 0, 0};
-  constexpr int PB[6] = {0, 2, 1, 0, 1, 0};
-  u32x4c A[3][TM][3], Bv[3][TN][3];
+  constexpr int PA[6] = {F16 ? 1 : 2, 0, F16 ? 0 : 1, 1, 0, 0};
+  constexpr int PB[6] = {0, F16 ? 1 : 2, F16 ? 0 : 1, 0, 1, 0};
+  u32x4c A[3][TM][NPLN], Bv[3][TN][NPLN];
   auto load_tap = [&](const u32x4c* wsl, const u32x4c* pbuf, int tap, int buf) {
     const int tl = tap % TPS;
     const int to = toff[tap];
 #pragma unroll
-    for (int p = 0; p < 3; ++p) {
+    for (int p = 0; p < NPLN; ++p) {
 #pragma unroll
       for (int i = 0; i < TM; ++i) A[buf][i][p] = wsl[((p * TPS + tl) * 2) * MB + 32 * i];
 #pragma unroll
@@ -730,16 +855,20 @@
   auto mfma_tap = [&](int buf, int slot) {
     const int cl = FUSED ? X6C_CLS[slot] : 0;
 #pragma unroll
-    for (int q = 0; q < 6; ++q)
+    for (int q = 0; q < NPROD; ++q)
 #pragma unroll
       for (int i = 0; i < TM; ++i)
 #pragma unroll
         for (int nb = 0; nb < TN; ++nb)
+          if constexpr (F16)
+            acc[cl][i][nb] = __builtin_amdgcn_mfma_f32_32x32x16_f16(__builtin_bit_cast(f16x8c, A[buf][i][PA[q]]), __builtin_bit_cast(f16x8c, Bv[buf][nb][PB[q]]),
+                                                                    acc[cl][i][nb], 0, 0, 0);
+          else
           acc[cl][i][nb] = __builtin_amdgcn_mfma_f32_32x32x16_bf16(__builtin_bit_cast(bf16x8c, A[buf][i][PA[q]]), __builtin_bit_cast(bf16x8c, Bv[buf][nb][PB[q]]),
                                                                    acc[cl][i][nb], 0, 0, 0);
   };
   auto ilv = [&]() {
-    constexpr int NR = 3 * TM + 3 * TN, NM = 6 * TM * TN;
+    constexpr int NR = NPLN * TM + NPLN * TN, NM = NPROD * TM * TN;
 #pragma unroll
     for (int i = 0; i < NM; ++i) {
       __builtin_amdgcn_sched_group_barrier(0x008, 1, 0);
@@ -749,7 +878,7 @@
   const int dHW = g.dT * g.dH * g.dW;
   const int mynb = (TN == 2 && producer) ? 1 : 0;
   const bool has_epi = wave < 2 * NCW;
-  const bool split = FUSED ? g.fused_atomic != 0 : g.ksplit > 1;
+  const bool split = !F16 && (FUSED ? g.fused_atomic != 0 : g.ksplit > 1);
   const float* const bias_q = (split && blockIdx.z) ? nullptr : g.bias;
   const float* const res_q = (split && blockIdx.z) ? nullptr : g.res;
   const bool blk1 = TN == 2 && producer;
@@ -844,6 +973,17 @@
   if (!producer && g.cons_prio) __builtin_amdgcn_s_setprio(0);
   if (TN == 1 && producer) return;
   if (has_epi && !(EARLY_C && !producer)) fetch(0, 0);
+  if constexpr (F16) {
+    if (!producer) {
+      const float dsc = x6h_pow2(-(kx + __builtin_amdgcn_readfirstlane(*g.w_kexp)));
+#pragma unroll
+      for (int i = 0; i < TM; ++i)
+#pragma unroll
+        for (int nb = 0; nb < TN; ++nb)
+#pragma unroll
+          for (int r = 0; r < 16; ++r) acc[0][i][nb][r] *= dsc;
+    }
+  }
   if constexpr (TN == 2) {
     if (!producer) {
 #pragma unroll
@@ -875,6 +1015,24 @@
   } else if constexpr (EPI4) {
     if (split) epilogue_pipelined<TM>(fetch, [&](int slot, int k) {
       epi_tile16_v4_finish(ops_v[slot], acc[0][k][0], tl, lane, P2I_ACT_NONE, res_q, g.mask_y, g.mask_act, g.dst, true); }, true);
+    else if constexpr (F16) {
+      unsigned amax = 0u;
+      epilogue_pipelined<TM>(fetch, [&](int slot, int k) {
+        epi_tile16_v4_finish(ops_v[slot], acc[0][k][0], tl, lane, g.act_epi, g.res, g.mask_y, g.mask_act, g.dst, false, &amax); }, true);
+      if (g.dst_part != nullptr) {
+        amax = wave_max_u32(amax);
+        if (lane == 0) reinterpret_cast<unsigned*>(tl)[0] = amax;
+        __syncthreads();
+        if (tid == 0) {
+          unsigned m = 0u;
+          for (int w = 0; w < 2 * NCW; ++w) {
+            const unsigned v = reinterpret_cast<const unsigned*>(xch + 4 * NCLS * TM * 16 * 64 + w * (32 * 36))[0];
+            m = v > m ? v : m;
+          }
+          g.dst_part[blockIdx.y * gridDim.x + blockIdx.x] = m;
+        }
+      }
+    }
     else epilogue_pipelined<TM>(fetch, [&](int slot, int k) {
       epi_tile16_v4_finish(ops_v[slot], acc[0][k][0], tl, lane, g.act_epi, g.res, g.mask_y, g.mask_act, g.dst, false); }, true);
   } else {
@@ -906,6 +1064,7 @@
 static int x6c_pc() { return env_int("P2I_X6C_PC", 1); }
 static int x6c_tps1() { return env_int("P2I_X6C_TPS", 9) == 3 ? 3 : 9; }
 static int x6p_prio() { return env_int("P2I_X6P_PRIO", 0); }
+static bool x6p_f16_on() { return env_int("P2I_X6P_F16", 0) != 0; }
 
 struct X6cVariant { int NW, TM; };
 static const X6cVariant kX6cVariants[] = {{8, 2}, {8, 1}, {4, 1}};
@@ -973,6 +1132,22 @@
   return x6c_pick(d->B * nT, nH, nW, Cm, ns * Ck, whole, Ck).v >= 0;
 }
 
+static size_t x6c_lds_bytes(int csl, int tm, int tps, int planes = 3) {
+  const int ring = tps == 9 ? 3 : (tm == 2 ? 4 : 6);
+  return sizeof(float) * (size_t)((csl + 3) & ~3) + 16 * (size_t)(ring * 2 * planes * tps * 32 * tm + 2 * 2 * planes * csl);
+}
+
+bool x6h_would_take(const p2i_conv_desc* d, bool dgrad) {
+  if (!x6p_f16_on() || !x6c_on() || !x6c_pc() || !P2I_ENV_ONCE("P2I_X6C_EPI4", 1)) return false;
+  if (d->kh != 3 || d->kw != 3 || d->sh != 1 || d->sw != 1 || d->ph != 1 || d->pw != 1 || d->kt != 1 || d->st != 1 || d->pt != 0) return false;
+  const int Ck = dgrad ? d->Cout : d->Cin, Cm = dgrad ? d->Cin : d->Cout;
+  const int nH = dgrad ? d->Hi : d->Ho, nW = dgrad ? d->Wi : d->Wo, nT = dgrad ? d->Ti : d->To;
+  if ((Ck & 15) != 0 || Ck < 32 || nT < 1 || (nW & 3) != 0) return false;
+  const X6cPick pk = x6c_pick(d->B * nT, nH, nW, Cm, Ck, true, Ck);
+  if (pk.v != 0 || pk.ksplit != 1 || pk.jw < 4) return false;
+  return (32 * 36 * 8 + 4 * 2 * 16 * 64) * 4 <= (int)x6c_lds_bytes(pk.csl, 2, 3, 2) - 4 * ((pk.csl + 3) & ~3);
+}
+
 __global__ __launch_bounds__(256) void x6c_post_act_kernel(float* __restrict__ y, const float* __restrict__ res, long long n4, int act) {
   typedef float f32x4p __attribute__((ext_vector_type(4)));
   for (long long i = blockIdx.x * 256ll + threadIdx.x; i < n4; i += (long long)gridDim.x * 256) {
@@ -990,19 +1165,16 @@
 
 static thread_local const void* g_next_splanes = nullptr;
 
-static size_t x6c_lds_bytes(int csl, int tm, int tps) {
-  const int ring = tps == 9 ? 3 : (tm == 2 ? 4 : 6);
-  return sizeof(float) * (size_t)((csl + 3) & ~3) + 16 * (size_t)(ring * 6 * tps * 32 * tm + 2 * 6 * csl);
-}
-
-static X6cGeom x6c_geom(const PatchGeom& g, const ClassSpec* css, int ncls, const X6cPick& pk, int halo, int ns, const uint16_t* wb, int ntaps_w) {
+
+static X6cGeom x6c_geom(const PatchGeom& g, const ClassSpec* css, int ncls, const X6cPick& pk, int halo, int ns, const uint16_t* wb, int ntaps_w,
+                        int planes = 3) {
   const ClassSpec& c0 = css[0];
   X6cGeom k{};
   k.src = g.src; k.dst = g.dst; k.wb = wb; k.bias = g.bias; k.res = g.res; k.mask_y = g.mask_y;
   int tw_max = 0;
   for (int q = 0; q < ncls; ++q)
     for (int i = 0; i < css[q].ntaps; ++i) tw_max = css[q].tw[i] > tw_max ? css[q].tw[i] : tw_max;
-  k.wb_bytes = (2u * (unsigned)ntaps_w + (unsigned)tw_max + 1u) * (unsigned)g.Ck * (unsigned)g.CmPad * 2u;
+  k.wb_bytes = ((unsigned)(planes - 1) * (unsigned)ntaps_w + (unsigned)tw_max + 1u) * (unsigned)g.Ck * (unsigned)g.CmPad * 2u;
   k.act_epi = g.act_epi; k.mask_act = g.mask_act;
   k.B = g.B; k.Ck = g.Ck; k.Cm = g.Cm; k.CmPad = g.CmPad;
   k.sH = g.sH; k.sW = g.sW; k.dT = g.dT; k.dH = g.dH; k.dW = g.dW; k.nH = c0.nH; k.nW = c0.nW;
@@ -1025,15 +1197,16 @@
   }
   P2I_LAUNCH(KERN, grid, dim3(NTHR), lds, s, k);
 }
-static void x6c_dispatch(const X6cGeom& k, const X6cVariant& tv, int tps, bool fused, int* plan6, hipStream_t s) {
-  const size_t lds = x6c_lds_bytes(k.CSl, tv.TM, tps);
+static void x6c_dispatch(const X6cGeom& k, const X6cVariant& tv, int tps, bool fused, int* plan6, hipStream_t s, bool f16 = false) {
+  const size_t lds = x6c_lds_bytes(k.CSl, tv.TM, tps, f16 ? 2 : 3);
   const dim3 grid((unsigned)(ceil_div(k.B * k.nT, 1 << k.ljb) * k.nth * k.ntw), (unsigned)ceil_div(k.Cm, 32 * tv.TM), (unsigned)k.ksplit);
   const bool pc = x6c_pc() && k.Ck >= 32 && (!fused || tps == 9);
-  if (plan6) { plan6[0] = 32 * tv.TM; plan6[1] = 32 * tv.NW; plan6[2] = k.ksplit; plan6[3] = pc ? 4 : 8; plan6[4] = tps; plan6[5] = fused ? 8 : 7; }
+  if (plan6) { plan6[0] = 32 * tv.TM; plan6[1] = 32 * tv.NW; plan6[2] = k.ksplit; plan6[3] = f16 ? 6 : (pc ? 4 : 8); plan6[4] = tps; plan6[5] = fused ? 8 : 7; }
   const bool pre = k.splanes != nullptr;
   if (!fused && pc) {
     if (tv.TM == 2) {
-      if (k.vec4_epi) x6c_launch<patch_gemm_x6p_kernel<2, 3, false, true>, 512>(k, grid, lds, s);
+      if (f16) x6c_launch<patch_gemm_x6p_kernel<2, 3, false, true, 4, 2, false, true>, 512>(k, grid, lds, s);
+      else if (k.vec4_epi) x6c_launch<patch_gemm_x6p_kernel<2, 3, false, true>, 512>(k, grid, lds, s);
       else x6c_launch<patch_gemm_x6p_kernel<2, 3>, 512>(k, grid, lds, s);
     } else if (tv.NW == 4) {
       if (pre) x6c_launch<patch_gemm_x6p_kernel<1, 9, false, false, 8, 1, true>, 768>(k, grid, lds, s);
@@ -1053,7 +1226,8 @@
 }
 
 int run_patch_gemm_x6c(const PatchGeom& g, const ClassSpec& cs, const uint16_t* wb, int ntaps_w, int* plan6, hipStream_t s, bool dry) {
-  if (!x6c_on() || (!dry && wb == nullptr) || g.src_y != nullptr || (g.Ck & 15) != 0 || g.Ck < 16) return 1;
+  const X6Ctx& xc = x6_ctx();
+  if (!x6c_on() || (!dry && wb == nullptr && xc.wh == nullptr) || g.src_y != nullptr || (g.Ck & 15) != 0 || g.Ck < 16) return 1;
   if (cs.mH != 1 || cs.mW != 1 || cs.oH != 1 || cs.oW != 1 || cs.pH || cs.pW) return 1;
   if (cs.ntaps != 9 && cs.ntaps != 18 && cs.ntaps != 27) return 1;
   const int ns = cs.ntaps / 9;
@@ -1080,9 +1254,18 @@
   if (pk.v < 0) return 1;
   const unsigned long long sbytes = 4ull * g.B * g.Ck * g.sT * g.sH * g.sW;
   if (sbytes >= 0x7FFFFFF0ull || 4ull * (unsigned long long)n_dst >= 0x7FFFFFF0ull) return 1;
+  const X6cVariant& tv = kX6cVariants[pk.v];
+  const int tps = tv.NW == 4 ? 9 : (tv.TM == 1 ? x6c_tps1() : 3);
+  auto al16 = [](const void* q) { return ((uintptr_t)q & 15) == 0; };
+  auto v4_ok = [&](int planes) {
+    return P2I_ENV_ONCE("P2I_X6C_EPI4", 1) && tv.TM == 2 && pk.ksplit == 1 && pk.jw >= 4 && (cs.nW & 3) == 0 && (g.dW & 3) == 0 && al16(g.dst) && al16(g.res) &&
+           al16(g.mask_y) && (32 * 36 * 8 + 4 * tv.TM * 16 * 64) * 4 <= (int)x6c_lds_bytes(pk.csl, tv.TM, tps, planes) - 4 * ((pk.csl + 3) & ~3);
+  };
+  const bool f16 = xc.wh != nullptr && xc.src_part != nullptr && xc.src_count >= 1 && xc.src_count <= X6H_MAX_PART && xc.w_kexp != nullptr && x6p_f16_on() &&
+                   ns == 1 && x6c_pc() && g.Ck >= 32 && v4_ok(2);
+  if (!f16 && wb == nullptr) return 1;
   if (dry) return 0;
-  const X6cVariant& tv = kX6cVariants[pk.v];
-  X6cGeom k = x6c_geom(g, &cs, 1, pk, 2, ns, wb, ntaps_w);
+  X6cGeom k = x6c_geom(g, &cs, 1, pk, 2, ns, f16 ? xc.wh : wb, ntaps_w, f16 ? 2 : 3);
   k.bH = lo[1]; k.bW = lo[2];
   for (int i = 0; i < 9; ++i) {
     k.tap_w[i] = cs.tw[i];
@@ -1091,8 +1274,6 @@
   k.sdt0 = cs.dt[0]; k.swt0 = 0;
   k.sdt1 = ns > 1 ? cs.dt[9] : 0; k.swt1 = ns > 1 ? cs.tw[9] - cs.tw[0] : 0;
   k.sdt2 = ns > 2 ? cs.dt[18] : 0; k.swt2 = ns > 2 ? cs.tw[18] - cs.tw[0] : 0;
-  const int tps = tv.NW == 4 ? 9 : (tv.TM == 1 ? x6c_tps1() : 3);
-  const size_t lds = x6c_lds_bytes(k.CSl, tv.TM, tps);
   const int post_act = (pk.ksplit > 1 && g.act_epi != P2I_ACT_NONE) ? g.act_epi : P2I_ACT_NONE;
   if (pk.ksplit > 1) {
     if (p2i::memset_async(g.dst, 0, sizeof(float) * (size_t)n_dst, s) != hipSuccess) return P2I_EINVAL;
@@ -1105,13 +1286,13 @@
     }
     g_next_splanes = nullptr;
   }
-  {
-    const int v4_on = P2I_ENV_ONCE("P2I_X6C_EPI4", 1);
-    auto al16 = [](const void* q) { return ((uintptr_t)q & 15) == 0; };
-    k.vec4_epi = v4_on && tv.TM == 2 && pk.ksplit == 1 && pk.jw >= 4 && (cs.nW & 3) == 0 && (g.dW & 3) == 0 && al16(g.dst) && al16(k.res) && al16(g.mask_y) &&
-                 (32 * 36 * 8 + 4 * tv.TM * 16 * 64) * 4 <= (int)lds - 4 * ((k.CSl + 3) & ~3);
-  }
-  x6c_dispatch(k, tv, tps, false, plan6, s);
+  k.vec4_epi = f16 || v4_ok(3);
+  if (f16) {
+    k.src_part = xc.src_part; k.src_count = xc.src_count; k.w_kexp = xc.w_kexp; k.dst_part = nullptr;
+    const long long wgs = (long long)ceil_div(k.B * k.nT, 1 << k.ljb) * k.nth * k.ntw * ceil_div(k.Cm, 64);
+    if (xc.dst_part != nullptr && xc.dst_count != nullptr && wgs <= X6H_MAX_PART) { k.dst_part = xc.dst_part; *xc.dst_count = (int)wgs; }
+  }
+  x6c_dispatch(k, tv, tps, false, plan6, s, f16);
   if (post_act != P2I_ACT_NONE) {
     const long long n4 = n_dst / 4;
     const long long blocks = (n4 + 255) / 256;
@@ -1169,6 +1350,29 @@
 
 }
 
+extern "C" int p2i_x6h_split(const float* wp, uint16_t* wh, int32_t* kexp, uint32_t* part, int n, int taps, int K, int Mpad, void* stream) {
+  using namespace p2i;
+  P2I_REQUIRE(wp && wh && kexp && part && n >= 1 && n <= 65535 && taps > 0 && K > 0 && (K & 7) == 0 && Mpad > 0 && (Mpad & 31) == 0, "p2i_x6h_split: bad arguments");
+  const long long per_layer = (long long)taps * K * Mpad;
+  P2I_REQUIRE((long long)n * per_layer < (1ll << 31), "p2i_x6h_split: stack too large");
+  const int units = taps * (K >> 3) * Mpad;
+  int blocks = (units + 255) / 256;
+  blocks = blocks > 64 ? 64 : blocks;
+  P2I_LAUNCH(wabsmax_kernel, dim3(blocks, n), dim3(256), 0, (hipStream_t)stream, wp, per_layer, part);
+  P2I_LAUNCH(wsplit_f16_kernel, dim3(blocks, n), dim3(256), 0, (hipStream_t)stream, wp, reinterpret_cast<u32x4c*>(wh), kexp, part, blocks, n, taps, K, Mpad);
+  return launch_status();
+}
+
+extern "C" int p2i_absmax_partials(const float* x, int64_t n, uint32_t* part, int* count, void* stream) {
+  using namespace p2i;
+  P2I_REQUIRE(x && part && count && n > 0 && ((uintptr_t)x & 15) == 0, "p2i_absmax_partials: non-empty, 16-byte aligned tensor");
+  const long long blocks = ((n >> 2) + 256 * 8 - 1) / (256 * 8);
+  const int nb = blocks < 1 ? 1 : (blocks > X6H_MAX_PART ? X6H_MAX_PART : (int)blocks);
+  P2I_LAUNCH(absmax_partials_kernel, dim3(nb), dim3(256), 0, (hipStream_t)stream, x, (long long)n, part);
+  *count = nb;
+  return launch_status();
+}
+
 extern "C" int p2i_x6_split_batched(const float* const* wp, uint16_t* const* wb, const int* ntaps, const int* K, const int* Mpad, int n,
                                     void* stream) {
   using namespace p2i;
diff --git a/p2i-gan-benchmark_amd/p2igan_bench/_hip.py b/p2i-gan-benchmark_amd/p2igan_bench/_hip.py
--- a/p2i-gan-benchmark_amd/p2igan_bench/_hip.py
+++ b/p2i-gan-benchmark_amd/p2igan_bench/_hip.py
@@ -34,6 +34,11 @@
     "p2i_x6c_would_take": [_D, _I, _I],
     "p2i_conv_fwd_x6s": [_D, _P, _P, _P, _I, _P, _P, _P, _I, _P],
     "p2i_conv_dgrad_x6s": [_D, _P, _P, _P, _I, _P, _P, _I, _P, _P],
+    "p2i_absmax_partials": [_P, _L, _P, C.POINTER(C.c_int), _P],
+    "p2i_x6h_split": [_P, _P, _P, _P, _I, _I, _I, _I, _P],
+    "p2i_x6h_would_take": [_D, _I],
+    "p2i_conv_fwd_x6h": [_D, _P, _P, _P, _P, _P, _I, _P, _I, _P, C.POINTER(C.c_int), _P, _P, _P, _I, _P],
+    "p2i_conv_dgrad_x6h": [_D, _P, _P, _P, _P, _P, _I, _P, _I, _P, C.POINTER(C.c_int), _P, _P, _I, _P, _P],
     "p2i_conv_last_plan": [C.POINTER(C.c_int)],
     "p2i_wgrad_last_plan": [C.POINTER(C.c_int)],
     "p2i_fast_div_magic": [_I, C.POINTER(C.c_uint32)],
diff --git a/p2i-gan-benchmark_amd/p2igan_bench/models/p2igan.py b/p2i-gan-benchmark_amd/p2igan_bench/models/p2igan.py
--- a/p2i-gan-benchmark_amd/p2igan_bench/models/p2igan.py
+++ b/p2i-gan-benchmark_amd/p2igan_bench/models/p2igan.py
@@ -189,8 +189,11 @@
         for cv, wp in zip(convs, wps):
             prep["folded"][id(cv)] = wp
         d = _spec2d(ch, ch, 3).desc(b, 1, h >> lvl, w >> lvl)
-        ops._x6s_of(wps[0][0], d, False, ACT_RELU)
-        ops._x6s_of(wps[0][1], d, True)
+        for wp_, dg in ((wps[0][0], False), (wps[0][1], True)):
+            if ops.x6h_stack_take(wp_, d, dg):
+                wp_._x6s[0].layer_h(0)
+            else:
+                ops._x6s_of(wp_, d, dg, ACT_NONE if dg else ACT_RELU)
     for i in (2, 1, 0):
         up = net.UP[i]
         cin_, cout_ = up.proj.weight.shape[1], up.proj.weight.shape[0]
@@ -243,12 +246,23 @@
             convs = [_doconv_of(m) for rb in net.Decoder[lvl].layers for m in (rb.main[0], rb.main[1])]
             for cv, wp in zip(convs, ops.doconv_fold_batched([cv.tensors() for cv in convs], ch, ch, need_d=True)):
                 folded[id(cv)] = wp
+        d = spec.desc(b, 1, h >> lvl, w >> lvl)
+        sc = None
+        f16 = None
         for rb in net.Decoder[lvl].layers:
             c1, c2 = _doconv_of(rb.main[0]), _doconv_of(rb.main[1])
             w1 = folded[id(c1)] if need_grad else fold(c1, ch, ch, 1, 3)
             w2 = folded[id(c2)] if need_grad else fold(c2, ch, ch, 1, 3)
-            y1 = ops.conv_fwd(spec, hcur, w1[0], act=ACT_RELU)
-            hn = ops.conv_fwd(spec, y1, w2[0], residual=hcur)
+            if f16 is None:
+                f16 = ops.x6h_stack_take(w1[0], d, False)
+            if f16 and ops.x6h_has_stack(w2[0]):
+                sc, s1, s2 = ops.scale_of(hcur, sc), ops.Scale(hcur.device), ops.Scale(hcur.device)
+                y1 = ops.conv_fwd(spec, hcur, w1[0], act=ACT_RELU, src_scale=sc, dst_scale=s1)
+                hn = ops.conv_fwd(spec, y1, w2[0], residual=hcur, src_scale=ops.scale_of(y1, s1), dst_scale=s2)
+                sc = s2
+            else:
+                y1 = ops.conv_fwd(spec, hcur, w1[0], act=ACT_RELU)
+                hn = ops.conv_fwd(spec, y1, w2[0], residual=hcur)
             rec.append((hcur, y1, w1[1], w2[1]))
             hcur = hn
         return hcur, rec
@@ -328,14 +342,29 @@
         spec = _spec2d(ch, ch, 3)
         blocks = net.Decoder[lvl].layers
         pend = []
+        d = spec.desc(b, 1, h >> lvl, w >> lvl)
+        sc = None
+        lvl_f16 = None
         for rb, (hin, y1, w1d, w2d) in zip(reversed(list(blocks)), reversed(S["rec"][lvl])):
             c1, c2 = _doconv_of(rb.main[0]), _doconv_of(rb.main[1])
+            if lvl_f16 is None:
+                lvl_f16 = ops.x6h_stack_take(w1d, d, True)
+            f16 = lvl_f16 and ops.x6h_has_stack(w2d)
+            if f16:
+                sc, s1, s2 = ops.scale_of(dh, sc), ops.Scale(dh.device), ops.Scale(dh.device)
             dwp2, _ = wgrad(spec, y1, dh)
             pend.append((dwp2, c2))
-            dy1 = ops.conv_dgrad(spec, dh, w2d, tuple(y1.shape), mask_y=y1, mask_act=ACT_RELU)
+            if f16:
+                dy1 = ops.conv_dgrad(spec, dh, w2d, tuple(y1.shape), mask_y=y1, mask_act=ACT_RELU, src_scale=sc, dst_scale=s1)
+            else:
+                dy1 = ops.conv_dgrad(spec, dh, w2d, tuple(y1.shape), mask_y=y1, mask_act=ACT_RELU)
             dwp1, _ = wgrad(spec, hin, dy1)
             pend.append((dwp1, c1))
-            dh = ops.conv_dgrad(spec, dy1, w1d, tuple(hin.shape), add=dh)
+            if f16:
+                dh = ops.conv_dgrad(spec, dy1, w1d, tuple(hin.shape), add=dh, src_scale=ops.scale_of(dy1, s1), dst_scale=s2)
+                sc = s2
+            else:
+                dh = ops.conv_dgrad(spec, dy1, w1d, tuple(hin.shape), add=dh)
         outs = ([cv.W.grad for _, cv in pend], [cv.D.grad for _, cv in pend]) if inplace else None
 
         def fold_level():
diff --git a/p2i-gan-benchmark_amd/p2igan_bench/ops.py b/p2i-gan-benchmark_amd/p2igan_bench/ops.py
--- a/p2i-gan-benchmark_amd/p2igan_bench/ops.py
+++ b/p2i-gan-benchmark_amd/p2igan_bench/ops.py
@@ -91,6 +91,9 @@
         _hip.load().p2i_conv_last_plan(plan)
         if plan[5] > 10:
             key = "patch_gemm_fused_kernel<%d, %d, %d, %d, %d> (strided dgrad, %d parity classes per workgroup)" % (plan[0], plan[1], plan[2], plan[3], plan[5] - 10, plan[5] - 10)
+        elif plan[5] == 7 and plan[3] == 6:
+            key = "patch_gemm_x6p_kernel<%d, %d, false, true, 4, 2, false, true> (%d x %d tile, %d taps per stage, producer / consumer waves, fp16-split x3)" % (
+                plan[0] // 32, plan[4], plan[0], plan[1], plan[4])
         elif plan[5] == 7 and plan[3] == 4:
             key = "patch_gemm_x6p_kernel<%d, %d, false> (%d x %d tile, %d taps per stage, producer / consumer waves, bf16-split x6)" % (
                 plan[0] // 32, plan[4], plan[0], plan[1], plan[4])
@@ -132,6 +135,7 @@
     def __init__(self, wstack):
         self.w = wstack
         self.wb = None
+        self.wh = self.kexp = None
         self.n, self.taps, self.k, self.mpad = wstack.shape
 
     def layer_ptr(self, i):
@@ -139,6 +143,14 @@
             self.wb = torch.empty(3 * self.w.numel(), device=self.w.device, dtype=torch.int16)
             _hip.check(_hip.load().p2i_x6_split(_ptr(self.w), _ptr(self.wb), self.n * self.taps, self.k, self.mpad, _stream()), "p2i_x6_split")
         return self.wb.data_ptr() + 2 * i * self.taps * self.k * self.mpad
+
+    def layer_h(self, i):
+        if self.wh is None:
+            self.wh = torch.empty(2 * self.w.numel(), device=self.w.device, dtype=torch.int16)
+            self.kexp = torch.empty(65 * self.n, device=self.w.device, dtype=torch.int32)
+            _hip.check(_hip.load().p2i_x6h_split(_ptr(self.w), _ptr(self.wh), _ptr(self.kexp), self.kexp.data_ptr() + 4 * self.n, self.n,
+                                                 self.taps, self.k, self.mpad, _stream()), "p2i_x6h_split")
+        return self.wh.data_ptr() + 2 * i * self.taps * self.k * self.mpad, self.kexp.data_ptr() + 4 * i
 
     @staticmethod
     def attach(wstack, views):
@@ -190,6 +202,64 @@
     return st.layer_ptr(i), st.n * st.taps
 
 
+_SCALE_POOL = {}
+_SCALE_SLOTS = 64
+
+
+class Scale:
+    __slots__ = ("ptr", "count", "_ring", "_slot")
+
+    def __init__(self, device):
+        key = (device.index, _stream())
+        ent = _SCALE_POOL.get(key)
+        if ent is None:
+            ent = _SCALE_POOL[key] = [torch.empty(_SCALE_SLOTS * 1024, device=device, dtype=torch.int32), 0]
+        self._ring, self._slot = ent[0], ent[1]
+        self.ptr = ent[0].data_ptr() + 4096 * ent[1]
+        ent[1] = (ent[1] + 1) % _SCALE_SLOTS
+        self.count = 0
+
+    def words(self) -> torch.Tensor:
+        return self._ring[1024 * self._slot:1024 * self._slot + self.count]
+
+
+def absmax_partials(x: torch.Tensor) -> Scale:
+    import ctypes
+    _chk(x)
+    sc = Scale(x.device)
+    cnt = ctypes.c_int(0)
+    _hip.check(_hip.load().p2i_absmax_partials(_ptr(x), x.numel(), sc.ptr, ctypes.byref(cnt), _stream()), "p2i_absmax_partials")
+    sc.count = cnt.value
+    return sc
+
+
+def x6h_would_take(d, dgrad: bool) -> bool:
+    return CONV_ENGINE in ("auto", "x6") and bool(_hip.load().p2i_x6h_would_take(d, 1 if dgrad else 0))
+
+
+def x6h_has_stack(wp) -> bool:
+    h = getattr(wp, "_x6s", None)
+    return h is not None and isinstance(h[0], X6Stack)
+
+
+def x6h_stack_take(wp, d, dgrad: bool) -> bool:
+    return x6h_has_stack(wp) and x6h_would_take(d, dgrad)
+
+
+def scale_of(x: torch.Tensor, sc: Optional["Scale"]) -> "Scale":
+    return sc if (sc is not None and sc.count > 0) else absmax_partials(x)
+
+
+def _x6h_of(wp, d, dgrad, src_scale):
+    if src_scale is None or src_scale.count < 1 or not x6h_would_take(d, dgrad):
+        return None
+    h = getattr(wp, "_x6s", None)
+    st, i = h if (h is not None and isinstance(h[0], X6Stack)) else (X6Stack(wp.reshape((1,) + tuple(wp.shape))), 0)
+    wh, kexp = st.layer_h(i)
+    wb = st.layer_ptr(i) if st.wb is not None else None
+    return wb, wh, kexp, st.n * st.taps, st
+
+
 WGRAD_SLICES = _os.environ.get("P2I_WGRAD_SLICES", "1") != "0"
 _WGRAD_WS = {}
 
@@ -335,7 +405,7 @@
     return b, c, t, h, w
 
 
-def conv_fwd(spec: ConvSpec, x, wp_f, bias=None, residual=None, act=ACT_NONE, out=None):
+def conv_fwd(spec: ConvSpec, x, wp_f, bias=None, residual=None, act=ACT_NONE, out=None, src_scale=None, dst_scale=None):
     lib = _hip.load()
     b, c, t, h, w = _dims5(x)
     if c != spec.cin or tuple(wp_f.shape) != spec.wp_f_shape():
@@ -350,6 +420,17 @@
     _chk(x, wp_f, bias, residual, y)
     d = spec.desc(b, t, h, w)
     e0 = _prof_begin()
+    h16 = _x6h_of(wp_f, d, False, src_scale)
+    if h16 is not None:
+        import ctypes
+        cnt = ctypes.c_int(0)
+        _hip.check(lib.p2i_conv_fwd_x6h(d, _ptr(x), _ptr(wp_f), h16[0], h16[1], h16[2], h16[3], src_scale.ptr, src_scale.count,
+                                        dst_scale.ptr if dst_scale is not None else None, ctypes.byref(cnt), _ptr(bias), _ptr(residual), _ptr(y), act,
+                                        _stream()), "p2i_conv_fwd_x6h")
+        if dst_scale is not None:
+            dst_scale.count = cnt.value
+        _prof_end(e0, "fwd", spec, d, True)
+        return y
     pre = _x6s_of(wp_f, d, False, act)
     ws = _x6_scratch(3 * wp_f.numel(), x.device) if (pre is None and spec.cin % 16 == 0) else None
     if pre is not None:
@@ -364,7 +445,8 @@
     return y
 
 
-def conv_dgrad(spec: ConvSpec, dy, wp_d, in_shape, y_act=None, act=ACT_NONE, add=None, mask_y=None, mask_act=ACT_NONE):
+def conv_dgrad(spec: ConvSpec, dy, wp_d, in_shape, y_act=None, act=ACT_NONE, add=None, mask_y=None, mask_act=ACT_NONE, src_scale=None,
+               dst_scale=None):
     lib = _hip.load()
     if len(in_shape) == 4:
         b, c, h, w = in_shape
@@ -385,6 +467,17 @@
     _chk(dy, wp_d, y_act, dx, add, mask_y)
     d = spec.desc(b, t, h, w)
     e0 = _prof_begin()
+    h16 = _x6h_of(wp_d, d, True, src_scale) if y_act is None else None
+    if h16 is not None:
+        import ctypes
+        cnt = ctypes.c_int(0)
+        _hip.check(lib.p2i_conv_dgrad_x6h(d, _ptr(dy), _ptr(wp_d), h16[0], h16[1], h16[2], h16[3], src_scale.ptr, src_scale.count,
+                                          dst_scale.ptr if dst_scale is not None else None, ctypes.byref(cnt), _ptr(add), _ptr(mask_y), mask_act,
+                                          _ptr(dx), _stream()), "p2i_conv_dgrad_x6h")
+        if dst_scale is not None:
+            dst_scale.count = cnt.value
+        _prof_end(e0, "dgrad", spec, d, True)
+        return dx
     pre = _x6s_of(wp_d, d, True) if y_act is None else None
     ws = _x6_scratch(3 * wp_d.numel(), dy.device) if (pre is None and y_act is None and spec.cout % 16 == 0 and spec.cin > 1) else None
     if pre is not None:
```

Result: no change. 11490, median of 6 (+0.3%).
